# 0xPolygonHermez/pil2-stark-js

Hardware: AMD Instinct MI355X
Metric: STARK prove time (ms_per_step) and trace-cells/s, synthetic Fibonacci AIR, GL Poseidon Merkle + FRI, blow-up 8 (higher is better)
Workload: dtype u64; 1 GPU; full proof (commit, Q, evals, FRI 27/22/17/12/7, 64 queries) of 2^24 rows x 100 cols -> 2^27 rows, plain linear hash, per GPU; mode=prove, config=c3, nBits=24, nCols=100, nBitsExt=27, hash=GL-Poseidon-12, parallelism=single GPU

## Files before the change

### include/pil2gl.h

```cpp
#pragma once
#include <stdint.h>
#include "pil2gl_expr.h"
#ifdef __cplusplus
extern "C" {
#endif

#define PIL2GL_OK        0
#define PIL2GL_EINVAL   -1
#define PIL2GL_ENODEV   -2
#define PIL2GL_ENOMEM   -3
#define PIL2GL_EHIP     -4

int         pil2gl_init(int device);
void        pil2gl_shutdown(void);
const char *pil2gl_last_error(void);
int         pil2gl_version(void);
int         pil2gl_device_info(char *name, uint32_t nameLen, uint32_t *numCUs, uint64_t *totalMem);

int pil2gl_dev_alloc(uint64_t nWords, uint64_t **out);
int pil2gl_dev_free(uint64_t *p);
int pil2gl_dev_zero(uint64_t *p, uint64_t nWords, void *stream);
int pil2gl_dev_upload(uint64_t *dst, const uint64_t *hostSrc, uint64_t nWords);
int pil2gl_dev_download(uint64_t *hostDst, const uint64_t *src, uint64_t nWords);
int pil2gl_sync(void *stream);

int pil2gl_host_alloc(uint64_t nWords, uint64_t **out);
int pil2gl_host_free(uint64_t *p);
int pil2gl_host_register(uint64_t *p, uint64_t nWords);
int pil2gl_host_unregister(uint64_t *p);
int pil2gl_dev_upload_async(uint64_t *dst, const uint64_t *hostSrc, uint64_t nWords);
int pil2gl_dev_download_async(uint64_t *hostDst, const uint64_t *src, uint64_t nWords);
int pil2gl_copy_after(void *stream);
int pil2gl_copy_fence(void *stream);
int pil2gl_copy_sync(void);
int pil2gl_land_rows_dev(const uint64_t *src, uint64_t srcCols, uint64_t *dst, uint64_t dstCols, uint64_t nRows,
                         uint64_t *hostFirstBad, void *stream);
int pil2gl_dev_load_file(const char *fileName, uint64_t byteOffset, uint64_t nRows, uint64_t srcCols,
                         uint64_t *dst, uint64_t dstCols, uint64_t chunkWords, uint64_t *hostFirstBad);
int pil2gl_dev_save_file(const char *fileName, uint64_t byteOffset, const uint64_t *src, uint64_t nWords, uint64_t chunkWords);

int pil2gl_interpolate(const uint64_t *src, uint64_t nPols, uint32_t nBits, uint64_t *dst, uint32_t nBitsExt);
int pil2gl_interpolate_dev(const uint64_t *src, uint64_t nPols, uint32_t nBits, uint64_t *dst, uint32_t nBitsExt, void *stream);
int pil2gl_interpolate_cosets_dev(const uint64_t *src, uint64_t nPols, uint32_t nBits, uint64_t *dst, uint32_t nBitsExt,
                                  uint32_t cosetBegin, uint32_t cosetCount, void *stream);
int pil2gl_extend_cosets_unshifted_dev(const uint64_t *src, uint64_t nPols, uint32_t nBits, uint64_t *dst, uint32_t nBitsExt,
                                       uint32_t cosetBegin, uint32_t cosetCount, void *stream);
int pil2gl_extend_coefs_brev_dev(const uint64_t *coefBrev, uint64_t nPols, uint32_t nBits, uint64_t *dst, uint32_t nBitsExt, void *stream);
int pil2gl_extend_coefs_brev_cosets_dev(const uint64_t *coefBrev, uint64_t nPols, uint32_t nBits, uint64_t *dst, uint32_t nBitsExt,
                                        uint32_t cosetBegin, uint32_t cosetCount, void *stream);
int pil2gl_interpolate_cosets_ws_dev(const uint64_t *src, uint64_t nPols, uint32_t nBits, uint64_t *dst, uint32_t nBitsExt,
                                     uint32_t cosetBegin, uint32_t cosetCount, uint64_t *workspace, void *stream);
int pil2gl_fft(const uint64_t *src, uint64_t nPols, uint32_t nBits, uint64_t *dst);
int pil2gl_ifft(const uint64_t *src, uint64_t nPols, uint32_t nBits, uint64_t *dst);
int pil2gl_fft_dev(const uint64_t *src, uint64_t nPols, uint32_t nBits, uint64_t *dst, void *stream);
int pil2gl_ifft_dev(const uint64_t *src, uint64_t nPols, uint32_t nBits, uint64_t *dst, void *stream);
int pil2gl_fft_block_dev(uint64_t *buf, uint64_t start_pos, uint64_t nPols, uint32_t nBits, uint32_t s, uint32_t blockBits, uint32_t layers, void *stream);
int pil2gl_interpolate_prepare_block_dev(uint64_t *buf, uint64_t width, uint64_t height, uint64_t start, uint64_t inc, void *stream);

int pil2gl_poseidon(const uint64_t *in, const uint64_t *cap, uint64_t count, uint32_t nOut, uint64_t *out);
int pil2gl_poseidon_dev(const uint64_t *in, const uint64_t *cap, uint64_t count, uint32_t nOut, uint64_t *out, void *stream);
int pil2gl_sponge_absorb(const uint64_t *hostBlocks, uint64_t nBlocks, const uint64_t hostCap[4], uint64_t hostOut12[12]);
int pil2gl_linear_hash_rows(const uint64_t *in, uint64_t width, uint64_t height, int split, uint64_t *out);
int pil2gl_linear_hash_rows_dev(const uint64_t *in, uint64_t width, uint64_t height, int split, uint64_t *out, void *stream);
int pil2gl_merkelize_level(const uint64_t *in, uint64_t nOps, uint64_t *out);
int pil2gl_merkelize_level_dev(const uint64_t *in, uint64_t nOps, uint64_t *out, void *stream);
uint64_t pil2gl_merkle_num_nodes(uint64_t height);
int pil2gl_merkelize(const uint64_t *elems, uint64_t width, uint64_t height, int split, uint64_t *nodes);
int pil2gl_merkelize_dev(const uint64_t *elems, uint64_t width, uint64_t height, int split, uint64_t *nodes, void *stream);
int pil2gl_merkelize_digests_dev(uint64_t *nodes, uint64_t height, void *stream);
int pil2gl_group_proof_dev(const uint64_t *elems, const uint64_t *nodes, uint64_t width, uint64_t height,
                           uint64_t idx, uint64_t *hostVals, uint64_t *hostSiblings, uint32_t *nLevels);

int pil2gl_group_proofs_dev(const uint64_t *elems, const uint64_t *nodes, uint64_t width, uint64_t height,
                            const uint64_t *hostIdxs, uint32_t nIdx, uint64_t *hostOut, uint32_t *nLevels);
int pil2gl_roots_from_group_proofs(const uint64_t *hostProofs, uint64_t width, uint32_t levels, const uint64_t *hostIdxs, uint32_t nIdx,
                                   int splitLinearHash, uint64_t *hostRoots );

int pil2gl_fri_fold(const uint64_t *pol, uint32_t polBits, uint32_t outBits, uint64_t shiftInv,
                    const uint64_t challenge[3], uint64_t *out);
int pil2gl_fri_fold_dev(const uint64_t *pol, uint32_t polBits, uint32_t outBits, uint64_t shiftInv,
                        const uint64_t challenge[3], uint64_t *out, void *stream);
int pil2gl_fri_verify_fold(const uint64_t *groups, uint32_t foldBits, uint32_t nQueries, const uint64_t *sinv,
                           const uint64_t challenge[3], uint64_t *out );
int pil2gl_fri_verify_fold_dev(const uint64_t *groups, uint32_t foldBits, uint32_t nQueries, const uint64_t *sinv,
                               const uint64_t challenge[3], uint64_t *out, void *stream);
int pil2gl_fri_transpose(const uint64_t *pol, uint32_t polBits, uint32_t transposeBits, uint64_t *out);
int pil2gl_fri_transpose_dev(const uint64_t *pol, uint32_t polBits, uint32_t transposeBits, uint64_t *out, void *stream);

int pil2gl_build_x_dev(uint32_t nBits, uint64_t shift, uint64_t *x, void *stream);
int pil2gl_geometric_dev(uint64_t first, uint64_t ratio, uint64_t n, uint64_t *out, void *stream);
int pil2gl_build_zhinv_dev(uint32_t nBits, uint32_t nBitsExt, uint64_t *out, void *stream);
int pil2gl_build_one_row_zerofier_inv_dev(uint32_t nBits, uint32_t nBitsExt, uint64_t rowIndex, uint64_t *out, void *stream);
int pil2gl_build_frame_zerofier_dev(uint32_t nBits, uint32_t nBitsExt, uint64_t offsetMin, uint64_t offsetMax, uint64_t *out, void *stream);
int pil2gl_compute_q_split_dev(const uint64_t *qq1, uint32_t nBits, uint32_t nBitsExt, uint32_t qDim, uint32_t qDeg, uint64_t *qq2, void *stream);
int pil2gl_compute_q_split_brev_dev(const uint64_t *qq1, uint32_t nBits, uint32_t nBitsExt, uint32_t qDim, uint32_t qDeg, uint64_t *coefBrev, void *stream);
int pil2gl_compute_q_stark_dev(const glx_program *prog, const glx_ctx *ctx, uint32_t qSection, uint32_t nBits, uint32_t nBitsExt,
                               uint32_t qDim, uint32_t qDeg, uint64_t *dstExt, void *stream);
int pil2gl_x_div_x_sub_xi_dev(uint32_t nBitsExt, const uint64_t xi[3], uint64_t nOpen, uint64_t iOpen, uint64_t *out, void *stream);
int pil2gl_x_div_x_sub_xi_cosets_dev(uint32_t nBitsExt, uint32_t extBits, const uint64_t xi[3], uint64_t nOpen, uint64_t iOpen,
                                     uint32_t cosetBegin, uint32_t cosetCount, uint64_t *out, void *stream);
int pil2gl_build_lev_dev(uint32_t nBits, const uint64_t xi[3], uint64_t *lev, void *stream);
typedef struct { const uint64_t *buf; uint64_t width; uint64_t offset; uint32_t dim; uint32_t levIndex; } pil2gl_eval_desc;
int pil2gl_compute_evals_dev(const pil2gl_eval_desc *descs, uint32_t nEvals, uint32_t nBits, uint32_t extendBits,
                             const uint64_t *const *levs, uint32_t nLevs, uint64_t *hostEvals , void *stream);

int pil2gl_rows_dot_ext_dev(const uint64_t *buf, uint64_t width, uint64_t nRows, const uint64_t *hostCoef, uint32_t nOut,
                            uint64_t *acc, int accumulate, void *stream);
int pil2gl_rows_dot_ext_multi_dev(const uint64_t *const *bufs, const uint64_t *widths, uint32_t nBufs, uint64_t nRows,
                                  const uint64_t *const *hostCoefs, uint32_t nOut, uint64_t *acc, int accumulate, void *stream);
int pil2gl_fri_combine_dev(const uint64_t *acc, const uint64_t *hostK, const uint64_t vf1[3], const uint64_t *xDivXSubXi,
                           uint32_t nOpen, uint64_t nRows, uint64_t *f, void *stream);
int pil2gl_fri_combine_order_dev(const uint64_t *acc, const uint64_t *hostK, const uint64_t vf1[3], const uint64_t *xDivXSubXi,
                                 uint32_t nOpen, const uint32_t *order, uint64_t nRows, uint64_t *f, void *stream);
int pil2gl_cols_dot_ext_dev(const uint64_t *buf, uint64_t width, uint64_t nRows, uint64_t rowStep, const uint64_t *const *levs,
                            uint32_t nLev, uint64_t *hostOut, void *stream);
int pil2gl_cols_dot_ext_multi_dev(const uint64_t *const *bufs, const uint64_t *widths, uint32_t nBufs, uint64_t nRows, uint64_t rowStep,
                                  const uint64_t *const *levs, uint32_t nLev, uint64_t *const *hostOuts, void *stream);
int pil2gl_cols_dot_ext_range_dev(const uint64_t *const *bufs, const uint64_t *strides, const uint64_t *colBegin, const uint64_t *widths, uint32_t nBufs,
                                  uint64_t nRows, uint64_t rowStep, const uint64_t *const *levs, uint32_t nLev, uint64_t *const *hostOuts, void *stream);

int pil2gl_eval_program_dev(const glx_program *prog, const glx_ctx *ctx, void *stream);
int pil2gl_first_nonzero_row_dev(const uint64_t *col, uint32_t dim, uint64_t first, uint64_t last, uint64_t *hostRow, uint64_t *hostVal, void *stream);

int pil2gl_gprod_dev(const uint64_t *num, uint32_t dimNum, const uint64_t *den, uint32_t dimDen, uint64_t n, uint64_t *out, void *stream);
int pil2gl_gsum_dev(const uint64_t *num, uint32_t dimNum, const uint64_t *den, uint32_t dimDen, uint64_t n, uint64_t *out, void *stream);
int pil2gl_h1h2_dev(const uint64_t *f, const uint64_t *t, uint64_t n, uint32_t dim, uint64_t *h1, uint64_t *h2, void *stream);

int pil2gl_bn128_poseidon(const uint64_t *in, const uint64_t *init, uint64_t count, uint32_t nIn, uint32_t nOut, uint64_t *out);
int pil2gl_bn128_sponge_absorb(const uint64_t *hostBlocks, uint64_t nBlocks, uint32_t nIn, const uint64_t hostInit[4], uint64_t *hostOut);
int pil2gl_bn128_poseidon_dev(const uint64_t *in, const uint64_t *init, uint64_t count, uint32_t nIn, uint32_t nOut, uint64_t *out, void *stream);
int pil2gl_bn128_linear_hash_rows(const uint64_t *in, uint64_t width, uint64_t height, uint32_t arity, int custom, uint64_t *out);
int pil2gl_bn128_linear_hash_rows_dev(const uint64_t *in, uint64_t width, uint64_t height, uint32_t arity, int custom, uint64_t *out, void *stream);
int pil2gl_bn128_merkelize_level_dev(const uint64_t *in, uint64_t nOps, uint32_t arity, uint64_t *out, void *stream);
uint64_t pil2gl_bn128_merkle_num_nodes(uint64_t height, uint32_t arity);
int pil2gl_bn128_merkelize(const uint64_t *elems, uint64_t width, uint64_t height, uint32_t arity, int custom, uint64_t *nodes);
int pil2gl_bn128_merkelize_dev(const uint64_t *elems, uint64_t width, uint64_t height, uint32_t arity, int custom, uint64_t *nodes, void *stream);
int pil2gl_bn128_group_proof_dev(const uint64_t *elems, const uint64_t *nodes, uint64_t width, uint64_t height, uint32_t arity,
                                 uint64_t idx, uint64_t *hostVals, uint64_t *hostSiblings, uint32_t *nLevels);
int pil2gl_bn128_group_proofs_dev(const uint64_t *elems, const uint64_t *nodes, uint64_t width, uint64_t height, uint32_t arity,
                                  const uint64_t *hostIdxs, uint32_t nIdx, uint64_t *hostVals, uint64_t *hostSiblings, uint32_t *nLevels);
int pil2gl_bn128_convert(const uint64_t *in, uint64_t n, int toMontgomery, uint64_t *out);
int pil2gl_bn128_convert_dev(const uint64_t *in, uint64_t n, int toMontgomery, uint64_t *out, void *stream);

int pil2gl_synth_fibonacci_dev(uint32_t nBits, uint32_t nPairs, const uint64_t *hostInit, uint64_t *cm, void *stream);

uint64_t pil2gl_add(uint64_t a, uint64_t b);
uint64_t pil2gl_mul(uint64_t a, uint64_t b);
uint64_t pil2gl_square(uint64_t a);

int pil2gl_selftest_field(const uint64_t *a, const uint64_t *b, uint64_t n, uint64_t *mul, uint64_t *add, uint64_t *sub);
int pil2gl_debug_compact_program(const glx_program *prog, glx_op *outOps, uint32_t *outInfo);
int pil2gl_debug_jit_compile(const glx_program *prog, const glx_ctx *ctx, uint64_t *codeBytes, uint32_t *fusedOps);
int pil2gl_debug_plan_program(const glx_program *prog, const glx_ctx *ctx, uint32_t *outInfo);
#define PIL2GL_PLAN_FFT 0
#define PIL2GL_PLAN_IFFT 1
#define PIL2GL_PLAN_INTERPOLATE 2
#define PIL2GL_PLAN_EXTEND_COEFS 3
#define PIL2GL_PLAN_LAUNCH_WORDS 14
int pil2gl_debug_plan_transform(uint32_t op, uint32_t nBits, uint64_t nPols, uint32_t nBitsExt, uint32_t cosetCount,
                                uint32_t *out, uint32_t maxLaunches, uint32_t *nLaunches);
int pil2gl_selftest_products(const uint64_t *a, const uint64_t *b, uint64_t n, uint64_t *x, uint64_t *pb, uint64_t *flag);
int pil2gl_selftest_mds(const uint64_t *states, uint64_t n, uint32_t layers, int mfma, uint64_t *out);
int pil2gl_selftest_poseidon(const uint64_t *states, uint64_t n, int what, uint64_t *out);
int pil2gl_selftest_clock(uint32_t iters, double *mhz);
int pil2gl_selftest_ext(const uint64_t *a, const uint64_t *b, uint64_t n, uint64_t *mul, uint64_t *inv);

#ifdef __cplusplus
}
#endif
```

### pil2-stark-js_amd/csrc/dot.hip

```cpp
#include "common.h"
#include "gl_field.cuh"
#include <vector>
#include <string.h>
#include <stdint.h>
#include <stdlib.h>
#include <algorithm>

using namespace gl;

namespace {

constexpr u32 LIMB_BITS = 22;
constexpr u32 LIMB_MASK = (1u << LIMB_BITS) - 1;

__device__ __forceinline__ u64 fold6(const u64 S[6]) {
    u64 r = canon(S[0]);
    r = add(r, mul(S[1], 1ull << 22));
    r = add(r, mul(S[2], 1ull << 44));
    r = add(r, mul(S[3], 1ull << 32));
    r = add(r, mul(S[4], 1ull << 54));
    r = add(r, mul(S[5], ((1ull << 32) - 1) << 12));
    return r;
}

struct RowsDotParams {
    const u64 *buf; u64 width; u64 nRows;
    u64 stride, col0;
    const u32 *coefLimbs;
    u32 nOut;
    u64 *acc;
    u32 accumulate;
};

template <int NOUT>
__global__ void __launch_bounds__(256) rows_dot_kernel(RowsDotParams P) {
    constexpr u32 CW = 16, LD = CW + 1;
    __shared__ u64 tile[4][64 * LD];
    const u32 wave = threadIdx.x >> 6, lane = threadIdx.x & 63;
    u64 *T = tile[wave];
    const u64 row0 = ((u64)blockIdx.x * 4 + wave) * 64;
    if (row0 >= P.nRows) return;
    u64 S[NOUT][3][6];
#pragma unroll
    for (int o = 0; o < NOUT; o++)
#pragma unroll
        for (int k = 0; k < 3; k++)
#pragma unroll
            for (int i = 0; i < 6; i++) S[o][k][i] = 0;
    const u64 myRow = row0 + lane;
    u64 nxt[CW];
    const u32 lr = lane >> 4, lc = lane & 15;
    auto fetch = [&](u64 c0) {
        const u32 cw = (u32)min((u64)CW, P.width - c0);
        u64 off = (row0 + lr) * P.stride + P.col0 + c0 + lc;
        asm volatile("" : "+v"(off));
        const u64 step = 4 * P.stride;
#pragma unroll
        for (u32 i = 0; i < CW; i++) {
            const u64 gr = row0 + lr + 4 * i;
            nxt[i] = (lc < cw && gr < P.nRows) ? P.buf[off + i * step] : 0;
        }
    };
    fetch(0);
    for (u64 c0 = 0; c0 < P.width; c0 += CW) {
        const u32 cw = (u32)min((u64)CW, P.width - c0);
        {
            u32 to = lr * LD + lc;
            asm volatile("" : "+v"(to));
#pragma unroll
            for (u32 i = 0; i < CW; i++) T[to + i * 4 * LD] = nxt[i];
        }
        if (c0 + CW < P.width) fetch(c0 + CW);
        __builtin_amdgcn_s_waitcnt(0xC07F);
        __builtin_amdgcn_wave_barrier();
        for (u32 c = 0; c < cw; c++) {
            const u64 p = T[lane * LD + c];
            const u32 p0 = (u32)p, p1 = (u32)(p >> 32);
#pragma unroll
            for (int o = 0; o < NOUT; o++) {
                const u32 *L = P.coefLimbs + (((u64)o * P.stride + P.col0 + c0 + c) * 9);
#pragma unroll
                for (int k = 0; k < 3; k++) {
                    const u32 w0 = L[3 * k], w1 = L[3 * k + 1], w2 = L[3 * k + 2];
                    S[o][k][0] += (u64)p0 * w0; S[o][k][1] += (u64)p0 * w1; S[o][k][2] += (u64)p0 * w2;
                    S[o][k][3] += (u64)p1 * w0; S[o][k][4] += (u64)p1 * w1; S[o][k][5] += (u64)p1 * w2;
                }
            }
        }
        __builtin_amdgcn_wave_barrier();
    }
    if (myRow >= P.nRows) return;
    u64 *out = P.acc + myRow * (3ull * P.nOut);
#pragma unroll
    for (int o = 0; o < NOUT; o++)
#pragma unroll
        for (int k = 0; k < 3; k++) {
            u64 v = fold6(S[o][k]);
            if (P.accumulate) v = add(v, out[3 * o + k]);
            out[3 * o + k] = v;
        }
}

constexpr u32 STREAM_CW_MAX = 128;
template <int NOUT>
__global__ void __launch_bounds__(256) rows_dot_stream_kernel(RowsDotParams P, u32 cw, u32 LD) {
    extern __shared__ u64 sm[];
    const u32 tid = threadIdx.x, lane = tid & 63;
    const u32 wave = __builtin_amdgcn_readfirstlane(tid >> 6);
    const u64 row0 = (u64)blockIdx.x * 64;
    u64 S[NOUT][3][6];
#pragma unroll
    for (int o = 0; o < NOUT; o++)
#pragma unroll
        for (int k = 0; k < 3; k++)
#pragma unroll
            for (int i = 0; i < 6; i++) S[o][k][i] = 0;
    constexpr u32 NB = 13;
    for (u64 c0 = 0; c0 < P.width; c0 += cw) {
        const u32 w = (u32)min((u64)cw, P.width - c0);
        const u32 total = 64 * w, dq = 256 / w, dr = 256 - dq * w;
        u32 r = tid / w, c = tid - r * w;
        for (u32 u0 = 0; u0 < total; u0 += 256 * NB) {
            u64 v[NB]; u32 at[NB];
#pragma unroll
            for (u32 i = 0; i < NB; i++) {
                const bool in = u0 + 256 * i + tid < total;
                at[i] = in ? r * LD + c : 0xFFFFFFFFu;
                v[i] = (in && row0 + r < P.nRows) ? P.buf[(row0 + r) * P.stride + P.col0 + c0 + c] : 0;
                c += dr; r += dq;
                if (c >= w) { c -= w; r++; }
            }
            if (u0 == 0) __syncthreads();
#pragma unroll
            for (u32 i = 0; i < NB; i++) if (at[i] != 0xFFFFFFFFu) sm[at[i]] = v[i];
        }
        __syncthreads();
        const u32 cb = w * wave / 4, ce = w * (wave + 1) / 4;
        for (u32 cc = cb; cc < ce; cc++) {
            const u64 p = sm[lane * LD + cc];
            const u32 p0 = (u32)p, p1 = (u32)(p >> 32);
#pragma unroll
            for (int o = 0; o < NOUT; o++) {
                const u32 *L = P.coefLimbs + (((u64)o * P.stride + P.col0 + c0 + cc) * 9);
#pragma unroll
                for (int k = 0; k < 3; k++) {
                    const u32 w0 = L[3 * k], w1 = L[3 * k + 1], w2 = L[3 * k + 2];
                    S[o][k][0] += (u64)p0 * w0; S[o][k][1] += (u64)p0 * w1; S[o][k][2] += (u64)p0 * w2;
                    S[o][k][3] += (u64)p1 * w0; S[o][k][4] += (u64)p1 * w1; S[o][k][5] += (u64)p1 * w2;
                }
            }
        }
    }
    __syncthreads();
    if (wave == 0) {
#pragma unroll
        for (int o = 0; o < NOUT; o++)
#pragma unroll
            for (int k = 0; k < 3; k++)
#pragma unroll
                for (int i = 0; i < 6; i++) sm[((o * 3 + k) * 6 + i) * 64 + lane] = S[o][k][i];
    }
    __syncthreads();
    if (wave != 0) {
#pragma unroll
        for (int o = 0; o < NOUT; o++)
#pragma unroll
            for (int k = 0; k < 3; k++)
#pragma unroll
                for (int i = 0; i < 6; i++)
                    __hip_atomic_fetch_add(&sm[((o * 3 + k) * 6 + i) * 64 + lane], S[o][k][i], __ATOMIC_RELAXED, __HIP_MEMORY_SCOPE_WORKGROUP);
    }
    __syncthreads();
    const u64 myRow = row0 + lane;
    if (myRow >= P.nRows) return;
    u64 *out = P.acc + myRow * (3ull * P.nOut);
    for (u32 pi = wave; pi < 3 * NOUT; pi += 4) {
        u64 T6[6];
#pragma unroll
        for (int i = 0; i < 6; i++) T6[i] = sm[(pi * 6 + i) * 64 + lane];
        u64 v = fold6(T6);
        if (P.accumulate) v = add(v, out[pi]);
        out[pi] = v;
    }
}


typedef int v4i __attribute__((ext_vector_type(4)));
typedef int v16i __attribute__((ext_vector_type(16)));
constexpr u32 MF_WAVES = 8, MF_ROWS = 64, MF_MAXW = 112;
constexpr int MF_PLANE_OFFSET = 1 << 24;

constexpr u32 MF_MAXSEG = 4;
struct RowsDotMfmaParams {
    const u64 *segBuf[MF_MAXSEG]; u32 segW[MF_MAXSEG], segPitch[MF_MAXSEG], segU0[MF_MAXSEG], nSeg;
    u64 nRows; u32 width, nOut;
    const v4i *atab;
    const u64 *bias;
    u64 *acc; u32 accumulate, accStride;
    u64 nTiles;
    u32 kSteps;
};

typedef int v4i_a8 __attribute__((ext_vector_type(4), aligned(8)));
template <int NT, bool ODD = false>
__global__ void __launch_bounds__(512, 1) rows_dot_mfma_kernel(RowsDotMfmaParams P) {
    extern __shared__ u64 sm[];
    constexpr u32 NTH = 64 * MF_WAVES, NG = MF_ROWS / 32;
    const u32 tid = threadIdx.x, lane = tid & 63;
    const u32 wave = __builtin_amdgcn_readfirstlane(tid >> 6);
    const u32 rowBytes = P.width * 8, LDB = rowBytes + 16;
    unsigned char *tile = (unsigned char *)sm;
    v4i *Alds = (v4i *)(tile + MF_ROWS * LDB);
    const u32 upr = P.width / 2;
    for (u32 i = tid; i < P.kSteps * NT * 64; i += NTH) Alds[i] = P.atab[i];
    const u32 n = lane & 31, gk = lane >> 5;
    const u32 total = MF_ROWS * upr, dq = NTH / upr, dr = NTH - dq * upr;
    constexpr u32 NL = (MF_ROWS * (MF_MAXW / 2) + NTH - 1) / NTH;
    const u32 r00 = tid / upr, c00 = tid - r00 * upr;
    v4i nxt[NL];
    auto fetch = [&](u64 tileIdx) {
        const u64 row0 = tileIdx * MF_ROWS;
        u32 r = r00, c = c00;
#pragma unroll
        for (u32 i = 0; i < NL; i++) {
            const v4i z = { 0, 0, 0, 0 };
            const u64 *sb = P.segBuf[0]; u32 sw = P.segW[0], sp = P.segPitch[0], su = 0;
#pragma unroll
            for (u32 k = 1; k < MF_MAXSEG; k++) if (k < P.nSeg && c >= P.segU0[k]) { sb = P.segBuf[k]; sw = P.segW[k]; sp = P.segPitch[k]; su = P.segU0[k]; }
            if constexpr (!ODD) nxt[i] = (NTH * i + tid < total && row0 + r < P.nRows) ? *(const v4i *)(sb + (row0 + r) * sp + 2 * (c - su)) : z;
            else {
                nxt[i] = z;
                if (NTH * i + tid < total && row0 + r < P.nRows) {
                    const u64 *q = sb + (row0 + r) * sp + 2 * (c - su);
                    if (2 * (c - su) + 1 < sw) nxt[i] = *(const v4i_a8 *)q;
                    else { const u64 v = *q; nxt[i][0] = (int)(u32)v; nxt[i][1] = (int)(u32)(v >> 32); }
                }
            }
            c += dr; r += dq;
            if (c >= upr) { c -= upr; r++; }
        }
    };
    if (blockIdx.x < P.nTiles) fetch(blockIdx.x);
    const u32 g = wave / NT, t = wave - g * NT;
    const unsigned char *brow = tile + (32 * g + n) * LDB + 16 * gk;
    const v4i *arow = Alds + t * 64 + lane;
    for (u64 tileIdx = blockIdx.x; tileIdx < P.nTiles; tileIdx += gridDim.x) {
        const u64 row0 = tileIdx * MF_ROWS;
        __syncthreads();
        {
            u32 r = r00, c = c00;
#pragma unroll
            for (u32 i = 0; i < NL; i++) {
                if (NTH * i + tid < total) *(v4i *)(tile + r * LDB + 16 * c) = nxt[i] ^ (int)0x80808080;
                c += dr; r += dq;
                if (c >= upr) { c -= upr; r++; }
            }
        }
        if (tileIdx + gridDim.x < P.nTiles) fetch(tileIdx + gridDim.x);
        __syncthreads();
        if (wave < NG * NT) {
            v16i acc;
#pragma unroll
            for (int i = 0; i < 16; i++) acc[i] = MF_PLANE_OFFSET;
            for (u32 s_ = 0; s_ < P.kSteps; s_++)
                acc = __builtin_amdgcn_mfma_i32_32x32x32_i8(arow[s_ * NT * 64], *(const v4i *)(brow + 32 * s_), acc, 0, 0, 0);
            const u32 o = 2 * t + gk;
            const u64 row = row0 + 32 * g + n;
            if (o < 3 * P.nOut && row < P.nRows) {
                u64 w[4];
#pragma unroll
                for (int j = 0; j < 4; j++)
                    w[j] = (u64)(u32)acc[4 * j] + ((u64)(u32)acc[4 * j + 1] << 8) + ((u64)(u32)acc[4 * j + 2] << 16) + ((u64)(u32)acc[4 * j + 3] << 24);
                u64 v = add(add(w[0], mul(w[1], 1ull << 32)), mul(w[2], EPS));
                v = add(sub(v, w[3]), P.bias[o]);
                u64 *out = P.acc + row * (u64)P.accStride + o;
                if (P.accumulate) v = add(v, *out);
                *out = v;
            }
        }
    }
}

__global__ void fri_combine_kernel(const u64 *__restrict__ acc, const u64 *__restrict__ K, E3 vf1, const u64 *__restrict__ xdiv,
                                   u32 nOpen, u32 order, u64 nRows, u64 *__restrict__ f) {
    const u64 r = (u64)blockIdx.x * blockDim.x + threadIdx.x;
    if (r >= nRows) return;
    E3 res = { { 0, 0, 0 } };
    for (u32 k = 0; k < nOpen; k++) {
        const u32 o = (order >> (8 * k)) & 255;
        const u64 *a = acc + (r * nOpen + o) * 3, *x = xdiv + (r * nOpen + o) * 3;
        E3 F = { { sub(a[0], K[3 * o]), sub(a[1], K[3 * o + 1]), sub(a[2], K[3 * o + 2]) } };
        E3 X = { { x[0], x[1], x[2] } };
        E3 t = e3_mul(F, X);
        res = k == 0 ? t : e3_add(e3_mul(vf1, res), t);
    }
    f[3 * r] = res.v[0]; f[3 * r + 1] = res.v[1]; f[3 * r + 2] = res.v[2];
}

constexpr u32 CD_MAXSEG = 8;
struct ColsDotParams {
    const u64 *segBuf[CD_MAXSEG]; u32 segW[CD_MAXSEG], segC0[CD_MAXSEG], segStride[CD_MAXSEG], nSeg;
    u64 width; u64 nRows; u64 rowStep;
    const u32 *levLimbs;
    u32 nLev;
    u64 *partial;
    u32 rowsPerChunk;
};

template <int NLEV>
__global__ void __launch_bounds__(256) cols_dot_kernel(ColsDotParams P) {
    const u64 c = (u64)blockIdx.y * blockDim.x + threadIdx.x;
    const u64 chunk = blockIdx.x;
    const u64 k0 = chunk * P.rowsPerChunk, k1 = min(P.nRows, k0 + P.rowsPerChunk);
    u64 S[NLEV][3][6];
#pragma unroll
    for (int l = 0; l < NLEV; l++)
#pragma unroll
        for (int k = 0; k < 3; k++)
#pragma unroll
            for (int i = 0; i < 6; i++) S[l][k][i] = 0;
    const bool valid = c < P.width;
    constexpr int RB = 8;
    const u64 *buf = P.segBuf[0]; u64 sw = P.segStride[0], cl = c;
#pragma unroll
    for (u32 k = 1; k < CD_MAXSEG; k++) if (k < P.nSeg && c >= P.segC0[k]) { buf = P.segBuf[k]; sw = P.segStride[k]; cl = c - P.segC0[k]; }
    const u64 stride = P.rowStep * sw;
    for (u64 kb = k0; kb < k1; kb += RB) {
        u64 pv[RB];
#pragma unroll
        for (int j = 0; j < RB; j++) pv[j] = (valid && kb + j < k1) ? buf[(kb + j) * stride + cl] : 0;
#pragma unroll
        for (int j = 0; j < RB; j++) {
            const u64 k = kb + j;
            if (k >= k1) break;
            const u32 p0 = (u32)pv[j], p1 = (u32)(pv[j] >> 32);
#pragma unroll
            for (int l = 0; l < NLEV; l++) {
                const u32 *L = P.levLimbs + (((u64)l * P.nRows + k) * 9);
#pragma unroll
                for (int q = 0; q < 3; q++) {
                    const u32 w0 = L[3 * q], w1 = L[3 * q + 1], w2 = L[3 * q + 2];
                    S[l][q][0] += (u64)p0 * w0; S[l][q][1] += (u64)p0 * w1; S[l][q][2] += (u64)p0 * w2;
                    S[l][q][3] += (u64)p1 * w0; S[l][q][4] += (u64)p1 * w1; S[l][q][5] += (u64)p1 * w2;
                }
            }
        }
    }
    if (!valid) return;
#pragma unroll
    for (int l = 0; l < NLEV; l++)
#pragma unroll
        for (int q = 0; q < 3; q++)
            P.partial[((chunk * P.nLev + l) * P.width + c) * 3 + q] = fold6(S[l][q]);
}
__global__ void cols_dot_final_kernel(const u64 *__restrict__ partial, u64 nChunks, u64 per, u64 n , u64 *__restrict__ out) {
    const u64 i = (u64)blockIdx.x * blockDim.x + threadIdx.x;
    if (i >= n) return;
    const u64 c0 = (u64)blockIdx.y * per, c1 = min(nChunks, c0 + per);
    u64 acc = 0;
    for (u64 ch = c0; ch < c1; ch++) acc = add(acc, partial[ch * n + i]);
    out[(u64)blockIdx.y * n + i] = acc;
}
__global__ void limbs_kernel(const u64 *__restrict__ in, u64 n, u32 *__restrict__ out) {
    const u64 i = (u64)blockIdx.x * blockDim.x + threadIdx.x;
    if (i >= n) return;
    const u64 v = in[i];
    out[3 * i] = (u32)v & LIMB_MASK; out[3 * i + 1] = (u32)(v >> LIMB_BITS) & LIMB_MASK; out[3 * i + 2] = (u32)(v >> (2 * LIMB_BITS));
}

inline unsigned nblk(u64 n, u32 t = 256) { return (unsigned)((n + t - 1) / t); }

}

using namespace pil2gl;

struct MfSeg { const u64 *buf; u64 pitch, col0, width; const u64 *coef; };
static u64 mf_padded(const MfSeg *segs, u32 n) { u64 t = 0; for (u32 k = 0; k < n; k++) t += segs[k].width + (segs[k].width & 1); return t; }
static bool rows_dot_mfma_fits(const MfSeg *segs, u32 nSeg, u32 nOut) {
    const char *sw = getenv("PIL2GL_ROWS_DOT_MFMA");
    if ((sw && sw[0] == '0') || nOut < 1 || nOut > 2 || nSeg < 1 || nSeg > MF_MAXSEG) return false;
    for (u32 k = 0; k < nSeg; k++)
        if (segs[k].width == 0 || ((uintptr_t)segs[k].buf & 7) || (segs[k].pitch >> 31)) return false;
    const u64 total = mf_padded(segs, nSeg);
    if (total < 32 || total > MF_MAXW) return false;
    static int ldsMax = -1;
    if (ldsMax < 0) {
        int dev = 0, v = 0;
        (void)hipGetDevice(&dev);
        if (hipDeviceGetAttribute(&v, hipDeviceAttributeMaxSharedMemoryPerBlock, dev) != hipSuccess) v = 0;
        ldsMax = v;
    }
    const u32 kSteps = (u32)((total * 8 + 31) / 32), NT = nOut == 1 ? 2 : 3;
    const size_t need = (size_t)MF_ROWS * (total * 8 + 16) + (size_t)kSteps * NT * 1024;
    return (size_t)ldsMax >= need;
}
static int launch_rows_dot_mfma(const MfSeg *segs, u32 nBufs, u64 nRows, u32 nOut, u64 *acc, u32 accStride, bool accumulate, hipStream_t st) {
    const u64 Pm = 0xFFFFFFFF00000001ull;
    const int NT = nOut == 1 ? 2 : 3;
    const u32 nO = 3 * nOut;
    const u64 winWidth = mf_padded(segs, nBufs);
    bool odd = false;
    for (u32 k = 0; k < nBufs; k++) odd |= ((segs[k].width | segs[k].pitch | segs[k].col0) & 1) != 0 || ((uintptr_t)segs[k].buf & 15);
    std::vector<signed char> dig((size_t)winWidth * nO * 9, 0);
    std::vector<u64> bias(nO);
    unsigned __int128 k128 = 0, offs = 0;
    for (int i = 0; i < 8; i++) k128 += (unsigned __int128)128 << (8 * i);
    {
        unsigned __int128 pw = 1;
        for (int p_ = 0; p_ < 16; p_++) { offs = (offs + (pw * (u64)MF_PLANE_OFFSET) % Pm) % Pm; pw = (pw * 256) % Pm; }
    }
    for (u32 o = 0; o < nO; o++) {
        unsigned __int128 sumw = 0;
        u64 c = 0;
        for (u32 k = 0; k < nBufs; k++, c += c & 1)
            for (u64 cl = 0; cl < segs[k].width; cl++, c++) {
                u64 w = segs[k].coef[((u64)(o / 3) * segs[k].pitch + segs[k].col0 + cl) * 3 + (o % 3)] % Pm;
                sumw = (sumw + w) % Pm;
                int carry = 0;
                for (int j = 0; j < 9; j++) {
                    int b = (j < 8 ? (int)((w >> (8 * j)) & 255) : 0) + carry;
                    carry = 0;
                    if (b >= 128) { b -= 256; carry = 1; }
                    dig[((size_t)c * nO + o) * 9 + j] = (signed char)b;
                }
            }
        unsigned __int128 b = ((k128 % Pm) * sumw) % Pm;
        bias[o] = (u64)((b + Pm - offs) % Pm);
    }
    const u32 kSteps = (u32)((winWidth * 8 + 31) / 32);
    std::vector<signed char> atab((size_t)kSteps * NT * 64 * 16, 0);
    for (u32 s_ = 0; s_ < kSteps; s_++)
        for (int t = 0; t < NT; t++)
            for (u32 lane = 0; lane < 64; lane++) {
                const u32 m = lane & 31, gk = lane >> 5;
                const u32 h = (m >> 2) & 1, pl = 4 * (m >> 3) + (m & 3), o = 2 * t + h;
                if (o >= nO) continue;
                signed char *dst = &atab[(((size_t)s_ * NT + t) * 64 + lane) * 16];
                for (u32 kk = 0; kk < 16; kk++) {
                    const u64 byteOff = 32ull * s_ + 16 * gk + kk;
                    if (byteOff >= winWidth * 8) continue;
                    const u64 c = byteOff >> 3; const u32 i = (u32)(byteOff & 7);
                    const int j = (int)pl - (int)i;
                    dst[kk] = (j >= 0 && j <= 8) ? dig[((size_t)c * nO + o) * 9 + j] : 0;
                }
            }
    u64 *d;
    const size_t atWords = (atab.size() + 7) / 8;
    P2_TRY(scratch(7, atWords + nO + 2, &d));
    HIP_TRY(hipMemcpyAsync(d, atab.data(), atab.size(), hipMemcpyHostToDevice, st));
    HIP_TRY(hipMemcpyAsync(d + atWords, bias.data(), nO * 8, hipMemcpyHostToDevice, st));
    RowsDotMfmaParams P;
    u32 u0 = 0;
    for (u32 k = 0; k < MF_MAXSEG; k++) {
        P.segBuf[k] = k < nBufs ? segs[k].buf + segs[k].col0 : nullptr; P.segW[k] = k < nBufs ? (u32)segs[k].width : 0; P.segPitch[k] = k < nBufs ? (u32)segs[k].pitch : 0; P.segU0[k] = u0;
        if (k < nBufs) u0 += (u32)((segs[k].width + 1) / 2);
    }
    P.nSeg = nBufs; P.nRows = nRows; P.width = (u32)winWidth; P.nOut = nOut; P.atab = (const v4i *)d; P.bias = d + atWords;
    P.acc = acc; P.accumulate = (u32)accumulate; P.accStride = accStride; P.nTiles = (nRows + MF_ROWS - 1) / MF_ROWS; P.kSteps = kSteps;
    const size_t lds = (size_t)MF_ROWS * (winWidth * 8 + 16) + atab.size();
    int dev = 0, cus = 256;
    (void)hipGetDevice(&dev);
    (void)hipDeviceGetAttribute(&cus, hipDeviceAttributeMultiprocessorCount, dev);
    const unsigned grid = (unsigned)std::min<u64>(P.nTiles, (u64)cus);
#define RD_LAUNCH(NT_, ODD_) { HIP_TRY(hipFuncSetAttribute((const void *)rows_dot_mfma_kernel<NT_, ODD_>, hipFuncAttributeMaxDynamicSharedMemorySize, (int)lds)); \
                              hipLaunchKernelGGL((rows_dot_mfma_kernel<NT_, ODD_>), dim3(grid), dim3(64 * MF_WAVES), lds, st, P); }
    if (NT == 2) { if (odd) RD_LAUNCH(2, true) else RD_LAUNCH(2, false) }
    else { if (odd) RD_LAUNCH(3, true) else RD_LAUNCH(3, false) }
#undef RD_LAUNCH
    KERNEL_CHECK();
    HIP_TRY(hipStreamSynchronize(st));
    return PIL2GL_OK;
}

static int rows_dot_ext_plain(const uint64_t *buf, uint64_t width, uint64_t nRows, const uint64_t *hostCoef, uint32_t nOut,
                              uint64_t *acc, int accumulate, void *stream) {
    hipStream_t st = as_stream(stream);
    const u64 nC = (u64)nOut * width * 3;
    std::vector<u32> limbs(nC * 3);
    for (u64 i = 0; i < nC; i++) {
        const u64 v = hostCoef[i] % 0xFFFFFFFF00000001ull;
        limbs[3 * i] = (u32)v & LIMB_MASK; limbs[3 * i + 1] = (u32)(v >> LIMB_BITS) & LIMB_MASK; limbs[3 * i + 2] = (u32)(v >> (2 * LIMB_BITS));
    }
    u64 *d;
    P2_TRY(scratch(7, (limbs.size() * 4 + 7) / 8 + 1, &d));
    HIP_TRY(hipMemcpyAsync(d, limbs.data(), limbs.size() * 4, hipMemcpyHostToDevice, st));
    const unsigned blocks = (unsigned)((nRows + 255) / 256);
    const char *sw = getenv("PIL2GL_ROWS_DOT_STREAM");
    const bool stream_ok = !(sw && sw[0] == '0');
    for (u64 col0 = 0; col0 < width; col0 += 1024) {
        RowsDotParams P = { buf, std::min<u64>(1024, width - col0), nRows, width, col0, (const u32 *)d, nOut, acc, (u32)(accumulate != 0 || col0 != 0) };
        if (stream_ok && P.width >= 32) {
            const u32 nch = (u32)((P.width + STREAM_CW_MAX - 1) / STREAM_CW_MAX), cw = (u32)((P.width + nch - 1) / nch), LD = cw | 1;
            const size_t lds = 8 * std::max<size_t>((size_t)64 * LD, (size_t)nOut * 18 * 64);
            const unsigned sb = (unsigned)((nRows + 63) / 64);
#define STREAM_CASE(N_) { if (lds > 48 * 1024) HIP_TRY(hipFuncSetAttribute((const void *)rows_dot_stream_kernel<N_>, hipFuncAttributeMaxDynamicSharedMemorySize, (int)lds)); \
                          hipLaunchKernelGGL((rows_dot_stream_kernel<N_>), dim3(sb), dim3(256), lds, st, P, cw, LD); }
            switch (nOut) {
            case 1: STREAM_CASE(1) break;
            case 2: STREAM_CASE(2) break;
            case 3: STREAM_CASE(3) break;
            default: STREAM_CASE(4) break;
            }
#undef STREAM_CASE
            KERNEL_CHECK();
            continue;
        }
        switch (nOut) {
        case 1: rows_dot_kernel<1><<<blocks, 256, 0, st>>>(P); break;
        case 2: rows_dot_kernel<2><<<blocks, 256, 0, st>>>(P); break;
        case 3: rows_dot_kernel<3><<<blocks, 256, 0, st>>>(P); break;
        default: rows_dot_kernel<4><<<blocks, 256, 0, st>>>(P); break;
        }
        KERNEL_CHECK();
    }
    HIP_TRY(hipStreamSynchronize(st));
    return PIL2GL_OK;
}

static bool rows_dot_mfma_plan(const uint64_t *const *bufs, const uint64_t *widths, const uint64_t *const *hostCoefs, u32 nBufs, u32 nOut,
                               std::vector<std::vector<MfSeg>> &launches, std::vector<u32> &leftovers) {
    std::vector<MfSeg> wins;
    for (u32 k = 0; k < nBufs; k++) {
        const u64 W = widths[k];
        if (W == 0) continue;
        const u64 n = (W + (W & 1) + MF_MAXW - 1) / MF_MAXW;
        u64 per = (W + n - 1) / n; per += per & 1;
        for (u64 c0 = 0; c0 < W; c0 += per) wins.push_back({ bufs[k], W, c0, std::min<u64>(per, W - c0), hostCoefs[k] });
    }
    std::stable_sort(wins.begin(), wins.end(), [](const MfSeg &a, const MfSeg &b) { return a.width > b.width; });
    std::vector<u64> fill;
    for (const MfSeg &w : wins) {
        const u64 pw = w.width + (w.width & 1);
        size_t b = 0;
        while (b < launches.size() && (launches[b].size() >= MF_MAXSEG || fill[b] + pw > MF_MAXW)) b++;
        if (b == launches.size()) { launches.emplace_back(); fill.push_back(0); }
        launches[b].push_back(w); fill[b] += pw;
    }
    bool any = false;
    for (size_t b = 0; b < launches.size();) {
        if (rows_dot_mfma_fits(launches[b].data(), (u32)launches[b].size(), std::min<u32>(nOut, 2))) { any = true; b++; continue; }
        for (const MfSeg &w : launches[b]) {
            if (w.width != w.pitch) return false;
            for (u32 k = 0; k < nBufs; k++) if (bufs[k] == w.buf && hostCoefs[k] == w.coef) { leftovers.push_back(k); break; }
        }
        launches.erase(launches.begin() + b); fill.erase(fill.begin() + b);
    }
    return any;
}

extern "C" {

int pil2gl_rows_dot_ext_multi_dev(const uint64_t *const *bufs, const uint64_t *widths, uint32_t nBufs, uint64_t nRows,
                                  const uint64_t *const *hostCoefs, uint32_t nOut, uint64_t *acc, int accumulate, void *stream);
int pil2gl_rows_dot_ext_dev(const uint64_t *buf, uint64_t width, uint64_t nRows, const uint64_t *hostCoef, uint32_t nOut,
                            uint64_t *acc, int accumulate, void *stream) {
    P2_TRY(ensure_init());
    if (!buf || !hostCoef || !acc) return fail(PIL2GL_EINVAL, "null buffer");
    if (nOut < 1 || nOut > 4) return fail(PIL2GL_EINVAL, "nOut must be 1..4");
    if (width == 0 || nRows == 0) return PIL2GL_OK;
    return pil2gl_rows_dot_ext_multi_dev(&buf, &width, 1, nRows, &hostCoef, nOut, acc, accumulate, stream);
}

int pil2gl_rows_dot_ext_multi_dev(const uint64_t *const *bufs, const uint64_t *widths, uint32_t nBufs, uint64_t nRows,
                                  const uint64_t *const *hostCoefs, uint32_t nOut, uint64_t *acc, int accumulate, void *stream) {
    P2_TRY(ensure_init());
    if (!bufs || !widths || !hostCoefs || !acc || nBufs == 0) return fail(PIL2GL_EINVAL, "null buffer");
    for (uint32_t k = 0; k < nBufs; k++) if (!bufs[k] || !hostCoefs[k]) return fail(PIL2GL_EINVAL, "null buffer");
    if (nOut < 1 || nOut > 4) return fail(PIL2GL_EINVAL, "nOut must be 1..4");
    if (nRows == 0) return PIL2GL_OK;
    std::vector<std::vector<MfSeg>> launches;
    std::vector<u32> leftovers;
    bool acc1 = accumulate != 0;
    if (rows_dot_mfma_plan(bufs, widths, hostCoefs, nBufs, nOut, launches, leftovers)) {
        for (u32 o0 = 0; o0 < nOut; o0 += 2) {
            const u32 no = std::min<u32>(2, nOut - o0);
            bool accg = accumulate != 0;
            for (auto l : launches) {
                for (MfSeg &sg : l) sg.coef += (u64)o0 * sg.pitch * 3;
                P2_TRY(launch_rows_dot_mfma(l.data(), (u32)l.size(), nRows, no, acc + 3 * o0, 3 * nOut, accg, as_stream(stream)));
                accg = true;
            }
        }
        acc1 = true;
        for (u32 k : leftovers) P2_TRY(rows_dot_ext_plain(bufs[k], widths[k], nRows, hostCoefs[k], nOut, acc, 1, stream));
        return PIL2GL_OK;
    }
    for (uint32_t k = 0; k < nBufs; k++) {
        if (widths[k] == 0) continue;
        P2_TRY(rows_dot_ext_plain(bufs[k], widths[k], nRows, hostCoefs[k], nOut, acc, acc1 ? 1 : 0, stream)); acc1 = true;
    }
    return PIL2GL_OK;
}

int pil2gl_fri_combine_dev(const uint64_t *acc, const uint64_t *hostK, const uint64_t vf1[3], const uint64_t *xDivXSubXi,
                           uint32_t nOpen, uint64_t nRows, uint64_t *f, void *stream) {
    const uint32_t ident[4] = { 0, 1, 2, 3 };
    return pil2gl_fri_combine_order_dev(acc, hostK, vf1, xDivXSubXi, nOpen, ident, nRows, f, stream);
}
int pil2gl_fri_combine_order_dev(const uint64_t *acc, const uint64_t *hostK, const uint64_t vf1[3], const uint64_t *xDivXSubXi,
                                 uint32_t nOpen, const uint32_t *order, uint64_t nRows, uint64_t *f, void *stream) {
    P2_TRY(ensure_init());
    if (!acc || !hostK || !vf1 || !xDivXSubXi || !f || !order || nOpen < 1 || nOpen > 4) return fail(PIL2GL_EINVAL, "bad FRI combine arguments");
    u32 ord = 0, seen = 0;
    for (u32 k = 0; k < nOpen; k++) {
        if (order[k] >= nOpen || (seen >> order[k] & 1)) return fail(PIL2GL_EINVAL, "order must be a permutation of the openings");
        seen |= 1u << order[k]; ord |= order[k] << (8 * k);
    }
    hipStream_t st = as_stream(stream);
    std::vector<u64> k(hostK, hostK + 3ull * nOpen);
    u64 *d;
    P2_TRY(scratch(7, 16, &d));
    HIP_TRY(hipMemcpyAsync(d, k.data(), k.size() * 8, hipMemcpyHostToDevice, st));
    E3 v = { { vf1[0], vf1[1], vf1[2] } };
    fri_combine_kernel<<<nblk(nRows), 256, 0, st>>>(acc, d, v, xDivXSubXi, nOpen, ord, nRows, f);
    KERNEL_CHECK();
    HIP_TRY(hipStreamSynchronize(st));
    return PIL2GL_OK;
}

int pil2gl_cols_dot_ext_multi_dev(const uint64_t *const *bufs, const uint64_t *widths, uint32_t nBufs, uint64_t nRows, uint64_t rowStep,
                                  const uint64_t *const *levs, uint32_t nLev, uint64_t *const *hostOuts, void *stream) {
    return pil2gl_cols_dot_ext_range_dev(bufs, widths, nullptr, widths, nBufs, nRows, rowStep, levs, nLev, hostOuts, stream);
}
int pil2gl_cols_dot_ext_range_dev(const uint64_t *const *bufs, const uint64_t *strides, const uint64_t *colBegin, const uint64_t *widths, uint32_t nBufs,
                                  uint64_t nRows, uint64_t rowStep, const uint64_t *const *levs, uint32_t nLev, uint64_t *const *hostOuts, void *stream) {
    P2_TRY(ensure_init());
    if (!bufs || !widths || !strides || !levs || !hostOuts || nBufs == 0) return fail(PIL2GL_EINVAL, "null buffer");
    for (uint32_t k = 0; k < nBufs && k < CD_MAXSEG; k++)
        if ((colBegin ? colBegin[k] : 0) + widths[k] > strides[k] || (strides[k] >> 31)) return fail(PIL2GL_EINVAL, "column range outside the matrix");
    if (nBufs > CD_MAXSEG) return fail(PIL2GL_EINVAL, "at most %u matrices per call", CD_MAXSEG);
    if (nLev < 1 || nLev > 64) return fail(PIL2GL_EINVAL, "nLev must be 1..64");
    u64 width = 0;
    for (uint32_t k = 0; k < nBufs; k++) { if (!bufs[k] || !hostOuts[k]) return fail(PIL2GL_EINVAL, "null buffer"); if (widths[k] >> 31) return fail(PIL2GL_EINVAL, "matrix too wide"); width += widths[k]; }
    for (uint32_t l = 0; l < nLev; l++) if (!levs[l]) return fail(PIL2GL_EINVAL, "null buffer");
    if (width == 0 || nRows == 0) return PIL2GL_OK;
    if (nLev > 4) {
        for (uint32_t l0 = 0; l0 < nLev; l0 += 4) {
            std::vector<uint64_t *> outs(nBufs);
            for (uint32_t k = 0; k < nBufs; k++) outs[k] = hostOuts[k] + (u64)l0 * widths[k] * 3;
            P2_TRY(pil2gl_cols_dot_ext_range_dev(bufs, strides, colBegin, widths, nBufs, nRows, rowStep, levs + l0, std::min<u32>(4, nLev - l0), outs.data(), stream));
        }
        return PIL2GL_OK;
    }
    hipStream_t st = as_stream(stream);
    const u32 rpc = 1024;
    const u64 nChunks = (nRows + rpc - 1) / rpc, n = (u64)nLev * width * 3;
    u64 *d;
    const u64 nGroups = std::min<u64>(64, nChunks), per = (nChunks + nGroups - 1) / nGroups;
    P2_TRY(scratch(7, ((u64)nLev * nRows * 9 * 4 + 7) / 8 + nChunks * n + nGroups * n + n + 1, &d));
    u32 *limbs = (u32 *)d;
    u64 *partial = d + ((u64)nLev * nRows * 9 * 4 + 7) / 8, *part2 = partial + nChunks * n, *res = part2 + nGroups * n;
    for (u32 l = 0; l < nLev; l++) limbs_kernel<<<nblk(nRows * 3), 256, 0, st>>>(levs[l], nRows * 3, limbs + (u64)l * nRows * 9);
    ColsDotParams P;
    u32 c0 = 0;
    for (u32 k = 0; k < CD_MAXSEG; k++) {
        P.segBuf[k] = k < nBufs ? bufs[k] + (colBegin ? colBegin[k] : 0) : nullptr; P.segW[k] = k < nBufs ? (u32)widths[k] : 0; P.segStride[k] = k < nBufs ? (u32)strides[k] : 0;
        P.segC0[k] = c0; if (k < nBufs) c0 += (u32)widths[k];
    }
    P.nSeg = nBufs; P.width = width; P.nRows = nRows; P.rowStep = rowStep; P.levLimbs = limbs; P.nLev = nLev; P.partial = partial; P.rowsPerChunk = rpc;
    const u32 threads = (u32)std::min<u64>(256, (width + 63) / 64 * 64);
    dim3 grid((unsigned)nChunks, nblk(width, threads));
    switch (nLev) {
    case 1: cols_dot_kernel<1><<<grid, threads, 0, st>>>(P); break;
    case 2: cols_dot_kernel<2><<<grid, threads, 0, st>>>(P); break;
    case 3: cols_dot_kernel<3><<<grid, threads, 0, st>>>(P); break;
    default: cols_dot_kernel<4><<<grid, threads, 0, st>>>(P); break;
    }
    cols_dot_final_kernel<<<dim3(nblk(n), (unsigned)nGroups), 256, 0, st>>>(partial, nChunks, per, n, part2);
    cols_dot_final_kernel<<<dim3(nblk(n), 1), 256, 0, st>>>(part2, (nChunks + per - 1) / per, nGroups, n, res);
    KERNEL_CHECK();
    std::vector<u64> host(n);
    HIP_TRY(hipMemcpyAsync(host.data(), res, n * 8, hipMemcpyDeviceToHost, st));
    HIP_TRY(hipStreamSynchronize(st));
    u64 cbeg = 0;
    for (uint32_t k = 0; k < nBufs; k++) {
        for (u32 l = 0; l < nLev; l++)
            memcpy(hostOuts[k] + ((u64)l * widths[k]) * 3, host.data() + ((u64)l * width + cbeg) * 3, widths[k] * 3 * 8);
        cbeg += widths[k];
    }
    return PIL2GL_OK;
}

int pil2gl_cols_dot_ext_dev(const uint64_t *buf, uint64_t width, uint64_t nRows, uint64_t rowStep, const uint64_t *const *levs,
                            uint32_t nLev, uint64_t *hostOut, void *stream) {
    if (!buf || !hostOut) { P2_TRY(ensure_init()); return fail(PIL2GL_EINVAL, "null buffer"); }
    return pil2gl_cols_dot_ext_multi_dev(&buf, &width, 1, nRows, rowStep, levs, nLev, &hostOut, stream);
}

}
```

### pil2-stark-js_amd/csrc/fri.hip

```cpp
#include "common.h"
#include "gl_field.cuh"
#include <vector>

using namespace gl;

namespace {

__device__ __forceinline__ u64 pow256(const u64 *__restrict__ T, u32 e) {
    u64 r = T[e & 255];
    r = mul_lazy(r, T[256 + ((e >> 8) & 255)]);
    r = mul_lazy(r, T[512 + ((e >> 16) & 255)]);
    return mul(r, T[768 + (e >> 24)]);
}
__device__ __forceinline__ u64 root_pow(const u64 *__restrict__ T, u32 logM, u32 e) { return logM ? pow256(T, e << (32 - logM)) : 1; }

__device__ __forceinline__ E3 ld3(const u64 *p) { return { { p[0], p[1], p[2] } }; }
__device__ __forceinline__ void st3(u64 *p, const E3 &v) { p[0] = v.v[0]; p[1] = v.v[1]; p[2] = v.v[2]; }

__global__ void fri_horner_kernel(const u64 *__restrict__ coef, u32 polBits, u64 pol2N, u64 nX, u64 shiftInv, E3 challenge,
                                  const u64 *__restrict__ powWi, const u64 *__restrict__ sinvOf, u64 *__restrict__ out) {
    const u64 g = (u64)blockIdx.x * blockDim.x + threadIdx.x;
    if (g >= pol2N) return;
    const u64 sinv = sinvOf ? sinvOf[g] : mul(shiftInv, root_pow(powWi, polBits, (u32)g));
    const E3 Y = e3_scale(challenge, sinv);
    E3 acc = ld3(coef + ((nX - 1) * pol2N + g) * 3);
    for (u64 i = nX - 1; i-- > 0;) acc = e3_add(e3_mul(acc, Y), ld3(coef + (i * pol2N + g) * 3));
    st3(out + 3 * g, acc);
}

__global__ void fri_transpose_kernel(const u64 *__restrict__ pol, u32 polBits, u32 tBits, u64 *__restrict__ out) {
    const u64 o = (u64)blockIdx.x * blockDim.x + threadIdx.x;
    const u64 n = 1ull << polBits;
    if (o >= n) return;
    const u64 h = n >> tBits;
    const u64 i = o / h, j = o - i * h;
    st3(out + 3 * o, ld3(pol + 3 * ((j << tBits) + i)));
}

__global__ void build_x_kernel(u32 nBits, u64 shift, const u64 *__restrict__ powW, u64 *__restrict__ x) {
    const u64 i = (u64)blockIdx.x * blockDim.x + threadIdx.x;
    if (i >= (1ull << nBits)) return;
    x[i] = mul(shift, root_pow(powW, nBits, (u32)i));
}
struct GeomPow { u64 p[40]; };
__global__ void geometric_kernel(u64 first, GeomPow R, u64 n, u64 *__restrict__ out) {
    const u64 i = (u64)blockIdx.x * blockDim.x + threadIdx.x;
    if (i >= n) return;
    u64 acc = first;
    for (u32 b = 0; (i >> b) != 0; b++) if ((i >> b) & 1) acc = mul(acc, R.p[b]);
    out[i] = acc;
}
__global__ void periodic_kernel(const u64 *__restrict__ tab, u64 period, u64 n, u64 *__restrict__ out) {
    const u64 i = (u64)blockIdx.x * blockDim.x + threadIdx.x;
    if (i < n) out[i] = tab[i % period];
}

template <int CH>
__device__ __forceinline__ void batch_inv(u64 v[CH]) {
    u64 pre[CH];
    u64 acc = 1;
#pragma unroll
    for (int i = 0; i < CH; i++) { pre[i] = acc; acc = mul(acc, v[i]); }
    u64 z = inv(acc);
#pragma unroll
    for (int i = CH - 1; i >= 0; i--) { u64 t = mul(z, pre[i]); z = mul(z, v[i]); v[i] = t; }
}

__global__ void one_row_zerofier_kernel(u32 nBitsExt, u64 root, const u64 *__restrict__ zh, u64 ext,
                                        const u64 *__restrict__ powW, u64 *__restrict__ out) {
    constexpr int CH = 8;
    const u64 i0 = ((u64)blockIdx.x * blockDim.x + threadIdx.x) * CH;
    const u64 n = 1ull << nBitsExt;
    if (i0 >= n) return;
    u64 v[CH];
#pragma unroll
    for (int k = 0; k < CH; k++) { u64 i = i0 + k < n ? i0 + k : i0; v[k] = sub(mul(7, root_pow(powW, nBitsExt, (u32)i)), root); }
    batch_inv<CH>(v);
#pragma unroll
    for (int k = 0; k < CH; k++) if (i0 + k < n) out[i0 + k] = mul(v[k], zh[(i0 + k) % ext]);
}
__global__ void frame_zerofier_kernel(u32 nBitsExt, const u64 *__restrict__ roots, u32 nRoots, const u64 *__restrict__ powW, u64 *__restrict__ out) {
    const u64 i = (u64)blockIdx.x * blockDim.x + threadIdx.x;
    if (i >= (1ull << nBitsExt)) return;
    const u64 x = mul(7, root_pow(powW, nBitsExt, (u32)i));
    u64 zi = 1;
    for (u32 j = 0; j < nRoots; j++) zi = mul(zi, sub(x, roots[j]));
    out[i] = zi;
}
__global__ void q_split_kernel(const u64 *__restrict__ qq1, u32 nBits, u32 nBitsExt, u32 qDim, u32 qDeg,
                               const u64 *__restrict__ sPow , u64 *__restrict__ qq2) {
    const u64 o = (u64)blockIdx.x * blockDim.x + threadIdx.x;
    const u64 W = (u64)qDim * qDeg, N = 1ull << nBits;
    if (o >= (W << nBitsExt)) return;
    const u64 i = o / W, r = o - i * W;
    if (i >= N) { qq2[o] = 0; return; }
    const u64 p = r / qDim, k = r - p * qDim;
    qq2[o] = mul(qq1[(p * N + i) * qDim + k], sPow[p]);
}
__global__ void q_split_brev_kernel(const u64 *__restrict__ qq1, u32 nBits, u32 qDim, u32 qDeg, const u64 *__restrict__ sPow, u64 *__restrict__ out) {
    const u64 o = (u64)blockIdx.x * blockDim.x + threadIdx.x;
    const u64 W = (u64)qDim * qDeg, N = 1ull << nBits;
    if (o >= W * N) return;
    const u64 i = o / W, r = o - i * W;
    const u64 p = r / qDim, k = r - p * qDim;
    out[(u64)bitrev32((u32)i, nBits) * W + r] = mul(qq1[(p * N + i) * qDim + k], sPow[p]);
}
constexpr int XD_BATCH = 16;
struct XDivConst { u64 xi0, b, c, c2, bc2, m1, k0, cc, ccbb; };
__global__ void __launch_bounds__(256) x_div_x_sub_xi_kernel(u32 nBitsExt, XDivConst K, u64 nOpen, u64 iOpen, const u64 *__restrict__ powW, u64 wStep, u64 *__restrict__ out,
                                                             u64 E , u32 extBits, u32 cosetBegin, u32 ccLog) {
    const u64 T = (u64)gridDim.x * blockDim.x;
    const u64 k0 = (u64)blockIdx.x * blockDim.x + threadIdx.x;
    if (k0 >= E) return;
    u64 xs[XD_BATCH], as[XD_BATCH], ts[XD_BATCH], pre[XD_BATCH];
    const u64 g0 = ((k0 >> ccLog) << extBits) + cosetBegin + (k0 & ((1ull << ccLog) - 1));
    u64 x = mul(7, root_pow(powW, nBitsExt, (u32)g0));
    int n = 0;
#pragma unroll
    for (int i = 0; i < XD_BATCH; i++) {
        if (k0 + (u64)i * T < E) {
            const u64 a = sub(x, K.xi0);
            const u64 u = mul(a, add(a, K.c2));
            const u64 t = add(mul(a, add(sub(K.m1, u), K.bc2)), K.k0);
            xs[i] = x; as[i] = a; ts[i] = t;
            pre[i] = i ? mul(pre[i - 1], t) : t;
            x = mul(x, wStep);
            n = i + 1;
        }
    }
    u64 tinv = inv(pre[n - 1]);
#pragma unroll
    for (int i = XD_BATCH - 1; i >= 0; i--) {
        if (i < n) {
            const u64 ti = i ? mul(tinv, pre[i - 1]) : tinv;
            if (i) tinv = mul(tinv, ts[i]);
            const u64 a = as[i], s = mul(ti, xs[i]);
            const u64 i1 = sub(K.m1, mul(a, add(a, K.c2)));
            const u64 i2 = sub(mul(K.b, a), K.cc);
            const u64 i3 = add(mul(K.c, a), K.ccbb);
            u64 *o = out + 3 * ((k0 + (u64)i * T) * nOpen + iOpen);
            o[0] = mul(i1, s); o[1] = mul(i2, s); o[2] = mul(i3, s);
        }
    }
}
__global__ void lev_pow_kernel(u32 nBits, const u64 *__restrict__ xiPow, u64 *__restrict__ lev) {
    const u64 k = (u64)blockIdx.x * blockDim.x + threadIdx.x;
    if (k >= (1ull << nBits)) return;
    E3 acc = { { 1, 0, 0 } };
    for (u32 b = 0; b < nBits; b++) if ((k >> b) & 1) acc = e3_mul(acc, ld3(xiPow + 3 * b));
    st3(lev + 3 * k, acc);
}
__global__ void evals_partial_kernel(pil2gl_eval_desc d, const u64 *__restrict__ lev, u32 nBits, u32 eb, u64 *__restrict__ partial) {
    __shared__ u64 red[256 * 3];
    const u64 N = 1ull << nBits;
    E3 acc = { { 0, 0, 0 } };
    for (u64 k = (u64)blockIdx.x * blockDim.x + threadIdx.x; k < N; k += (u64)gridDim.x * blockDim.x) {
        const u64 *v = d.buf + (k << eb) * d.width + d.offset;
        const E3 l = ld3(lev + 3 * k);
        acc = e3_add(acc, d.dim == 1 ? e3_scale(l, v[0]) : e3_mul(ld3(v), l));
    }
    red[threadIdx.x * 3] = acc.v[0]; red[threadIdx.x * 3 + 1] = acc.v[1]; red[threadIdx.x * 3 + 2] = acc.v[2];
    __syncthreads();
    for (u32 s = blockDim.x / 2; s > 0; s >>= 1) {
        if (threadIdx.x < s) for (int c = 0; c < 3; c++) red[threadIdx.x * 3 + c] = add(red[threadIdx.x * 3 + c], red[(threadIdx.x + s) * 3 + c]);
        __syncthreads();
    }
    if (threadIdx.x < 3) partial[(u64)blockIdx.x * 3 + threadIdx.x] = red[threadIdx.x];
}
__global__ void evals_final_kernel(const u64 *__restrict__ partial, u32 nBlocks, u32 nEvals, u64 *__restrict__ out) {
    const u32 e = blockIdx.x * blockDim.x + threadIdx.x;
    if (e >= nEvals * 3) return;
    const u32 ev = e / 3, c = e % 3;
    u64 acc = 0;
    for (u32 b = 0; b < nBlocks; b++) acc = add(acc, partial[((u64)ev * nBlocks + b) * 3 + c]);
    out[e] = acc;
}

__global__ void synth_fibonacci_kernel(u32 nBits, u32 nPairs, const u64 *__restrict__ init, u64 *__restrict__ cm) {
    const u32 k = blockIdx.x * blockDim.x + threadIdx.x;
    if (k >= nPairs) return;
    u64 l1 = canon(init[2 * k]), l2 = canon(init[2 * k + 1]);
    const u64 N = 1ull << nBits, W = 2ull * nPairs;
    for (u64 i = 0; i < N; i++) {
        cm[i * W + 2 * k] = l1; cm[i * W + 2 * k + 1] = l2;
        const u64 n1 = add(mul(l1, l1), mul(l2, l2));
        l2 = l1; l1 = n1;
    }
}

inline unsigned nblk(u64 n, u32 t = 256) { return (unsigned)((n + t - 1) / t); }

}

using namespace pil2gl;

extern "C" {

int pil2gl_fri_fold_dev(const uint64_t *pol, uint32_t polBits, uint32_t outBits, uint64_t shiftInv,
                        const uint64_t challenge[3], uint64_t *out, void *stream) {
    P2_TRY(ensure_init());
    if (!pol || !out || !challenge) return fail(PIL2GL_EINVAL, "null buffer");
    if (outBits > polBits || polBits > PIL2GL_MAX_NTT_BITS) return fail(PIL2GL_EINVAL, "Invalid polynomial size");
    hipStream_t st = as_stream(stream);
    const u64 n = 1ull << polBits;
    u64 *coef;
    P2_TRY(scratch(1, 3 * n, &coef));
    P2_TRY(ntt_launch(pol, 3ull << outBits, polBits - outBits, coef, true, st));
    E3 ch = { { challenge[0], challenge[1], challenge[2] } };
    fri_horner_kernel<<<nblk(1ull << outBits), 256, 0, st>>>(coef, polBits, 1ull << outBits, 1ull << (polBits - outBits), shiftInv, ch, tables().powWi, nullptr, out);
    KERNEL_CHECK();
    return PIL2GL_OK;
}

int pil2gl_fri_verify_fold_dev(const uint64_t *groups, uint32_t foldBits, uint32_t nQueries, const uint64_t *sinv,
                               const uint64_t challenge[3], uint64_t *out, void *stream) {
    P2_TRY(ensure_init());
    if (!groups || !sinv || !out || !challenge) return fail(PIL2GL_EINVAL, "null buffer");
    if (foldBits > 20 || nQueries == 0) return fail(PIL2GL_EINVAL, "Invalid group size or query count");
    hipStream_t st = as_stream(stream);
    const u64 nX = 1ull << foldBits;
    const u64 *coef = groups;
    if (foldBits > 0) {
        u64 *c;
        P2_TRY(scratch(1, 3 * nX * nQueries, &c));
        P2_TRY(ntt_launch(groups, 3ull * nQueries, foldBits, c, true, st));
        coef = c;
    }
    E3 ch = { { challenge[0], challenge[1], challenge[2] } };
    fri_horner_kernel<<<nblk(nQueries), 256, 0, st>>>(coef, 0, nQueries, nX, 0, ch, tables().powWi, sinv, out);
    KERNEL_CHECK();
    return PIL2GL_OK;
}

int pil2gl_fri_transpose_dev(const uint64_t *pol, uint32_t polBits, uint32_t transposeBits, uint64_t *out, void *stream) {
    P2_TRY(ensure_init());
    if (!pol || !out) return fail(PIL2GL_EINVAL, "null buffer");
    if (transposeBits > polBits || polBits > 31) return fail(PIL2GL_EINVAL, "Invalid polynomial size");
    fri_transpose_kernel<<<nblk(1ull << polBits), 256, 0, as_stream(stream)>>>(pol, polBits, transposeBits, out);
    KERNEL_CHECK();
    return PIL2GL_OK;
}

static int host3(const uint64_t *in, u64 nIn, uint64_t *out, u64 nOut, int (*fn)(const u64 *, u64 *, void *), void *arg) {
    P2_TRY(ensure_init());
    u64 *d = nullptr;
    HIP_TRY(hipMalloc((void **)&d, (nIn + nOut + 1) * 8));
    int rc = PIL2GL_OK;
    hipError_t e = hipMemcpy(d, in, nIn * 8, hipMemcpyHostToDevice);
    if (e != hipSuccess) rc = hip_fail(e, "hipMemcpy H2D");
    if (rc == PIL2GL_OK) rc = fn(d, d + nIn, arg);
    if (rc == PIL2GL_OK) { e = hipMemcpy(out, d + nIn, nOut * 8, hipMemcpyDeviceToHost); if (e != hipSuccess) rc = hip_fail(e, "hipMemcpy D2H"); }
    (void)hipFree(d);
    return rc;
}
struct FoldArgs { u32 polBits, outBits; u64 shiftInv; const u64 *ch; };
int pil2gl_fri_fold(const uint64_t *pol, uint32_t polBits, uint32_t outBits, uint64_t shiftInv, const uint64_t challenge[3], uint64_t *out) {
    if (outBits > polBits || polBits > PIL2GL_MAX_NTT_BITS) return fail(PIL2GL_EINVAL, "Invalid polynomial size");
    FoldArgs a = { polBits, outBits, shiftInv, challenge };
    return host3(pol, 3ull << polBits, out, 3ull << outBits,
                 [](const u64 *i, u64 *o, void *p) { FoldArgs *a = (FoldArgs *)p; return pil2gl_fri_fold_dev(i, a->polBits, a->outBits, a->shiftInv, a->ch, o, nullptr); }, &a);
}
int pil2gl_fri_verify_fold(const uint64_t *groups, uint32_t foldBits, uint32_t nQueries, const uint64_t *sinv,
                           const uint64_t challenge[3], uint64_t *out) {
    P2_TRY(ensure_init());
    if (!groups || !sinv || !out || !challenge) return fail(PIL2GL_EINVAL, "null buffer");
    if (foldBits > 20 || nQueries == 0) return fail(PIL2GL_EINVAL, "Invalid group size or query count");
    const u64 nG = (3ull << foldBits) * nQueries;
    u64 *d = nullptr;
    HIP_TRY(hipMalloc((void **)&d, (nG + 4ull * nQueries) * 8));
    int rc = PIL2GL_OK;
    hipError_t e = hipMemcpy(d, groups, nG * 8, hipMemcpyHostToDevice);
    if (e == hipSuccess) e = hipMemcpy(d + nG, sinv, nQueries * 8ull, hipMemcpyHostToDevice);
    if (e != hipSuccess) rc = hip_fail(e, "hipMemcpy H2D");
    if (rc == PIL2GL_OK) rc = pil2gl_fri_verify_fold_dev(d, foldBits, nQueries, d + nG, challenge, d + nG + nQueries, nullptr);
    if (rc == PIL2GL_OK) { e = hipMemcpy(out, d + nG + nQueries, 3ull * nQueries * 8, hipMemcpyDeviceToHost); if (e != hipSuccess) rc = hip_fail(e, "hipMemcpy D2H"); }
    (void)hipFree(d);
    return rc;
}
int pil2gl_fri_transpose(const uint64_t *pol, uint32_t polBits, uint32_t transposeBits, uint64_t *out) {
    if (transposeBits > polBits || polBits > 31) return fail(PIL2GL_EINVAL, "Invalid polynomial size");
    u32 a[2] = { polBits, transposeBits };
    return host3(pol, 3ull << polBits, out, 3ull << polBits,
                 [](const u64 *i, u64 *o, void *p) { u32 *a = (u32 *)p; return pil2gl_fri_transpose_dev(i, a[0], a[1], o, nullptr); }, a);
}

int pil2gl_build_x_dev(uint32_t nBits, uint64_t shift, uint64_t *x, void *stream) {
    P2_TRY(ensure_init());
    if (nBits > 31) return fail(PIL2GL_EINVAL, "nBits too large");
    if (!x) return fail(PIL2GL_EINVAL, "null buffer");
    build_x_kernel<<<nblk(1ull << nBits), 256, 0, as_stream(stream)>>>(nBits, shift, tables().powW, x);
    KERNEL_CHECK();
    return PIL2GL_OK;
}

int pil2gl_geometric_dev(uint64_t first, uint64_t ratio, uint64_t n, uint64_t *out, void *stream) {
    P2_TRY(ensure_init());
    if (n == 0) return PIL2GL_OK;
    if (!out || n > (1ull << 40)) return fail(PIL2GL_EINVAL, "bad geometric-sequence arguments");
    if ((n + 255) / 256 > 0x7fffffffull) return fail(PIL2GL_EINVAL, "grid too large");
    const u64 p = 0xFFFFFFFF00000001ull;
    GeomPow R;
    u64 cur = ratio % p;
    for (int b = 0; b < 40; b++) { R.p[b] = cur; cur = h_mul(cur, cur); }
    geometric_kernel<<<nblk(n), 256, 0, as_stream(stream)>>>(first % p, R, n, out);
    KERNEL_CHECK();
    return PIL2GL_OK;
}

static void zh_table(u32 nBits, u32 nBitsExt, std::vector<u64> &zh, bool inverted) {
    u32 eb = nBitsExt - nBits;
    u64 sn = 7;
    for (u32 i = 0; i < nBits; i++) sn = h_mul(sn, sn);
    u64 w = 1, we = h_root(eb);
    zh.resize(1ull << eb);
    for (u64 i = 0; i < zh.size(); i++) { u64 z = h_sub(h_mul(sn, w), 1); zh[i] = inverted ? h_inv(z) : z; w = h_mul(w, we); }
}
static int upload_small(const std::vector<u64> &h, u32 slot, u64 **d, hipStream_t st) {
    P2_TRY(scratch(slot, h.size() ? h.size() : 1, d));
    HIP_TRY(hipMemcpyAsync(*d, h.data(), h.size() * 8, hipMemcpyHostToDevice, st));
    return PIL2GL_OK;
}

int pil2gl_build_zhinv_dev(uint32_t nBits, uint32_t nBitsExt, uint64_t *out, void *stream) {
    P2_TRY(ensure_init());
    if (nBitsExt < nBits || nBitsExt > 31 || nBitsExt - nBits > 20) return fail(PIL2GL_EINVAL, "bad domain sizes");
    if (!out) return fail(PIL2GL_EINVAL, "null buffer");
    std::vector<u64> zh; zh_table(nBits, nBitsExt, zh, true);
    u64 *d; P2_TRY(upload_small(zh, 2, &d, as_stream(stream)));
    periodic_kernel<<<nblk(1ull << nBitsExt), 256, 0, as_stream(stream)>>>(d, zh.size(), 1ull << nBitsExt, out);
    KERNEL_CHECK();
    HIP_TRY(hipStreamSynchronize(as_stream(stream)));
    return PIL2GL_OK;
}
int pil2gl_build_one_row_zerofier_inv_dev(uint32_t nBits, uint32_t nBitsExt, uint64_t rowIndex, uint64_t *out, void *stream) {
    P2_TRY(ensure_init());
    if (nBitsExt < nBits || nBitsExt > 31 || nBitsExt - nBits > 20) return fail(PIL2GL_EINVAL, "bad domain sizes");
    if (!out) return fail(PIL2GL_EINVAL, "null buffer");
    std::vector<u64> zh; zh_table(nBits, nBitsExt, zh, false);
    u64 *d; P2_TRY(upload_small(zh, 2, &d, as_stream(stream)));
    u64 root = h_pow(h_root(nBits), rowIndex);
    one_row_zerofier_kernel<<<nblk(((1ull << nBitsExt) + 7) / 8), 256, 0, as_stream(stream)>>>(nBitsExt, root, d, zh.size(), tables().powW, out);
    KERNEL_CHECK();
    HIP_TRY(hipStreamSynchronize(as_stream(stream)));
    return PIL2GL_OK;
}
int pil2gl_build_frame_zerofier_dev(uint32_t nBits, uint32_t nBitsExt, uint64_t offsetMin, uint64_t offsetMax, uint64_t *out, void *stream) {
    P2_TRY(ensure_init());
    if (nBitsExt < nBits || nBitsExt > 31 || offsetMin + offsetMax > 4096 || !out) return fail(PIL2GL_EINVAL, "bad frame zerofier arguments");
    std::vector<u64> roots;
    u64 w = h_root(nBits), N = 1ull << nBits;
    for (u64 i = 0; i < offsetMin; i++) roots.push_back(h_pow(w, i));
    for (u64 i = 0; i < offsetMax; i++) roots.push_back(h_pow(w, N - i - 1));
    u64 *d; P2_TRY(upload_small(roots, 2, &d, as_stream(stream)));
    frame_zerofier_kernel<<<nblk(1ull << nBitsExt), 256, 0, as_stream(stream)>>>(nBitsExt, d, (u32)roots.size(), tables().powW, out);
    KERNEL_CHECK();
    HIP_TRY(hipStreamSynchronize(as_stream(stream)));
    return PIL2GL_OK;
}
int pil2gl_compute_q_split_dev(const uint64_t *qq1, uint32_t nBits, uint32_t nBitsExt, uint32_t qDim, uint32_t qDeg, uint64_t *qq2, void *stream) {
    P2_TRY(ensure_init());
    if (!qq1 || !qq2) return fail(PIL2GL_EINVAL, "null buffer");
    if (nBitsExt < nBits || nBitsExt > 31 || !qDim || !qDeg || ((u64)qDeg << nBits) > (1ull << nBitsExt)) return fail(PIL2GL_EINVAL, "bad q split arguments");
    std::vector<u64> sp(qDeg);
    u64 shiftIn = h_pow(h_inv(7), 1ull << nBits), cur = 1;
    for (u32 p = 0; p < qDeg; p++) { sp[p] = cur; cur = h_mul(cur, shiftIn); }
    u64 *d; P2_TRY(upload_small(sp, 2, &d, as_stream(stream)));
    q_split_kernel<<<nblk(((u64)qDim * qDeg) << nBitsExt), 256, 0, as_stream(stream)>>>(qq1, nBits, nBitsExt, qDim, qDeg, d, qq2);
    KERNEL_CHECK();
    HIP_TRY(hipStreamSynchronize(as_stream(stream)));
    return PIL2GL_OK;
}
int pil2gl_compute_q_split_brev_dev(const uint64_t *qq1, uint32_t nBits, uint32_t nBitsExt, uint32_t qDim, uint32_t qDeg, uint64_t *coefBrev, void *stream) {
    P2_TRY(ensure_init());
    if (!qq1 || !coefBrev) return fail(PIL2GL_EINVAL, "null buffer");
    if (nBitsExt < nBits || nBitsExt > 31 || !qDim || !qDeg || ((u64)qDeg << nBits) > (1ull << nBitsExt)) return fail(PIL2GL_EINVAL, "bad q split arguments");
    std::vector<u64> sp(qDeg);
    u64 shiftIn = h_pow(h_inv(7), 1ull << nBits), cur = 1;
    for (u32 p = 0; p < qDeg; p++) { sp[p] = cur; cur = h_mul(cur, shiftIn); }
    u64 *d; P2_TRY(upload_small(sp, 2, &d, as_stream(stream)));
    q_split_brev_kernel<<<nblk(((u64)qDim * qDeg) << nBits), 256, 0, as_stream(stream)>>>(qq1, nBits, qDim, qDeg, d, coefBrev);
    KERNEL_CHECK();
    HIP_TRY(hipStreamSynchronize(as_stream(stream)));
    return PIL2GL_OK;
}
int pil2gl_compute_q_stark_dev(const glx_program *prog, const glx_ctx *ctx, uint32_t qSection, uint32_t nBits, uint32_t nBitsExt,
                               uint32_t qDim, uint32_t qDeg, uint64_t *dstExt, void *stream) {
    P2_TRY(ensure_init());
    if (!prog || !ctx || !dstExt || (prog->nOps && !prog->ops) || (ctx->nSections && !ctx->sections)) return fail(PIL2GL_EINVAL, "null argument");
    if (nBitsExt < nBits || nBitsExt > PIL2GL_MAX_NTT_BITS || !qDim || !qDeg || ((u64)qDeg << nBits) > (1ull << nBitsExt)) return fail(PIL2GL_EINVAL, "bad q stage arguments");
    if (ctx->nBits != nBitsExt) return fail(PIL2GL_EINVAL, "the context has 2^%u rows, the extended domain 2^%u", ctx->nBits, nBitsExt);
    if (qSection >= ctx->nSections || ctx->sections[qSection].width != qDim) return fail(PIL2GL_EINVAL, "section %u is not a destination of %u columns", qSection, qDim);
    u32 m = nBits;
    while ((1ull << m) < ((u64)qDeg << nBits)) m++;
    const u32 s = nBitsExt - m;
    for (u32 k = 0; k < prog->nOps; k++) {
        const glx_op &o = prog->ops[k];
        if (o.dest.kind == GLX_SEC && o.dest.section != qSection) return fail(PIL2GL_EINVAL, "op %u writes section %u, not the quotient's", k, o.dest.section);
        for (int t = 0; t < 3; t++) {
            const glx_ref &r = t < 2 ? o.src[t] : o.dest;
            if (r.kind == GLX_SEC && r.prime != 0 && ctx->primeShift < s && !(t == 1 && o.op == GLX_OP_COPY))
                return fail(PIL2GL_EINVAL, "op %u: row offset %d << %u leaves the rows k * 2^%u", k, r.prime, ctx->primeShift, s);
        }
    }
    for (u32 i = 0; i < ctx->nSections; i++) if (i != qSection && (ctx->sections[i].width << s) >> 32) return fail(PIL2GL_EINVAL, "section %u too wide", i);
    const u64 M = 1ull << m, W = (u64)qDim * qDeg;
    u64 *q, *coef;
    P2_TRY(scratch(14, M * qDim, &q));
    P2_TRY(scratch(15, W << nBits, &coef));
    std::vector<glx_section> secs(ctx->sections, ctx->sections + ctx->nSections);
    for (u32 i = 0; i < ctx->nSections; i++) secs[i].width <<= s;
    secs[qSection].ptr = q; secs[qSection].width = qDim;
    glx_ctx sub = *ctx;
    sub.nBits = m; sub.primeShift = ctx->primeShift < s ? 0 : ctx->primeShift - s; sub.sections = secs.data();
    P2_TRY(pil2gl_eval_program_dev(prog, &sub, stream));
    P2_TRY(ntt_launch(q, qDim, m, q, true, as_stream(stream)));
    P2_TRY(pil2gl_compute_q_split_brev_dev(q, nBits, nBitsExt, qDim, qDeg, coef, stream));
    return lde_launch(coef, W, nBits, dstExt, nBitsExt, as_stream(stream), 0, 0, nullptr, true, true);
}
static bool base_point_is_a_row(u64 xi0, u64 xi1, u64 xi2, u32 nBitsExt) {
    return xi1 == 0 && xi2 == 0 && h_pow(h_mul(xi0, h_inv(7)), 1ull << nBitsExt) == 1;
}
int pil2gl_x_div_x_sub_xi_dev(uint32_t nBitsExt, const uint64_t xi[3], uint64_t nOpen, uint64_t iOpen, uint64_t *out, void *stream) {
    return pil2gl_x_div_x_sub_xi_cosets_dev(nBitsExt, 0, xi, nOpen, iOpen, 0, 1, out, stream);
}
int pil2gl_x_div_x_sub_xi_cosets_dev(uint32_t nBitsExt, uint32_t extBits, const uint64_t xi[3], uint64_t nOpen, uint64_t iOpen,
                                     uint32_t cosetBegin, uint32_t cosetCount, uint64_t *out, void *stream) {
    P2_TRY(ensure_init());
    if (!xi || !out || iOpen >= nOpen || nBitsExt > 31 || extBits > nBitsExt) return fail(PIL2GL_EINVAL, "bad xDivXSubXi arguments");
    if (cosetCount == 0 || (cosetCount & (cosetCount - 1)) || (uint64_t)cosetBegin + cosetCount > (1ull << extBits))
        return fail(PIL2GL_EINVAL, "coset range [%u,%u) outside 2^%u (the count must be a power of two)", cosetBegin, cosetBegin + cosetCount, extBits);
    if (cosetCount > 256) return fail(PIL2GL_EINVAL, "at most 256 cosets per call (%u asked)", cosetCount);
    u32 ccLog = 0; while ((1u << ccLog) < cosetCount) ccLog++;
    const u64 GP = 0xFFFFFFFF00000001ull;
    const u64 xi0 = xi[0] % GP, b = h_sub(0, xi[1] % GP), c = h_sub(0, xi[2] % GP);
    if (base_point_is_a_row(xi0, b, c, nBitsExt)) return fail(PIL2GL_EINVAL, "xi is a point of the 2^%u-row coset 7<w>: x / (x - xi) divides by zero at that row", nBitsExt);
    const u64 bb = h_mul(b, b), cc = h_mul(c, c), bc = h_mul(b, c);
    XDivConst K;
    K.xi0 = xi0; K.b = b; K.c = c; K.c2 = h_add(c, c); K.bc2 = h_add(bc, bc);
    K.m1 = h_sub(h_add(bc, bb), cc);
    K.k0 = h_sub(h_sub(h_mul(b, cc), h_mul(bb, b)), h_mul(cc, c));
    K.cc = cc; K.ccbb = h_sub(cc, bb);
    const u64 E = (1ull << (nBitsExt - extBits)) << ccLog;
    const unsigned blocks = nblk((E + XD_BATCH - 1) / XD_BATCH);
    const u64 T = (u64)blocks * 256;
    const u64 wStep = h_pow(h_root(nBitsExt), (T >> ccLog) << extBits);
    x_div_x_sub_xi_kernel<<<blocks, 256, 0, as_stream(stream)>>>(nBitsExt, K, nOpen, iOpen, tables().powW, wStep, out, E, extBits, cosetBegin, ccLog);
    KERNEL_CHECK();
    return PIL2GL_OK;
}
__global__ void e3_scale_kernel(u64 *__restrict__ v, u64 n, E3 c) {
    const u64 k = (u64)blockIdx.x * blockDim.x + threadIdx.x;
    if (k < n) st3(v + 3 * k, e3_mul(ld3(v + 3 * k), c));
}
int pil2gl_build_lev_dev(uint32_t nBits, const uint64_t xi[3], uint64_t *lev, void *stream) {
    P2_TRY(ensure_init());
    if (!xi || !lev || nBits > PIL2GL_MAX_NTT_BITS) return fail(PIL2GL_EINVAL, "bad LEv arguments");
    static const bool viaNtt = getenv("PIL2GL_LEV_NTT") && atoi(getenv("PIL2GL_LEV_NTT"));
    const u64 GP = 0xFFFFFFFF00000001ull;
    if (!viaNtt && nBits > 0 && !base_point_is_a_row(h_mul(7, xi[0] % GP), xi[1] % GP, xi[2] % GP, nBits)) {
        u64 z[3] = { xi[0] % GP, xi[1] % GP, xi[2] % GP }, zN[3] = { z[0], z[1], z[2] };
        for (u32 b = 0; b < nBits; b++) h_e3_mul(zN, zN, zN);
        const u64 invN = h_inv((1ull << nBits) % GP);
        E3 c = { { h_mul(h_sub(1, zN[0]), invN), h_mul(h_sub(0, zN[1]), invN), h_mul(h_sub(0, zN[2]), invN) } };
        const u64 z7[3] = { h_mul(7, z[0]), h_mul(7, z[1]), h_mul(7, z[2]) };
        P2_TRY(pil2gl_x_div_x_sub_xi_cosets_dev(nBits, 0, z7, 1, 0, 0, 1, lev, stream));
        e3_scale_kernel<<<nblk(1ull << nBits), 256, 0, as_stream(stream)>>>(lev, 1ull << nBits, c);
        KERNEL_CHECK();
        HIP_TRY(hipStreamSynchronize(as_stream(stream)));
        return PIL2GL_OK;
    }
    std::vector<u64> xp(3 * (nBits ? nBits : 1));
    u64 cur[3] = { xi[0], xi[1], xi[2] };
    for (u32 b = 0; b < nBits; b++) { xp[3 * b] = cur[0]; xp[3 * b + 1] = cur[1]; xp[3 * b + 2] = cur[2]; h_e3_mul(cur, cur, cur); }
    u64 *d; P2_TRY(upload_small(xp, 2, &d, as_stream(stream)));
    lev_pow_kernel<<<nblk(1ull << nBits), 256, 0, as_stream(stream)>>>(nBits, d, lev);
    KERNEL_CHECK();
    P2_TRY(ntt_launch(lev, 3, nBits, lev, true, as_stream(stream)));
    HIP_TRY(hipStreamSynchronize(as_stream(stream)));
    return PIL2GL_OK;
}
int pil2gl_compute_evals_dev(const pil2gl_eval_desc *descs, uint32_t nEvals, uint32_t nBits, uint32_t extendBits,
                             const uint64_t *const *levs, uint32_t nLevs, uint64_t *hostEvals, void *stream) {
    P2_TRY(ensure_init());
    if (!nEvals) return PIL2GL_OK;
    if (!descs || !levs || !hostEvals) return fail(PIL2GL_EINVAL, "null buffer");
    hipStream_t st = as_stream(stream);
    const u32 nBlocks = (u32)std::min<u64>(256, ((1ull << nBits) + 255) / 256);
    u64 *partial, *res;
    P2_TRY(scratch(3, (u64)nEvals * nBlocks * 3 + (u64)nEvals * 3, &partial));
    res = partial + (u64)nEvals * nBlocks * 3;
    for (u32 e = 0; e < nEvals; e++) {
        if (descs[e].levIndex >= nLevs || (descs[e].dim != 1 && descs[e].dim != 3)) return fail(PIL2GL_EINVAL, "bad eval descriptor %u", e);
        evals_partial_kernel<<<nBlocks, 256, 0, st>>>(descs[e], levs[descs[e].levIndex], nBits, extendBits, partial + (u64)e * nBlocks * 3);
    }
    KERNEL_CHECK();
    evals_final_kernel<<<nblk(nEvals * 3), 256, 0, st>>>(partial, nBlocks, nEvals, res);
    KERNEL_CHECK();
    HIP_TRY(hipMemcpyAsync(hostEvals, res, (u64)nEvals * 24, hipMemcpyDeviceToHost, st));
    HIP_TRY(hipStreamSynchronize(st));
    return PIL2GL_OK;
}

int pil2gl_synth_fibonacci_dev(uint32_t nBits, uint32_t nPairs, const uint64_t *hostInit, uint64_t *cm, void *stream) {
    P2_TRY(ensure_init());
    if (!hostInit || !cm || nBits > 31 || nPairs == 0) return fail(PIL2GL_EINVAL, "bad synthetic trace arguments");
    std::vector<u64> h(hostInit, hostInit + 2ull * nPairs);
    u64 *d; P2_TRY(upload_small(h, 2, &d, as_stream(stream)));
    synth_fibonacci_kernel<<<nblk(nPairs, 64), 64, 0, as_stream(stream)>>>(nBits, nPairs, d, cm);
    KERNEL_CHECK();
    HIP_TRY(hipStreamSynchronize(as_stream(stream)));
    return PIL2GL_OK;
}

}
```

### pil2-stark-js_amd/csrc/merkle.hip

```cpp
#include "common.h"
#include <vector>
#include <string.h>
#include "poseidon_gl.cuh"
#include <algorithm>

using namespace gl;

namespace {

__device__ __forceinline__ void sponge(const u64 *__restrict__ v, u32 width, u64 digest[4], const MdsMfma &m) {
    u64 st[12];
    st[8] = st[9] = st[10] = st[11] = 0;
    for (u32 i = 0; i < width; i += 8) {
        const u32 n = min(8u, width - i);
#pragma unroll
        for (u32 j = 0; j < 8; j++) st[j] = j < n ? v[i + j] : 0;
        poseidon_perm<0, 4>(st, m);
        st[8] = st[0]; st[9] = st[1]; st[10] = st[2]; st[11] = st[3];
    }
    digest[0] = canon(st[8]); digest[1] = canon(st[9]); digest[2] = canon(st[10]); digest[3] = canon(st[11]);
}
__device__ __forceinline__ void linear_hash_plain(const u64 *__restrict__ v, u32 width, u64 digest[4], const MdsMfma &m) {
    if (width <= 4) {
#pragma unroll
        for (u32 j = 0; j < 4; j++) digest[j] = j < width ? v[j] : 0;
        return;
    }
    sponge(v, width, digest, m);
}

__global__ void __launch_bounds__(256, 4) linear_hash_kernel(const u64 *__restrict__ in, u64 width, u64 height, u64 *__restrict__ out) {
    const u64 row0 = (u64)blockIdx.x * blockDim.x + threadIdx.x;
    const bool live = row0 < height;
    const u64 row = live ? row0 : height - 1;
    const u64 *v = in + row * width;
    MdsMfma m;
    poseidon_init(m);
    u64 d[4];
    linear_hash_plain(v, (u32)width, d, m);
    if (!live) return;
    u64 *o = out + 4 * row;
    o[0] = d[0]; o[1] = d[1]; o[2] = d[2]; o[3] = d[3];
}

constexpr u32 SPLIT_BLOCK = 512;
__global__ void __launch_bounds__(SPLIT_BLOCK, 4) linear_hash_split_kernel(const u64 *__restrict__ in, u64 width, u64 height, u64 *__restrict__ out) {
    __shared__ u64 park[8][SPLIT_BLOCK];
    const u32 tid = threadIdx.x;
    const u64 row0 = (u64)blockIdx.x * blockDim.x + tid;
    const bool live = row0 < height;
    const u64 row = live ? row0 : height - 1;
    const u64 *v = in + row * width;
    MdsMfma m;
    poseidon_init(m);
    const u32 w = (u32)width, batch = max(8u, (w + 3) / 4), nb = (w + batch - 1) / batch;
    u64 st[12];
    for (u32 b = 0; b < nb; b++) {
        const u32 bw = min(batch, w - b * batch);
        const u64 *vb = v + (u64)b * batch;
        const u32 nChunks = bw <= 4 ? 0 : (bw + 7) / 8;
        const bool closes = (b & 1) || b == nb - 1;
        for (u32 i = 0; i < nChunks + (closes ? 1 : 0); i++) {
            if (i < nChunks) {
                const u32 n = min(8u, bw - 8 * i);
#pragma unroll
                for (u32 j = 0; j < 8; j++) st[j] = j < n ? vb[8 * i + j] : 0;
                if (i == 0) st[8] = st[9] = st[10] = st[11] = 0;
            } else {
                u64 d[4];
#pragma unroll
                for (u32 j = 0; j < 4; j++) d[j] = nChunks ? canon(st[8 + j]) : (j < bw ? vb[j] : 0);
#pragma unroll
                for (u32 j = 0; j < 4; j++) {
                    st[j] = (b & 1) ? park[j][tid] : d[j];
                    st[4 + j] = (b & 1) ? d[j] : 0;
                    st[8 + j] = b >= 2 ? park[4 + j][tid] : 0;
                }
            }
            poseidon_perm<0, 4>(st, m);
            st[8] = st[0]; st[9] = st[1]; st[10] = st[2]; st[11] = st[3];
        }
        if (!closes) {
#pragma unroll
            for (u32 j = 0; j < 4; j++) park[j][tid] = nChunks ? canon(st[8 + j]) : (j < bw ? vb[j] : 0);
        } else if (b < nb - 1) {
#pragma unroll
            for (u32 j = 0; j < 4; j++) park[4 + j][tid] = st[8 + j];
        }
    }
    if (!live) return;
    u64 *o = out + 4 * row;
    o[0] = canon(st[8]); o[1] = canon(st[9]); o[2] = canon(st[10]); o[3] = canon(st[11]);
}

__global__ void __launch_bounds__(256, 4) merkle_level_kernel(const u64 *__restrict__ in, u64 nOps, u64 *__restrict__ out) {
    const u64 i0 = (u64)blockIdx.x * blockDim.x + threadIdx.x;
    const bool live = i0 < nOps;
    const u64 i = live ? i0 : nOps - 1;
    MdsMfma m;
    poseidon_init(m);
    u64 st[12];
#pragma unroll
    for (int j = 0; j < 8; j++) st[j] = in[8 * i + j];
    st[8] = st[9] = st[10] = st[11] = 0;
    poseidon_perm<4, 4>(st, m);
    if (!live) return;
    u64 *o = out + 4 * i;
    o[0] = st[0]; o[1] = st[1]; o[2] = st[2]; o[3] = st[3];
}

__global__ void __launch_bounds__(256, 2) merkle_path_roots_kernel(const u64 *__restrict__ leaf, const u64 *__restrict__ sib, const u64 *__restrict__ idx,
                                                                  u64 count, u32 levels, u64 *__restrict__ roots) {
    const u64 i0 = (u64)blockIdx.x * blockDim.x + threadIdx.x;
    const bool live = i0 < count;
    const u64 i = live ? i0 : count - 1;
    MdsMfma m;
    poseidon_init(m);
    u64 cur[4];
#pragma unroll
    for (int j = 0; j < 4; j++) cur[j] = canon(leaf[4 * i + j]);
    u64 pos = idx[i];
    for (u32 l = 0; l < levels; l++) {
        const u64 *s = sib + (i * levels + l) * 4;
        const bool right = pos & 1;
        u64 st[12];
#pragma unroll
        for (int j = 0; j < 4; j++) { const u64 sv = canon(s[j]); st[j] = right ? sv : cur[j]; st[4 + j] = right ? cur[j] : sv; }
        st[8] = st[9] = st[10] = st[11] = 0;
        poseidon_perm(st, m);
#pragma unroll
        for (int j = 0; j < 4; j++) cur[j] = st[j];
        pos >>= 1;
    }
    if (!live) return;
#pragma unroll
    for (int j = 0; j < 4; j++) roots[4 * i + j] = cur[j];
}

__global__ void __launch_bounds__(64) sponge_chain_kernel(const u64 *__restrict__ blocks, u64 nBlocks, const u64 *__restrict__ cap, u64 *__restrict__ out12) {
    constexpr u32 MC[12] = { 17, 15, 41, 16, 2, 28, 13, 13, 39, 18, 34, 20 };
    __shared__ u64 sh[12];
    const u32 lane = threadIdx.x;
    const bool act = lane < 12;
    const u32 l = act ? lane : 0;
    u32 mrow[12];
#pragma unroll
    for (int j = 0; j < 12; j++) mrow[j] = MC[(j + 12 - l) % 12] + ((l == 0 && j == 0) ? 8u : 0u);
    u64 carry = (act && l >= 8) ? canon(cap[l - 8]) : 0;
    u64 s = 0;
    for (u64 b = 0; b < nBlocks; b++) {
        s = l < 8 ? canon(blocks[8 * b + l]) : carry;
        for (int r = 0; r < 30; r++) {
            s = add_lazy_canon(s, POSEIDON_GL_RC[r * 12 + l]);
            const bool full = r < 4 || r >= 26;
            if (full || l == 0) s = pow7_lazy(s);
            if (act) sh[l] = s;
            __builtin_amdgcn_s_waitcnt(0xC07F);
            __builtin_amdgcn_wave_barrier();
            u64 al = 0, ah = 0;
#pragma unroll
            for (int j = 0; j < 12; j++) { const u64 v = sh[j]; al += (u64)(u32)v * mrow[j]; ah += (u64)(u32)(v >> 32) * mrow[j]; }
            __builtin_amdgcn_wave_barrier();
            const u64 lo = al + (ah << 32);
            const u64 hi = (ah >> 32) + (lo < al ? 1 : 0);
            s = reduce128_lazy(lo, hi);
        }
        s = canon(s);
        if (act) sh[l] = s;
        __builtin_amdgcn_s_waitcnt(0xC07F);
        __builtin_amdgcn_wave_barrier();
        carry = (l >= 8) ? sh[l - 8] : 0;
        __builtin_amdgcn_wave_barrier();
    }
    if (act) out12[l] = s;
}

__global__ void __launch_bounds__(256, 4) poseidon_batch_kernel(const u64 *__restrict__ in, const u64 *__restrict__ cap, u64 count, u32 nOut, u64 *__restrict__ out) {
    const u64 i0 = (u64)blockIdx.x * blockDim.x + threadIdx.x;
    const bool live = i0 < count;
    const u64 i = live ? i0 : count - 1;
    MdsMfma m;
    poseidon_init(m);
    u64 st[12];
#pragma unroll
    for (int j = 0; j < 8; j++) st[j] = canon(in[8 * i + j]);
#pragma unroll
    for (int j = 0; j < 4; j++) st[8 + j] = cap ? canon(cap[4 * i + j]) : 0;
    poseidon_perm(st, m);
    if (!live) return;
    for (u32 j = 0; j < nOut; j++) out[(u64)nOut * i + j] = st[j];
}

__global__ void __launch_bounds__(256, 2) mds_selftest_kernel(const u64 *__restrict__ in, u64 n, u32 layers, int mfma, u64 *__restrict__ out) {
    const u64 i0 = (u64)blockIdx.x * blockDim.x + threadIdx.x;
    const bool live = i0 < n;
    const u64 i = live ? i0 : n - 1;
    MdsMfma m;
    mds_mfma_init(m);
    u64 st[12];
#pragma unroll
    for (int j = 0; j < 12; j++) st[j] = in[12 * i + j];
    for (u32 l = 0; l < layers; l++) { if (mfma) mds_layer_mfma(st, m); else mds_layer(st); }
    if (!live) return;
#pragma unroll
    for (int j = 0; j < 12; j++) out[12 * i + j] = canon(st[j]);
}

__global__ void __launch_bounds__(256, 2) poseidon_selftest_kernel(const u64 *__restrict__ in, u64 n, int what, u64 *__restrict__ out) {
    const u64 i0 = (u64)blockIdx.x * blockDim.x + threadIdx.x;
    const bool live = i0 < n;
    const u64 i = live ? i0 : n - 1;
    MdsMfma m;
    mds_mfma_init(m);
    poseidon_init(m);
    u64 st[12];
#pragma unroll
    for (int j = 0; j < 12; j++) st[j] = in[12 * i + j];
    if (what == 0) poseidon_perm(st, m);
    else if (what == 1) poseidon_perm_single(st, m);
    else if (what == 2) poseidon_perm(st);
    else poseidon_partial_rounds(st, m, what == 3 ? 0 : 1);
    if (!live) return;
#pragma unroll
    for (int j = 0; j < 12; j++) out[12 * i + j] = canon(st[j]);
}

__global__ void __launch_bounds__(256, 4) clock_probe_kernel(u64 *__restrict__ sink, int iters, u64 *__restrict__ clk) {
    MdsMfma m;
    poseidon_init(m);
    u64 st[12];
    const u64 id = (u64)blockIdx.x * blockDim.x + threadIdx.x;
#pragma unroll
    for (int j = 0; j < 12; j++) st[j] = ((id * 12 + j) * 0x9E3779B97F4A7C15ull) >> 1;
    const u64 c0 = __builtin_readcyclecounter(), r0 = wall_clock64();
    for (int i = 0; i < iters; i++) poseidon_perm<0>(st, m);
    const u64 c1 = __builtin_readcyclecounter(), r1 = wall_clock64();
    u64 x = 0;
#pragma unroll
    for (int j = 0; j < 12; j++) x ^= st[j];
    sink[id] = x;
    if (threadIdx.x == 0) { clk[2 * blockIdx.x] = c1 - c0; clk[2 * blockIdx.x + 1] = r1 - r0; }
}

__global__ void group_proofs_kernel(const u64 *__restrict__ elems, const u64 *__restrict__ nodes, u64 width, u64 height,
                                    const u64 *__restrict__ idxs, u32 nLevels, u64 *__restrict__ out) {
    const u64 stride = width + 4ull * nLevels;
    u64 *o = out + (u64)blockIdx.x * stride;
    u64 idx = idxs[blockIdx.x];
    for (u64 c = threadIdx.x; c < width; c += blockDim.x) o[c] = elems[idx * width + c];
    if (threadIdx.x < 4) {
        u64 offset = 0, n = height * 4;
        for (u32 l = 0; l < nLevels; l++) {
            o[width + 4 * l + threadIdx.x] = nodes[offset + (idx ^ 1) * 4 + threadIdx.x];
            const u64 nextN = ((n - 1) / 8 + 1) * 4;
            offset += nextN * 2; n = nextN; idx >>= 1;
        }
    }
}

}

using namespace pil2gl;

extern "C" {

uint64_t pil2gl_merkle_num_nodes(uint64_t height) {
    if (height == 0) return 0;
    uint64_t n = height * 4;
    uint64_t nextN = ((n - 1) / 8 + 1) * 4;
    uint64_t acc = nextN * 2;
    while (n > 4) {
        n = nextN;
        nextN = ((n - 1) / 8 + 1) * 4;
        if (n > 4) acc += nextN * 2; else acc += 4;
    }
    return acc;
}

int pil2gl_linear_hash_rows_dev(const uint64_t *in, uint64_t width, uint64_t height, int split, uint64_t *out, void *stream) {
    P2_TRY(ensure_init());
    if (height == 0) return PIL2GL_OK;
    if (!out || (!in && width)) return fail(PIL2GL_EINVAL, "null buffer");
    if (width >= (1ull << 31)) return fail(PIL2GL_EINVAL, "row width too large");
    u64 blocks = (height + 255) / 256;
    if (blocks > 0x7fffffffull) return fail(PIL2GL_EINVAL, "grid too large");
    if (split && width > 8) linear_hash_split_kernel<<<(unsigned)((height + SPLIT_BLOCK - 1) / SPLIT_BLOCK), SPLIT_BLOCK, 0, as_stream(stream)>>>(in, width, height, out);
    else linear_hash_kernel<<<(unsigned)blocks, 256, 0, as_stream(stream)>>>(in, width, height, out);
    KERNEL_CHECK();
    return PIL2GL_OK;
}

int pil2gl_merkelize_level_dev(const uint64_t *in, uint64_t nOps, uint64_t *out, void *stream) {
    P2_TRY(ensure_init());
    if (nOps == 0) return PIL2GL_OK;
    if (!in || !out) return fail(PIL2GL_EINVAL, "null buffer");
    if (nOps > (0x7fffffffull << 8)) return fail(PIL2GL_EINVAL, "grid too large");
    merkle_level_kernel<<<(unsigned)((nOps + 255) / 256), 256, 0, as_stream(stream)>>>(in, nOps, out);
    KERNEL_CHECK();
    return PIL2GL_OK;
}

int pil2gl_poseidon_dev(const uint64_t *in, const uint64_t *cap, uint64_t count, uint32_t nOut, uint64_t *out, void *stream) {
    P2_TRY(ensure_init());
    if (count == 0) return PIL2GL_OK;
    if (!in || !out) return fail(PIL2GL_EINVAL, "null buffer");
    if (nOut < 1 || nOut > 12) return fail(PIL2GL_EINVAL, "nOut must be 1..12");
    if (count > (0x7fffffffull << 8)) return fail(PIL2GL_EINVAL, "grid too large");
    poseidon_batch_kernel<<<(unsigned)((count + 255) / 256), 256, 0, as_stream(stream)>>>(in, cap, count, nOut, out);
    KERNEL_CHECK();
    return PIL2GL_OK;
}

int pil2gl_merkelize_digests_dev(uint64_t *nodes, uint64_t height, void *stream) {
    P2_TRY(ensure_init());
    if (height == 0) return fail(PIL2GL_EINVAL, "height must be > 0");
    if (!nodes) return fail(PIL2GL_EINVAL, "null buffer");
    hipStream_t st = as_stream(stream);
    u64 total = pil2gl_merkle_num_nodes(height);
    if (total > height * 4) HIP_TRY(hipMemsetAsync(nodes + height * 4, 0, (total - height * 4) * 8, st));
    u64 pIn = 0, n64 = height * 4;
    u64 nextN64 = ((n64 - 1) / 8 + 1) * 4;
    u64 pOut = pIn + nextN64 * 2;
    while (n64 > 4) {
        P2_TRY(pil2gl_merkelize_level_dev(nodes + pIn, nextN64 / 4, nodes + pOut, stream));
        n64 = nextN64;
        nextN64 = ((n64 - 1) / 8 + 1) * 4;
        pIn = pOut;
        pOut = pIn + nextN64 * 2;
    }
    return PIL2GL_OK;
}

int pil2gl_merkelize_dev(const uint64_t *elems, uint64_t width, uint64_t height, int split, uint64_t *nodes, void *stream) {
    P2_TRY(ensure_init());
    if (height == 0) return fail(PIL2GL_EINVAL, "height must be > 0");
    if (!nodes || (!elems && width)) return fail(PIL2GL_EINVAL, "null buffer");
    P2_TRY(pil2gl_linear_hash_rows_dev(elems, width, height, split, nodes, stream));
    return pil2gl_merkelize_digests_dev(nodes, height, stream);
}

int pil2gl_group_proof_dev(const uint64_t *elems, const uint64_t *nodes, uint64_t width, uint64_t height,
                           uint64_t idx, uint64_t *hostVals, uint64_t *hostSiblings, uint32_t *nLevels) {
    P2_TRY(ensure_init());
    if (idx >= height) return fail(PIL2GL_EINVAL, "Out of range");
    if (!nodes || !hostSiblings || (width && (!elems || !hostVals))) return fail(PIL2GL_EINVAL, "null buffer");
    if (width) HIP_TRY(hipMemcpy(hostVals, elems + idx * width, width * 8, hipMemcpyDeviceToHost));
    u64 offset = 0, n = height * 4;
    uint32_t lvl = 0;
    while (n > 4) {
        u64 si = (idx ^ 1) * 4;
        HIP_TRY(hipMemcpy(hostSiblings + 4 * lvl, nodes + offset + si, 32, hipMemcpyDeviceToHost));
        u64 nextN = ((n - 1) / 8 + 1) * 4;
        offset += nextN * 2; n = nextN; idx >>= 1; lvl++;
    }
    if (nLevels) *nLevels = lvl;
    return PIL2GL_OK;
}

int pil2gl_group_proofs_dev(const uint64_t *elems, const uint64_t *nodes, uint64_t width, uint64_t height,
                            const uint64_t *hostIdxs, uint32_t nIdx, uint64_t *hostOut, uint32_t *nLevels) {
    P2_TRY(ensure_init());
    if (!nIdx) return PIL2GL_OK;
    if (!nodes || !hostIdxs || !hostOut || (!elems && width)) return fail(PIL2GL_EINVAL, "null buffer");
    u32 lv = 0;
    for (u64 n = height * 4; n > 4; n = ((n - 1) / 8 + 1) * 4) lv++;
    for (u32 i = 0; i < nIdx; i++) if (hostIdxs[i] >= height) return fail(PIL2GL_EINVAL, "Out of range");
    const u64 stride = width + 4ull * lv;
    u64 *d;
    P2_TRY(scratch(6, (u64)nIdx * (stride + 1), &d));
    u64 *dIdx = d + (u64)nIdx * stride;
    HIP_TRY(hipMemcpy(dIdx, hostIdxs, (u64)nIdx * 8, hipMemcpyHostToDevice));
    group_proofs_kernel<<<nIdx, 64>>>(elems, nodes, width, height, dIdx, lv, d);
    KERNEL_CHECK();
    HIP_TRY(hipMemcpy(hostOut, d, (u64)nIdx * stride * 8, hipMemcpyDeviceToHost));
    if (nLevels) *nLevels = lv;
    return PIL2GL_OK;
}

int pil2gl_roots_from_group_proofs(const uint64_t *hostProofs, uint64_t width, uint32_t levels, const uint64_t *hostIdxs, uint32_t nIdx,
                                   int splitLinearHash, uint64_t *hostRoots) {
    P2_TRY(ensure_init());
    if (!nIdx) return PIL2GL_OK;
    if (!hostProofs || !hostIdxs || !hostRoots) return fail(PIL2GL_EINVAL, "null buffer");
    if (levels > 64) return fail(PIL2GL_EINVAL, "too many levels");
    const u64 stride = width + 4ull * levels, nv = (u64)nIdx * width, ns = (u64)nIdx * levels * 4;
    std::vector<u64> h(nv + ns + nIdx + 1);
    for (u32 q = 0; q < nIdx; q++) {
        memcpy(h.data() + (u64)q * width, hostProofs + q * stride, width * 8);
        memcpy(h.data() + nv + (u64)q * levels * 4, hostProofs + q * stride + width, 4ull * levels * 8);
        h[nv + ns + q] = hostIdxs[q];
    }
    u64 *d;
    P2_TRY(scratch(6, nv + ns + nIdx + 8ull * nIdx + 1, &d));
    u64 *dVals = d, *dSib = d + nv, *dIdx = dSib + ns, *dLeaf = dIdx + nIdx, *dRoots = dLeaf + 4ull * nIdx;
    HIP_TRY(hipMemcpy(d, h.data(), (nv + ns + nIdx) * 8, hipMemcpyHostToDevice));
    P2_TRY(pil2gl_linear_hash_rows_dev(dVals, width, nIdx, splitLinearHash, dLeaf, nullptr));
    merkle_path_roots_kernel<<<(nIdx + 255) / 256, 256>>>(dLeaf, dSib, dIdx, nIdx, levels, dRoots);
    KERNEL_CHECK();
    HIP_TRY(hipMemcpy(hostRoots, dRoots, 4ull * nIdx * 8, hipMemcpyDeviceToHost));
    return PIL2GL_OK;
}

int pil2gl_sponge_absorb(const uint64_t *hostBlocks, uint64_t nBlocks, const uint64_t hostCap[4], uint64_t hostOut12[12]) {
    P2_TRY(ensure_init());
    if (!hostBlocks || !hostCap || !hostOut12) return fail(PIL2GL_EINVAL, "null buffer");
    if (nBlocks == 0) return fail(PIL2GL_EINVAL, "nothing to absorb");
    u64 *d; bool owned;
    P2_TRY(stage_acquire(8 * nBlocks + 4 + 12, &d, &owned));
    int rc = PIL2GL_OK;
    hipError_t e = hipMemcpy(d, hostBlocks, 8 * nBlocks * 8, hipMemcpyHostToDevice);
    if (e == hipSuccess) e = hipMemcpy(d + 8 * nBlocks, hostCap, 32, hipMemcpyHostToDevice);
    if (e != hipSuccess) rc = hip_fail(e, "hipMemcpy H2D");
    if (rc == PIL2GL_OK) {
        sponge_chain_kernel<<<1, 64>>>(d, nBlocks, d + 8 * nBlocks, d + 8 * nBlocks + 4);
        e = hipGetLastError();
        if (e == hipSuccess) e = hipMemcpy(hostOut12, d + 8 * nBlocks + 4, 96, hipMemcpyDeviceToHost);
        if (e != hipSuccess) rc = hip_fail(e, "sponge_chain_kernel");
    }
    stage_release(d, owned);
    return rc;
}

static int with_dev(const uint64_t *hIn, u64 nIn, const uint64_t *hIn2, u64 nIn2, uint64_t *hOut, u64 nOut,
                    int (*fn)(const u64 *, const u64 *, u64 *, void *), void *arg) {
    P2_TRY(ensure_init());
    u64 *d = nullptr; bool owned = false;
    P2_TRY(stage_acquire(nIn + nIn2 + nOut, &d, &owned));
    int rc = PIL2GL_OK;
    hipError_t e = hipSuccess;
    if (nIn) e = hipMemcpy(d, hIn, nIn * 8, hipMemcpyHostToDevice);
    if (e == hipSuccess && nIn2) e = hipMemcpy(d + nIn, hIn2, nIn2 * 8, hipMemcpyHostToDevice);
    if (e != hipSuccess) rc = hip_fail(e, "hipMemcpy H2D");
    if (rc == PIL2GL_OK) rc = fn(d, nIn2 ? d + nIn : nullptr, d + nIn + nIn2, arg);
    if (rc == PIL2GL_OK && nOut) { e = hipMemcpy(hOut, d + nIn + nIn2, nOut * 8, hipMemcpyDeviceToHost); if (e != hipSuccess) rc = hip_fail(e, "hipMemcpy D2H"); }
    stage_release(d, owned);
    return rc;
}
struct LhArgs { u64 width, height; int split; };
struct PsArgs { u64 count; u32 nOut; };

int pil2gl_linear_hash_rows(const uint64_t *in, uint64_t width, uint64_t height, int split, uint64_t *out) {
    LhArgs a = { width, height, split };
    return with_dev(in, width * height, nullptr, 0, out, height * 4,
                    [](const u64 *i, const u64 *, u64 *o, void *p) { LhArgs *a = (LhArgs *)p; return pil2gl_linear_hash_rows_dev(i, a->width, a->height, a->split, o, nullptr); }, &a);
}
int pil2gl_merkelize_level(const uint64_t *in, uint64_t nOps, uint64_t *out) {
    return with_dev(in, nOps * 8, nullptr, 0, out, nOps * 4,
                    [](const u64 *i, const u64 *, u64 *o, void *p) { return pil2gl_merkelize_level_dev(i, *(u64 *)p, o, nullptr); }, &nOps);
}
int pil2gl_poseidon(const uint64_t *in, const uint64_t *cap, uint64_t count, uint32_t nOut, uint64_t *out) {
    if (nOut < 1 || nOut > 12) return fail(PIL2GL_EINVAL, "nOut must be 1..12");
    PsArgs a = { count, nOut };
    return with_dev(in, count * 8, cap, cap ? count * 4 : 0, out, count * nOut,
                    [](const u64 *i, const u64 *c, u64 *o, void *p) { PsArgs *a = (PsArgs *)p; return pil2gl_poseidon_dev(i, c, a->count, a->nOut, o, nullptr); }, &a);
}
struct MdsArgs { u64 n; u32 layers; int mfma; };
int pil2gl_selftest_mds(const uint64_t *states, uint64_t n, uint32_t layers, int mfma, uint64_t *out) {
    if (n == 0) return PIL2GL_OK;
    MdsArgs a = { n, layers, mfma };
    return with_dev(states, n * 12, nullptr, 0, out, n * 12,
                    [](const u64 *i, const u64 *, u64 *o, void *p) {
                        MdsArgs *a = (MdsArgs *)p;
                        mds_selftest_kernel<<<(unsigned)((a->n + 255) / 256), 256>>>(i, a->n, a->layers, a->mfma, o);
                        KERNEL_CHECK();
                        return (int)PIL2GL_OK;
                    }, &a);
}
int pil2gl_selftest_poseidon(const uint64_t *states, uint64_t n, int what, uint64_t *out) {
    if (n == 0) return PIL2GL_OK;
    if (what < 0 || what > 4) return fail(PIL2GL_EINVAL, "what must be 0..4");
    MdsArgs a = { n, 0, what };
    return with_dev(states, n * 12, nullptr, 0, out, n * 12,
                    [](const u64 *i, const u64 *, u64 *o, void *p) {
                        MdsArgs *a = (MdsArgs *)p;
                        poseidon_selftest_kernel<<<(unsigned)((a->n + 255) / 256), 256>>>(i, a->n, a->mfma, o);
                        KERNEL_CHECK();
                        return (int)PIL2GL_OK;
                    }, &a);
}
int pil2gl_selftest_clock(uint32_t iters, double *mhz ) {
    P2_TRY(ensure_init());
    if (!mhz || iters == 0 || iters > 4096) return fail(PIL2GL_EINVAL, "iters must be 1..4096");
    const unsigned blocks = 256 * 4 * 8;
    u64 *d;
    P2_TRY(scratch(5, (u64)blocks * 256 + 2ull * blocks, &d));
    clock_probe_kernel<<<blocks, 256>>>(d, (int)iters, d + (u64)blocks * 256);
    KERNEL_CHECK();
    std::vector<u64> h(2 * blocks);
    HIP_TRY(hipMemcpy(h.data(), d + (u64)blocks * 256, 16ull * blocks, hipMemcpyDeviceToHost));
    std::vector<double> v;
    for (unsigned i = 0; i < blocks; i++) if (h[2 * i + 1]) v.push_back(100.0 * (double)h[2 * i] / (double)h[2 * i + 1]);
    if (v.empty()) return fail(PIL2GL_EHIP, "no clock samples");
    std::sort(v.begin(), v.end());
    mhz[0] = v[v.size() / 2]; mhz[1] = v[v.size() / 20]; mhz[2] = v[v.size() * 19 / 20];
    return PIL2GL_OK;
}
int pil2gl_merkelize(const uint64_t *elems, uint64_t width, uint64_t height, int split, uint64_t *nodes) {
    if (height == 0) return fail(PIL2GL_EINVAL, "height must be > 0");
    LhArgs a = { width, height, split };
    return with_dev(elems, width * height, nullptr, 0, nodes, pil2gl_merkle_num_nodes(height),
                    [](const u64 *i, const u64 *, u64 *o, void *p) { LhArgs *a = (LhArgs *)p; return pil2gl_merkelize_dev(i, a->width, a->height, a->split, o, nullptr); }, &a);
}

}
```

### pil2-stark-js_amd/python/pil2gl/_lib.py

```python
import ctypes as C
import os

_HERE = os.path.dirname(os.path.abspath(__file__))
PKG_ROOT = os.path.dirname(os.path.dirname(_HERE))
LIB_PATH = os.environ.get("PIL2GL_LIB") or os.path.join(PKG_ROOT, "lib", "libpil2gl.so")

u64p = C.POINTER(C.c_uint64)
vp = C.c_void_p


class Pil2glError(RuntimeError):
    pass


class GlxRef(C.Structure):
    _fields_ = [("kind", C.c_uint8), ("dim", C.c_uint8), ("section", C.c_uint16),
                ("prime", C.c_int32), ("index", C.c_uint32), ("pad_", C.c_uint32)]


class GlxOp(C.Structure):
    _fields_ = [("op", C.c_uint32), ("pad_", C.c_uint32), ("dest", GlxRef), ("src", GlxRef * 2)]


class GlxSection(C.Structure):
    _fields_ = [("ptr", C.c_void_p), ("width", C.c_uint64)]


class GlxCtx(C.Structure):
    _fields_ = [("nBits", C.c_uint32), ("primeShift", C.c_uint32), ("nSections", C.c_uint32),
                ("nScalars", C.c_uint32), ("sections", C.POINTER(GlxSection)), ("scalars", u64p)]


class GlxProgram(C.Structure):
    _fields_ = [("nOps", C.c_uint32), ("nTmp", C.c_uint32), ("ops", C.POINTER(GlxOp))]


class EvalDesc(C.Structure):
    _fields_ = [("buf", C.c_void_p), ("width", C.c_uint64), ("offset", C.c_uint64),
                ("dim", C.c_uint32), ("levIndex", C.c_uint32)]


_U64, _U32, _I = C.c_uint64, C.c_uint32, C.c_int
SIGNATURES = {
    "pil2gl_init": (_I, [_I]),
    "pil2gl_shutdown": (None, []),
    "pil2gl_last_error": (C.c_char_p, []),
    "pil2gl_version": (_I, []),
    "pil2gl_device_info": (_I, [C.c_char_p, _U32, C.POINTER(_U32), C.POINTER(_U64)]),
    "pil2gl_dev_alloc": (_I, [_U64, C.POINTER(vp)]),
    "pil2gl_dev_free": (_I, [vp]),
    "pil2gl_dev_zero": (_I, [vp, _U64, vp]),
    "pil2gl_dev_upload": (_I, [vp, vp, _U64]),
    "pil2gl_add": (_U64, [_U64, _U64]),
    "pil2gl_mul": (_U64, [_U64, _U64]),
    "pil2gl_square": (_U64, [_U64]),
    "pil2gl_dev_download": (_I, [vp, vp, _U64]),
    "pil2gl_sync": (_I, [vp]),
    "pil2gl_host_alloc": (_I, [_U64, C.POINTER(vp)]),
    "pil2gl_host_free": (_I, [vp]),
    "pil2gl_host_register": (_I, [vp, _U64]),
    "pil2gl_host_unregister": (_I, [vp]),
    "pil2gl_dev_upload_async": (_I, [vp, vp, _U64]),
    "pil2gl_dev_download_async": (_I, [vp, vp, _U64]),
    "pil2gl_copy_after": (_I, [vp]),
    "pil2gl_copy_fence": (_I, [vp]),
    "pil2gl_copy_sync": (_I, []),
    "pil2gl_land_rows_dev": (_I, [vp, _U64, vp, _U64, _U64, C.POINTER(_U64), vp]),
    "pil2gl_dev_load_file": (_I, [C.c_char_p, _U64, _U64, _U64, vp, _U64, _U64, C.POINTER(_U64)]),
    "pil2gl_dev_save_file": (_I, [C.c_char_p, _U64, vp, _U64, _U64]),
    "pil2gl_interpolate": (_I, [vp, _U64, _U32, vp, _U32]),
    "pil2gl_interpolate_dev": (_I, [vp, _U64, _U32, vp, _U32, vp]),
    "pil2gl_interpolate_cosets_dev": (_I, [vp, _U64, _U32, vp, _U32, _U32, _U32, vp]),
    "pil2gl_extend_cosets_unshifted_dev": (_I, [vp, _U64, _U32, vp, _U32, _U32, _U32, vp]),
    "pil2gl_interpolate_cosets_ws_dev": (_I, [vp, _U64, _U32, vp, _U32, _U32, _U32, vp, vp]),
    "pil2gl_fft": (_I, [vp, _U64, _U32, vp]),
    "pil2gl_ifft": (_I, [vp, _U64, _U32, vp]),
    "pil2gl_fft_dev": (_I, [vp, _U64, _U32, vp, vp]),
    "pil2gl_ifft_dev": (_I, [vp, _U64, _U32, vp, vp]),
    "pil2gl_poseidon": (_I, [vp, vp, _U64, _U32, vp]),
    "pil2gl_poseidon_dev": (_I, [vp, vp, _U64, _U32, vp, vp]),
    "pil2gl_linear_hash_rows": (_I, [vp, _U64, _U64, _I, vp]),
    "pil2gl_linear_hash_rows_dev": (_I, [vp, _U64, _U64, _I, vp, vp]),
    "pil2gl_merkelize_level": (_I, [vp, _U64, vp]),
    "pil2gl_merkelize_level_dev": (_I, [vp, _U64, vp, vp]),
    "pil2gl_merkle_num_nodes": (_U64, [_U64]),
    "pil2gl_merkelize": (_I, [vp, _U64, _U64, _I, vp]),
    "pil2gl_merkelize_dev": (_I, [vp, _U64, _U64, _I, vp, vp]),
    "pil2gl_merkelize_digests_dev": (_I, [vp, _U64, vp]),
    "pil2gl_group_proof_dev": (_I, [vp, vp, _U64, _U64, _U64, vp, vp, C.POINTER(_U32)]),
    "pil2gl_group_proofs_dev": (_I, [vp, vp, _U64, _U64, vp, _U32, vp, C.POINTER(_U32)]),
    "pil2gl_roots_from_group_proofs": (_I, [vp, _U64, _U32, vp, _U32, C.c_int, vp]),
    "pil2gl_sponge_absorb": (_I, [vp, _U64, vp, vp]),
    "pil2gl_bn128_sponge_absorb": (_I, [vp, _U64, _U32, vp, vp]),
    "pil2gl_fri_fold": (_I, [vp, _U32, _U32, _U64, vp, vp]),
    "pil2gl_fri_fold_dev": (_I, [vp, _U32, _U32, _U64, vp, vp, vp]),
    "pil2gl_fri_verify_fold": (_I, [vp, _U32, _U32, vp, vp, vp]),
    "pil2gl_fri_verify_fold_dev": (_I, [vp, _U32, _U32, vp, vp, vp, vp]),
    "pil2gl_fri_transpose": (_I, [vp, _U32, _U32, vp]),
    "pil2gl_fri_transpose_dev": (_I, [vp, _U32, _U32, vp, vp]),
    "pil2gl_build_x_dev": (_I, [_U32, _U64, vp, vp]),
    "pil2gl_geometric_dev": (_I, [_U64, _U64, _U64, vp, vp]),
    "pil2gl_build_zhinv_dev": (_I, [_U32, _U32, vp, vp]),
    "pil2gl_build_one_row_zerofier_inv_dev": (_I, [_U32, _U32, _U64, vp, vp]),
    "pil2gl_build_frame_zerofier_dev": (_I, [_U32, _U32, _U64, _U64, vp, vp]),
    "pil2gl_compute_q_split_dev": (_I, [vp, _U32, _U32, _U32, _U32, vp, vp]),
    "pil2gl_compute_q_split_brev_dev": (_I, [vp, _U32, _U32, _U32, _U32, vp, vp]),
    "pil2gl_compute_q_stark_dev": (_I, [C.POINTER(GlxProgram), C.POINTER(GlxCtx), _U32, _U32, _U32, _U32, _U32, vp, vp]),
    "pil2gl_extend_coefs_brev_dev": (_I, [vp, _U64, _U32, vp, _U32, vp]),
    "pil2gl_extend_coefs_brev_cosets_dev": (_I, [vp, _U64, _U32, vp, _U32, _U32, _U32, vp]),
    "pil2gl_x_div_x_sub_xi_dev": (_I, [_U32, vp, _U64, _U64, vp, vp]),
    "pil2gl_x_div_x_sub_xi_cosets_dev": (_I, [_U32, _U32, vp, _U64, _U64, _U32, _U32, vp, vp]),
    "pil2gl_build_lev_dev": (_I, [_U32, vp, vp, vp]),
    "pil2gl_compute_evals_dev": (_I, [C.POINTER(EvalDesc), _U32, _U32, _U32, C.POINTER(vp), _U32, vp, vp]),
    "pil2gl_rows_dot_ext_dev": (_I, [vp, _U64, _U64, vp, _U32, vp, _I, vp]),
    "pil2gl_rows_dot_ext_multi_dev": (_I, [vp, vp, _U32, _U64, vp, _U32, vp, _I, vp]),
    "pil2gl_fri_combine_dev": (_I, [vp, vp, vp, vp, _U32, _U64, vp, vp]),
    "pil2gl_fri_combine_order_dev": (_I, [vp, vp, vp, vp, _U32, vp, _U64, vp, vp]),
    "pil2gl_cols_dot_ext_dev": (_I, [vp, _U64, _U64, _U64, C.POINTER(vp), _U32, vp, vp]),
    "pil2gl_cols_dot_ext_multi_dev": (_I, [vp, vp, _U32, _U64, _U64, vp, _U32, vp, vp]),
    "pil2gl_cols_dot_ext_range_dev": (_I, [vp, vp, vp, vp, _U32, _U64, _U64, vp, _U32, vp, vp]),
    "pil2gl_eval_program_dev": (_I, [C.POINTER(GlxProgram), C.POINTER(GlxCtx), vp]),
    "pil2gl_first_nonzero_row_dev": (_I, [vp, _U32, _U64, _U64, vp, vp, vp]),
    "pil2gl_fft_block_dev": (_I, [vp, _U64, _U64, _U32, _U32, _U32, _U32, vp]),
    "pil2gl_interpolate_prepare_block_dev": (_I, [vp, _U64, _U64, _U64, _U64, vp]),
    "pil2gl_synth_fibonacci_dev": (_I, [_U32, _U32, vp, vp, vp]),
    "pil2gl_debug_compact_program": (_I, [C.POINTER(GlxProgram), C.POINTER(GlxOp), C.POINTER(_U32)]),
    "pil2gl_debug_jit_compile": (_I, [C.POINTER(GlxProgram), C.POINTER(GlxCtx), C.POINTER(_U64), C.POINTER(_U32)]),
    "pil2gl_debug_plan_program": (_I, [C.POINTER(GlxProgram), C.POINTER(GlxCtx), C.POINTER(_U32)]),
    "pil2gl_debug_plan_transform": (_I, [_U32, _U32, _U64, _U32, _U32, C.POINTER(_U32), _U32, C.POINTER(_U32)]),
    "pil2gl_gprod_dev": (_I, [vp, _U32, vp, _U32, _U64, vp, vp]),
    "pil2gl_gsum_dev": (_I, [vp, _U32, vp, _U32, _U64, vp, vp]),
    "pil2gl_h1h2_dev": (_I, [vp, vp, _U64, _U32, vp, vp, vp]),
    "pil2gl_bn128_poseidon": (_I, [vp, vp, _U64, _U32, _U32, vp]),
    "pil2gl_bn128_poseidon_dev": (_I, [vp, vp, _U64, _U32, _U32, vp, vp]),
    "pil2gl_bn128_linear_hash_rows": (_I, [vp, _U64, _U64, _U32, _I, vp]),
    "pil2gl_bn128_linear_hash_rows_dev": (_I, [vp, _U64, _U64, _U32, _I, vp, vp]),
    "pil2gl_bn128_merkelize_level_dev": (_I, [vp, _U64, _U32, vp, vp]),
    "pil2gl_bn128_merkle_num_nodes": (_U64, [_U64, _U32]),
    "pil2gl_bn128_merkelize": (_I, [vp, _U64, _U64, _U32, _I, vp]),
    "pil2gl_bn128_merkelize_dev": (_I, [vp, _U64, _U64, _U32, _I, vp, vp]),
    "pil2gl_bn128_group_proof_dev": (_I, [vp, vp, _U64, _U64, _U32, _U64, vp, vp, vp]),
    "pil2gl_bn128_group_proofs_dev": (_I, [vp, vp, _U64, _U64, _U32, vp, _U32, vp, vp, vp]),
    "pil2gl_bn128_convert": (_I, [vp, _U64, _I, vp]),
    "pil2gl_bn128_convert_dev": (_I, [vp, _U64, _I, vp, vp]),
    "pil2gl_selftest_field": (_I, [vp, vp, _U64, vp, vp, vp]),
    "pil2gl_selftest_ext": (_I, [vp, vp, _U64, vp, vp]),
    "pil2gl_selftest_products": (_I, [vp, vp, _U64, vp, vp, vp]),
    "pil2gl_selftest_mds": (_I, [vp, _U64, _U32, _I, vp]),
    "pil2gl_selftest_poseidon": (_I, [vp, _U64, _I, vp]),
    "pil2gl_selftest_clock": (_I, [C.c_uint32, vp]),
}

_lib = None


def load():
    global _lib
    if _lib is not None:
        return _lib
    if not os.path.exists(LIB_PATH):
        raise Pil2glError("libpil2gl.so not built (%s): run `make -C pil2-stark-js_amd` or __graft_entry__.build(); "
                          "there is no CPU fallback" % LIB_PATH)
    L = C.CDLL(LIB_PATH)
    for name, (res, args) in SIGNATURES.items():
        fn = getattr(L, name)
        fn.restype = res
        fn.argtypes = args
    _lib = L
    return L


def check(rc):
    if rc != 0:
        msg = load().pil2gl_last_error()
        raise Pil2glError("pil2gl error %d: %s" % (rc, msg.decode() if msg else "?"))


def call(name, *args):
    check(getattr(load(), name)(*args))
```

### pil2-stark-js_amd/python/pil2gl/stark.py

```python
import ctypes as C

import numpy as np

from . import _lib
from ._lib import call

P = 0xFFFFFFFF00000001
SHIFT = 7
TMP, SEC, SCALAR = 0, 1, 2
OPC = {"add": 0, "sub": 1, "mul": 2, "copy": 3}


def _inv(a):
    return pow(int(a) % P, P - 2, P)


def root_of_unity(bits):
    w = 7277203076849721926
    for _ in range(32 - bits):
        w = w * w % P
    return w


def ext_mul(a, b):
# ... 400 lines not shown
        hints.append({"name": "gprod", "fields": [{"name": "numerator", "op": "tmp", "id": 2 + 2 * k, "dim": 3}, {"name": "denominator", "op": "tmp", "id": 3 + 2 * k, "dim": 3},
                                                  {"name": "reference", "op": "cm", "id": Z(k)}]
                                       + ([{"name": "result", "op": "subproofValue", "id": k}] if with_result else [])})
    expressionsInfo = {"imPolsCode": [{"tmpUsed": 0, "code": []}, {"tmpUsed": 0, "code": []}], "hintsInfo": hints, "expressionsCode": codes,
                       "constraints": constraint_codes([(c, {"boundary": "everyRow"}) for c in cexp(prover_leaf, None)], 2, "permutation.pil")}
    info["cExpId"], info["friExpId"] = 0, 1
    return info, expressionsInfo, {"qVerifier": qVerifier, "friexp": friexp}


def permutation_trace(n_bits, seed=3, stride=5, offset=3, copies=1):
    N = 1 << n_bits
    rng = np.random.default_rng(seed)
    cols = []
    for k in range(copies):
        a = rng.integers(0, 1 << 62, size=N, dtype=np.uint64)
        idx = (np.arange(N, dtype=np.uint64) * np.uint64(stride + 2 * k) + np.uint64(offset + k)) % np.uint64(N)
        cols += [a, a[idx.astype(np.int64)]]
    cm = np.stack(cols, axis=1).astype(np.uint64)
    consts = np.zeros((N, 2), dtype=np.uint64)
    consts[0, 0] = 1; consts[N - 1, 1] = 1
    return cm, consts, []


def fibonacci_trace(n_bits, n_pairs, seed=1, im_pols=False):
    N = 1 << n_bits
    rng = np.random.default_rng(seed)
    l2 = [int(v) for v in rng.integers(0, 1 << 62, size=n_pairs)]
    l1 = [int(v) for v in rng.integers(0, 1 << 62, size=n_pairs)]
    cm = np.zeros((N, 2 * n_pairs), dtype=np.uint64)
    a = np.array(l1, dtype=object); b = np.array(l2, dtype=object)
    for i in range(N):
        cm[i, 0::2] = np.array([int(v) for v in a], dtype=np.uint64); cm[i, 1::2] = np.array([int(v) for v in b], dtype=np.uint64)
        a, b = (a * a + b * b) % P, a
    consts = np.zeros((N, 2), dtype=np.uint64)
    consts[0, 0] = 1; consts[N - 1, 1] = 1
    publics = [int(cm[0, 1]), int(cm[0, 0]), int(cm[N - 1, 0])]
    if im_pols:
        cm = np.concatenate([cm, np.zeros((N, n_pairs), dtype=np.uint64)], axis=1)
    return cm, consts, publics


def query_verifier_of(info, exprs):
    import copy
    code = copy.deepcopy(expr_code(exprs, info["friExpId"])["code"])
    n_tmp = 1 + max([r["id"] for c in code for r in [c["dest"]] + c["src"] if r["type"] == "tmp"], default=-1)
    for c in code:
        for r in [c["dest"]] + c["src"]:
            if r["type"] == "cm":
                p = info["cmPolsMap"][r["id"]]
                r.update(type="tree%d" % p["stage"], treePos=p["stagePos"], dim=p["dim"], stageId=0)
                r.pop("id"); r.pop("prime", None)
            elif r["type"] == "const":
                r.pop("prime", None)
    assert code[-1]["dest"]["type"] == "f"
    code[-1]["dest"] = {"type": "tmp", "id": n_tmp, "dim": 3}
    return {"code": code}


def build_zi_table(be, boundary, nb, nbe):
    name = boundary["name"]
    if name == "everyRow":
        return be.build_zhinv(nb, nbe)
    if name == "firstRow":
        return be.build_one_row_zerofier_inv(nb, nbe, 0)
    if name == "lastRow":
        return be.build_one_row_zerofier_inv(nb, nbe, (1 << nb) - 1)
    if name == "everyFrame":
        return be.build_frame_zerofier(nb, nbe, boundary["offsetMin"], boundary["offsetMax"])
    raise ValueError("Boundary " + str(name) + " not supported")


def zi_at(boundary, xi, nb):
    N = 1 << nb
    xN = ext_pow(xi, N)
    zh = [(xN[0] - 1) % P, xN[1], xN[2]]
    name = boundary["name"]
    w = root_of_unity(nb)
    sub = lambda r: [(int(xi[0]) - r) % P, int(xi[1]), int(xi[2])]
    if name == "everyRow":
        return ext_inv(zh)
    if name == "firstRow":
        return ext_mul(zh, ext_inv(sub(1)))
    if name == "lastRow":
        return ext_mul(zh, ext_inv(sub(pow(w, N - 1, P))))
    if name == "everyFrame":
        z = [1, 0, 0]
        for j in range(boundary["offsetMin"]):
            z = ext_mul(z, sub(pow(w, j, P)))
        for j in range(boundary["offsetMax"]):
            z = ext_mul(z, sub(pow(w, N - j - 1, P)))
        return z
    raise ValueError("Boundary " + str(name) + " not supported")


def encode_code(code, dom, ctx):
    info = ctx["pilInfo"]
    sections, sec_index, scalars = [], {}, []

    def section(name):
        if name not in sec_index:
            sec_index[name] = len(sections); sections.append(name)
        return sec_index[name]

    def scalar(v):
        off = len(scalars)
        if isinstance(v, (list, tuple, np.ndarray)):
            scalars.extend(int(x) % P for x in v); return off, 3
        scalars.append(int(v) % P); return off, 1

    def ref(r):
        t = r["type"]
        if t == "tmp":
            return (TMP, r["dim"], 0, 0, r["id"])
        if t == "const":
            return (SEC, 1, section("const_" + dom), r.get("prime", 0), r["id"])
        if t == "cm":
            p = info["cmPolsMap"][r["id"]]
            return (SEC, p["dim"], section("cm%d_%s" % (p["stage"], dom)), r.get("prime", 0), p["stagePos"])
        if t.startswith("tree"):
            return (SEC, r["dim"], section("cm%d_%s" % (int(t[4:]), dom)), 0, r["treePos"])
        if t == "q":
            return (SEC, r["dim"], section("q_ext"), 0, 0)
        if t == "f":
            return (SEC, 3, section("f_ext"), 0, 0)
        if t == "$ret":
            return (SEC, r["dim"], section("$ret"), 0, 0)
        if t == "x":
            return (SEC, r.get("dim", 1), section("x_" + dom), 0, 0)
        if t == "Zi":
            return (SEC, 1, section("Zi_ext#%d" % r["boundaryId"]), 0, 0)
        if t == "xDivXSubXi":
            return (SEC, 3, section("xDivXSubXi_ext"), 0, 3 * r["id"])
        if t == "number":
            v = r["value"]
            o, d = scalar(int(v, 0) if isinstance(v, str) else int(v)); return (SCALAR, d, 0, 0, o)
        if t == "public":
            o, d = scalar(ctx["publics"][r["id"]]); return (SCALAR, d, 0, 0, o)
        if t == "challenge":
            ch = ctx["challenges"][r["stage"] - 1][r["stageId"]] if "stage" in r else ctx["challengesFlat"][r["id"]]
            o, _ = scalar(ch); return (SCALAR, 3, 0, 0, o)
        if t == "subproofValue":
            sv = ctx["subproofValues"]
            v = sv[r["subproofId"]][r["id"]] if ctx.get("global") else sv[r["id"]]
            o, d = scalar(v); return (SCALAR, d, 0, 0, o)
        if t == "eval":
            o, _ = scalar(ctx["evals"][r["id"]]); return (SCALAR, 3, 0, 0, o)
        raise ValueError("Invalid reference type get: " + t)
    ops, n_tmp = [], 0
    for c in code:
        for r in [c["dest"]] + c["src"]:
            if r["type"] == "tmp":
                n_tmp = max(n_tmp, r["id"] + 1)
    for c in code:
        if c["op"] == "muladd":
            prod = (TMP, max(r.get("dim", 1) for r in c["src"][:2]), 0, 0, n_tmp)
            ops.append((OPC["mul"], prod, ref(c["src"][0]), ref(c["src"][1])))
            ops.append((OPC["add"], ref(c["dest"]), prod, ref(c["src"][2])))
            continue
        if c["op"] not in OPC:
            raise ValueError("Invalid op:" + c["op"])
        ops.append((OPC[c["op"]], ref(c["dest"]), ref(c["src"][0]), ref(c["src"][1]) if c["op"] != "copy" else None))
    if any(c["op"] == "muladd" for c in code):
        n_tmp += 1
    return ops, n_tmp, sections, np.array(scalars if scalars else [0], dtype=np.uint64)


def make_c_program(ops, n_tmp):
    arr = (_lib.GlxOp * len(ops))()
    for k, (op, d, s0, s1) in enumerate(ops):
        arr[k].op = op
        for tgt, r in ((arr[k].dest, d), (arr[k].src[0], s0), (arr[k].src[1], s1)):
            if r is not None:
                tgt.kind, tgt.dim, tgt.section, tgt.prime, tgt.index = r
    prog = _lib.GlxProgram(len(ops), n_tmp, arr)
    prog._keep = arr
    return prog


class GpuBackend:
    name = "gpu"

    def __init__(self, device=0, split=False, hash_type="GL", arity=16, custom=False):
        import torch
        import pil2gl
        self.torch, self.gl = torch, pil2gl
        pil2gl.init(device)
        self.dev = torch.device("cuda", device)
        self.hash_type, self.arity, self.custom = hash_type, arity, custom
        if hash_type == "BN128":
            from pil2gl import bn128
            self.bn = bn128
            self.MH = bn128.buildMerkleHash(arity, custom)
        else:
            self.MH = pil2gl.buildMerkleHash(split)

    def _st(self):
        return C.c_void_p(self.torch.cuda.current_stream().cuda_stream)

    def _p(self, t):
        return C.c_void_p(t.data_ptr())

    def empty(self, n):
        return self.torch.empty(int(n), dtype=self.torch.int64, device=self.dev)

    def zeros(self, n):
        return self.torch.zeros(int(n), dtype=self.torch.int64, device=self.dev)

    def from_host(self, a):
        return self.torch.from_numpy(np.ascontiguousarray(a, dtype=np.uint64).reshape(-1).view(np.int64)).to(self.dev)

    def to_host(self, t):
        return t.reshape(-1).cpu().numpy().view(np.uint64)

    def interpolate(self, src, C_, nb, dst, nbe): self.gl.interpolate(src, C_, nb, dst, nbe)
    def fft(self, src, C_, nb, dst): self.gl.fft(src, C_, nb, dst)
    def ifft(self, src, C_, nb, dst): self.gl.ifft(src, C_, nb, dst)
    def merkelize(self, buf, w, h): return self.MH.merkelize(buf, w, h)
    def interpolate_cosets(self, src, C_, nb, dst, nbe, cb, cc, ws=None): self.gl.interpolateCosets(src, C_, nb, dst, nbe, cb, cc, ws)
    def merkelize_digest_block(self, parts, N, cc, r, sliced=False):
        world = len(parts)
        nb_ = N // world
        h = nb_ * cc * world
        nodes = self.torch.empty(self.MH._getNNodes(h * 4), dtype=self.torch.int64, device=self.dev)
        leaf = nodes[:h * 4].view(nb_, world, cc * 4)
        for s_, part in enumerate(parts):
            leaf[:, s_, :] = (part.view(nb_, cc * 4) if sliced else part.view(N, cc * 4)[r * nb_:(r + 1) * nb_]).to(self.dev, non_blocking=True)
        self.gl.call("pil2gl_merkelize_digests_dev", self._p(nodes), h, self._st())
        return nodes

    def extend_cosets_unshifted(self, src, C_, nb, dst, nbe, cb, cc):
        call("pil2gl_extend_cosets_unshifted_dev", self._p(src), C_, nb, self._p(dst), nbe, cb, cc, self._st())

    def extend_coefs_brev_cosets(self, coef_brev, C_, nb, dst, nbe, cb, cc):
        call("pil2gl_extend_coefs_brev_cosets_dev", self._p(coef_brev), C_, nb, self._p(dst), nbe, cb, cc, self._st())

    def linear_hash_rows(self, buf, w, h): return self.gl.linearHash(buf[:w * h], w, self.MH.splitLinearHash)
    def linear_hash_rows_into(self, buf, w, h, out): self.gl.linearHash(buf[:w * h], w, self.MH.splitLinearHash, out=out)
    def merkelize_digests(self, leaves, h): return self.MH.merkelizeDigests(leaves, h)

    def merkelize_digest_parts(self, parts, N, cc):
        world, h = len(parts), N * cc * len(parts)
        nodes = self.torch.empty(self.MH._getNNodes(h * 4), dtype=self.torch.int64, device=self.dev)
        leaf = nodes[:h * 4].view(N, world, cc * 4)
        for r, part in enumerate(parts):
            leaf[:, r, :] = part.view(N, cc * 4).to(self.dev, non_blocking=True)
        self.gl.call("pil2gl_merkelize_digests_dev", self._p(nodes), h, self._st())
        return nodes
    def as_torch(self, t): return t
    def from_torch(self, t): return t.to(self.dev)
    def root(self, tree): return self.MH.root(tree)
    def group_proofs(self, tree, idxs):
        return self.MH.getGroupProofs(tree, idxs)

    def get_column(self, buf, width, off, dim, n): return buf.view(n, width)[:, off:off + dim].contiguous().reshape(-1)
    def set_column(self, buf, width, off, dim, n, col): buf.view(n, width)[:, off:off + dim] = col.view(n, dim)
    def gprod(self, num, dn, den, dd): return self.gl.calculateZ(num, den, dn, dd)
    def gsum(self, num, dn, den, dd): return self.gl.calculateS(num, den, dn, dd)
    def h1h2(self, f, t, dim): return self.gl.calculateH1H2(f, t, dim)

    def merkle_siblings(self, nodes, height, idxs):
        tree = {"elements": self.empty(1), "nodes": nodes, "width": 0, "height": height}
        return [mp for _, mp in self.MH.getGroupProofs(tree, idxs)]

    def new_transcript(self):
        if self.hash_type == "BN128":
            return self.bn.Transcript(self.arity if self.custom else 16)
        return self.gl.Transcript()
    def poseidon(self, inp, cap, n): return self.gl.poseidon(inp, cap, n)

    def build_x(self, nb, shift):
        x = self.empty(1 << nb); call("pil2gl_build_x_dev", nb, shift, self._p(x), self._st()); return x

    def geometric(self, first, ratio, n):
        o = self.empty(n); call("pil2gl_geometric_dev", int(first) % P, int(ratio) % P, int(n), self._p(o), self._st()); return o

    def build_zhinv(self, nb, nbe):
        z = self.empty(1 << nbe); call("pil2gl_build_zhinv_dev", nb, nbe, self._p(z), self._st()); return z

    def build_one_row_zerofier_inv(self, nb, nbe, row):
        z = self.empty(1 << nbe); call("pil2gl_build_one_row_zerofier_inv_dev", nb, nbe, row, self._p(z), self._st()); return z

    def build_frame_zerofier(self, nb, nbe, off_min, off_max):
        z = self.empty(1 << nbe); call("pil2gl_build_frame_zerofier_dev", nb, nbe, off_min, off_max, self._p(z), self._st()); return z

    def q_extend(self, qq1, nb, nbe, qDim, qDeg, out):
        c = self.empty((qDim * qDeg) << nb)
        call("pil2gl_compute_q_split_brev_dev", self._p(qq1), nb, nbe, qDim, qDeg, self._p(c), self._st())
        call("pil2gl_extend_coefs_brev_dev", self._p(c), qDim * qDeg, nb, self._p(out), nbe, self._st())

    def q_stark(self, ops, n_tmp, sections, scalars, q_section, nb, nbe, qDim, qDeg, out):
        prog = make_c_program(ops, n_tmp)
        cs = (_lib.GlxSection * len(sections))()
        for i, (t, w) in enumerate(sections):
            cs[i].ptr = None if t is None else t.data_ptr(); cs[i].width = w
        ctx = _lib.GlxCtx(nbe, nbe - nb, len(sections), scalars.size, cs, scalars.ctypes.data_as(_lib.u64p))
        call("pil2gl_compute_q_stark_dev", C.byref(prog), C.byref(ctx), q_section, nb, nbe, qDim, qDeg, self._p(out), self._st())

    def q_split(self, qq1, nb, nbe, qDim, qDeg):
        o = self.empty((qDim * qDeg) << nbe)
        call("pil2gl_compute_q_split_dev", self._p(qq1), nb, nbe, qDim, qDeg, self._p(o), self._st()); return o

    def x_div_x_sub_xi(self, nbe, xis):
        n_open = len(xis); o = self.empty((3 * n_open) << nbe)
        for i, xi in enumerate(xis):
            a = np.array([int(v) % P for v in xi], dtype=np.uint64)
            call("pil2gl_x_div_x_sub_xi_dev", nbe, C.c_void_p(a.ctypes.data), n_open, i, self._p(o), self._st())
        return o

    def x_div_x_sub_xi_cosets(self, nbe, eb, xis, cb, cc):
        n_open = len(xis); o = self.empty((3 * n_open * cc) << (nbe - eb))
        for i, xi in enumerate(xis):
            a = np.array([int(v) % P for v in xi], dtype=np.uint64)
            call("pil2gl_x_div_x_sub_xi_cosets_dev", nbe, eb, C.c_void_p(a.ctypes.data), n_open, i, cb, cc, self._p(o), self._st())
        return o

    def build_lev(self, nb, xi):
        o = self.empty(3 << nb); a = np.array([int(v) % P for v in xi], dtype=np.uint64)
        call("pil2gl_build_lev_dev", nb, C.c_void_p(a.ctypes.data), self._p(o), self._st()); return o

    def compute_evals(self, descs, nb, eb, levs):
        n = len(descs)
        d = (_lib.EvalDesc * n)()
        for i, (buf, width, off, dim, li) in enumerate(descs):
            d[i].buf = buf.data_ptr(); d[i].width = width; d[i].offset = off; d[i].dim = dim; d[i].levIndex = li
        lv = (C.c_void_p * len(levs))(*[t.data_ptr() for t in levs])
        res = np.zeros((n, 3), np.uint64)
        call("pil2gl_compute_evals_dev", d, n, nb, eb, lv, len(levs), C.c_void_p(res.ctypes.data), self._st())
        return [[int(v) for v in r] for r in res]

    def eval_program(self, ops, n_tmp, sections, scalars, nb, prime_shift):
        prog = make_c_program(ops, n_tmp)
        cs = (_lib.GlxSection * len(sections))()
        for i, (t, w) in enumerate(sections):
            cs[i].ptr = t.data_ptr(); cs[i].width = w
        ctx = _lib.GlxCtx(nb, prime_shift, len(sections), scalars.size, cs, scalars.ctypes.data_as(_lib.u64p))
        call("pil2gl_eval_program_dev", C.byref(prog), C.byref(ctx), self._st())

    def fri_polynomial_fast(self, info, bufs, widths, evals, vf1, vf2, nbe, f_ext):
        plan = fri_polynomial_plan(info, evals, vf2)
        if plan is None:
            return False
        coefs, K, n_open, order = plan
        acc = self.empty((3 * n_open) << nbe)
        names = list(coefs)
        ptrs = (C.c_void_p * len(names))(*[bufs[nm].data_ptr() for nm in names])
        ws = np.array([widths[nm] for nm in names], dtype=np.uint64)
        cps = (C.c_void_p * len(names))(*[coefs[nm].ctypes.data for nm in names])
        call("pil2gl_rows_dot_ext_multi_dev", ptrs, C.c_void_p(ws.ctypes.data), len(names), 1 << nbe, cps, n_open, self._p(acc), 0, self._st())
        v1 = np.array([int(c) % P for c in vf1], dtype=np.uint64)
        od = np.array(order, dtype=np.uint32)
        call("pil2gl_fri_combine_order_dev", self._p(acc), C.c_void_p(K.ctypes.data), C.c_void_p(v1.ctypes.data), self._p(bufs["xDivXSubXi_ext"]),
             n_open, C.c_void_p(od.ctypes.data), 1 << nbe, self._p(f_ext), self._st())
        return True

    def eval_matrices(self, info):
        return sorted({("const_ext" if ev["type"] == "const" else "cm%d_ext" % info["cmPolsMap"][ev["id"]]["stage"]) for ev in info["evMap"]})

    def col_sums(self, names, bufs, widths, nb, eb, levs, ranges=None):
        n_lev = len(levs)
        lv = (C.c_void_p * n_lev)(*[t.data_ptr() for t in levs])
        sums = {name: np.zeros((n_lev, widths[name], 3), np.uint64) for name in names}
        live = [nm for nm in names if ranges is None or ranges[nm][1] > ranges[nm][0]]
        for g0 in range(0, len(live), 8):
            grp = live[g0:g0 + 8]
            ptrs = (C.c_void_p * len(grp))(*[bufs[nm].data_ptr() for nm in grp])
            st = np.array([widths[nm] for nm in grp], dtype=np.uint64)
            c0 = np.array([0 if ranges is None else ranges[nm][0] for nm in grp], dtype=np.uint64)
            ws = np.array([widths[nm] if ranges is None else ranges[nm][1] - ranges[nm][0] for nm in grp], dtype=np.uint64)
            part = [np.zeros((n_lev, int(w), 3), np.uint64) for w in ws]
            outs = (C.c_void_p * len(grp))(*[p.ctypes.data for p in part])
            call("pil2gl_cols_dot_ext_range_dev", ptrs, C.c_void_p(st.ctypes.data), C.c_void_p(c0.ctypes.data), C.c_void_p(ws.ctypes.data), len(grp), 1 << nb, 1 << eb, lv, n_lev, outs, self._st())
            for nm, b, w, p in zip(grp, c0, ws, part):
                sums[nm][:, int(b):int(b) + int(w)] = p
        return sums

    def evals_fast(self, info, bufs, widths, nb, eb, levs):
        return evals_from_col_sums(info, self.col_sums(self.eval_matrices(info), bufs, widths, nb, eb, levs))

    def fri_fold(self, pol, pol_bits, out_bits, shift_inv, challenge):
        o = self.empty(3 << out_bits); ch = np.array([int(c) % P for c in challenge], dtype=np.uint64)
        call("pil2gl_fri_fold_dev", self._p(pol), pol_bits, out_bits, shift_inv, C.c_void_p(ch.ctypes.data), self._p(o), self._st()); return o

    def fri_transpose(self, pol, pol_bits, t_bits):
        o = self.empty(3 << pol_bits); call("pil2gl_fri_transpose_dev", self._p(pol), pol_bits, t_bits, self._p(o), self._st()); return o

    def sync(self):
        self.torch.cuda.synchronize()


def evals_from_col_sums(info, sums):
    res = []
    for ev in info["evMap"]:
        li = info["openingPoints"].index(ev["prime"])
        if ev["type"] == "const":
            res.append([int(v) for v in sums["const_ext"][li, ev["id"]]])
        else:
            p = info["cmPolsMap"][ev["id"]]
            s = sums["cm%d_ext" % p["stage"]][li]
            if p["dim"] == 1:
                res.append([int(v) for v in s[p["stagePos"]]])
            else:
                acc = [0, 0, 0]
                for t in range(3):
                    term = [int(v) for v in s[p["stagePos"] + t]]
                    for _ in range(t):
                        term = ext_mul_x(term)
                    acc = [(a + b) % P for a, b in zip(acc, term)]
                res.append(acc)
    return res


class Transcript:
    def __init__(self, be):
        self.be, self.state, self.pending, self.out = be, [0, 0, 0, 0], [], []

    def _perm(self):
        while len(self.pending) < 8:
            self.pending.append(0)
        self.out = [int(v) for v in self.be.poseidon(self.pending, self.state, 12)]
        self.pending = []; self.state = self.out[:4]

    def put(self, a):
        if isinstance(a, (list, tuple, np.ndarray)):
            for v in a:
                self.put(v)
            return
        self.out = []
        self.pending.append(int(a))
        if len(self.pending) == 8:
            self._perm()

    def getState(self):
        if self.pending:
            self._perm()
        return self.state

    def getFields1(self):
        if not self.out:
            self._perm()
        return self.out.pop(0)

    def getField(self):
        return [self.getFields1(), self.getFields1(), self.getFields1()]

    def getPermutations(self, n, nBits):
        NFields = (n * nBits - 1) // 63 + 1
        fields = [self.getFields1() for _ in range(NFields)]
        res, cf, cb = [], 0, 0
        for _ in range(n):
            a = 0
            for j in range(nBits):
                if (fields[cf] >> cb) & 1:
                    a += 1 << j
                cb += 1
                if cb == 63:
                    cb = 0; cf += 1
            res.append(a)
        return res


def calculate_hash(be, inputs):
    t = be.new_transcript()
    for v in inputs:
        t.put(v)
    st = t.getState()
    return list(st) if isinstance(st, (list, tuple)) else st


def put_commit(be, transcript, values, hash_commits):
    transcript.put(calculate_hash(be, values) if hash_commits else values)


def build_const_tree(be, consts, info):
    ss = info["starkStruct"]
    nC = info["nConstants"]
    const_n = be.from_host(consts)
    const_ext = be.empty(nC << ss["nBitsExt"])
    be.interpolate(const_n, nC, ss["nBits"], const_ext, ss["nBitsExt"])
    tree = be.merkelize(const_ext, nC, 1 << ss["nBitsExt"])
    return {"const_n": const_n, "constTree": tree, "constRoot": be.root(tree)}


def fri_commit_phase(be, ss, f_ext, transcript, tree_builder=None, resume=None):
    steps = ss["steps"]
    friPol, friTrees, friProof, challengesFRI = f_ext, [None] * len(steps), [{} for _ in range(len(steps) + 1)], []
    pol_bits, first = steps[0]["nBits"], 0
    if resume is not None:
        first, friPol, friTrees, friProof, challengesFRI = resume
        pol_bits = steps[first]["nBits"]
    for step in range(first, len(steps)):
        out_bits = steps[step]["nBits"]
        if resume is None or step > first:
            ch = transcript.getField(); challengesFRI.append(ch)
            if step > 0:
                shift_inv = pow(_inv(SHIFT), 1 << (steps[0]["nBits"] - steps[step - 1]["nBits"]), P)
                friPol = be.fri_fold(friPol, pol_bits, out_bits, shift_inv, ch)
        if step < len(steps) - 1:
            gb = steps[step + 1]["nBits"]
            tb = be.fri_transpose(friPol, out_bits, gb)
            w, h = 3 * ((1 << out_bits) >> gb), 1 << gb
            tree = tree_builder(step + 1, tb, w, h) if tree_builder else None
            if tree is None:
                tree = be.merkelize(tb, w, h)
            friTrees[step + 1] = tree
            friProof[step + 1] = {"root": list(tree.root) if hasattr(tree, "root") else be.root(tree)}
            transcript.put(friProof[step + 1]["root"])
        else:
            last = [[int(v) for v in r] for r in be.to_host(friPol).reshape(-1, 3)]
            friProof[step + 1] = last
            put_commit(be, transcript, last, ss.get("hashCommits", False))
        pol_bits = out_bits
    return friTrees, friProof, challengesFRI


def expr_code(exprs, exp_id):
    e = next((x for x in exprs["expressionsCode"] if x and x.get("expId") == exp_id), None)
    if e is None:
        raise ValueError("expression %d not found" % exp_id)
    return e["code"]


def calculate_expression(be, exprs, exp_id, bufs, widths, nb, ctx):
    entry = next((e for e in exprs["expressionsCode"] if e and e.get("expId") == exp_id), None)
    if entry is None:
        raise ValueError("expression %d not found" % exp_id)
    code = [dict(c) for c in entry["code"]["code"]]
    if not code:
        raise ValueError("expression %d is empty" % exp_id)
    dim = code[-1]["dest"].get("dim", 1)
    if code[-1]["dest"]["type"] == "tmp":
        code[-1]["dest"] = {"type": "$ret", "dim": dim}
    else:
        code.append({"op": "copy", "dest": {"type": "$ret", "dim": dim}, "src": [dict(code[-1]["dest"])]})
    ops, n_tmp, secs, scalars = encode_code(code, "n", ctx)
    out = be.zeros(dim << nb)
    be.eval_program(ops, n_tmp, [((out, dim) if s_ == "$ret" else (bufs[s_], widths[s_])) for s_ in secs], scalars, nb, 0)
    return out, dim


def resolve_hints_info(be, info, exprs, stage, bufs, widths, nb, ctx):
    N = 1 << nb

    def field(h, name, required=True):
        f = next((x for x in h["fields"] if x["name"] == name), None)
        if f is None and required:
            raise ValueError("%s field is missing" % name)
        return f

    def column(f):
        if f["op"] == "cm":
            p = info["cmPolsMap"][f["id"]]
            name = "cm%d_n" % p["stage"]
            return be.get_column(bufs[name], widths[name], p["stagePos"], p["dim"], N), p["dim"]
        if f["op"] == "const":
            return be.get_column(bufs["const_n"], widths["const_n"], f["id"], 1, N), 1
        if f["op"] == "tmp":
            return calculate_expression(be, exprs, f["id"], bufs, widths, nb, ctx)
        raise ValueError("Case not considered")

    def field_stage(f):
        if f["op"] == "cm":
            return info["cmPolsMap"][f["id"]]["stage"]
        if f["op"] == "tmp":
            entry = next((e for e in exprs["expressionsCode"] if e and e.get("expId") == f["id"]), None)
            st = 0
            for c in (entry["code"]["code"] if entry else []):
                for r in [c["dest"]] + c["src"]:
                    if r["type"] == "cm":
                        st = max(st, info["cmPolsMap"][r["id"]]["stage"])
                    elif r["type"] == "challenge":
                        st = max(st, r.get("stage", 0))
            return st
        return 0

    def store(f, col, dim):
        p = info["cmPolsMap"][f["id"]]
        name = "cm%d_n" % p["stage"]
        if dim == 1 and p["dim"] == 3:
            wide = be.zeros(3 * N)
            be.set_column(wide, 3, 0, 1, N, col)
            col = wide
        elif dim != p["dim"]:
            raise ValueError("invalid dim")
        be.set_column(bufs[name], widths[name], p["stagePos"], p["dim"], N, col)
        return col

    for h in exprs.get("hintsInfo", []):
        if h["name"] in ("gprod", "gsum"):
            ref = field(h, "reference")
            if info["cmPolsMap"][ref["id"]]["stage"] != stage:
                continue
            den, dd = column(field(h, "denominator"))
            numf = field(h, "numerator")
            if h["name"] == "gprod":
                num, dn = column(numf)
                out = be.gprod(num, dn, den, dd)
            else:
                if numf["op"] != "number":
                    raise ValueError("gsum takes a constant numerator")
                out = be.gsum(be.from_host(np.array([int(numf["value"]) % P], dtype=np.uint64)), 1, den, dd)
            store(ref, out, max(dd, dn if h["name"] == "gprod" else 1))
            res = field(h, "result", required=False)
            if res is not None:
                last = [int(v) for v in be.to_host(out).reshape(N, -1)[N - 1]]
                sv = ctx.setdefault("subproofValues", [])
                while len(sv) <= res["id"]:
                    sv.append(0)
                sv[res["id"]] = last if len(last) == 3 else last[0]
        elif h["name"] == "h1h2":
            h1f = field(h, "referenceH1")
            if info["cmPolsMap"][h1f["id"]]["stage"] != stage:
                continue
            f_, df = column(field(h, "f")); t_, dt = column(field(h, "t"))
            if df != dt:
                raise ValueError("h1h2: f and t differ in dimension")
            h1, h2 = be.h1h2(f_, t_, df)
            store(h1f, h1, df); store(field(h, "referenceH2"), h2, df)
        elif h["name"] in ("public", "subproofValue"):
            ef = field(h, "expression")
            if max(1, field_stage(ef)) != stage:
                continue
            col, dim = column(ef)
            row = field(h, "row_index", required=False)
            r = int(row["value"]) if row is not None else N - 1
            v = [int(x) for x in be.to_host(col).reshape(N, -1)[r]]
            v = v if dim == 3 else v[0]
            ref = field(h, "reference")
            tgt = ctx["publics"] if h["name"] == "public" else ctx.setdefault("subproofValues", [])
            while len(tgt) <= ref["id"]:
                tgt.append(0)
            tgt[ref["id"]] = v
        else:
            raise ValueError("Unknown hint type " + h["name"])


def resolve_hints(be, info, stage, bufs, widths, nb, ctx, exprs=None):
    if exprs is not None and exprs.get("hintsInfo"):
        resolve_hints_info(be, info, exprs, stage, bufs, widths, nb, ctx)
    N = 1 << nb
    for h in info.get("hints", []):
        if h["stage"] != stage:
            continue
        name = "cm%d_n" % stage
        w = widths[name]

        def col(pid):
            p = info["cmPolsMap"][pid]
            return be.get_column(bufs[name], w, p["stagePos"], p["dim"], N), p["dim"]
        den, dd = col(h["denominator"])
        ref = info["cmPolsMap"][h["reference"]]
        if h["name"] == "gprod":
            num, dn = col(h["numerator"])
            out = be.gprod(num, dn, den, dd)
        elif h["name"] == "gsum":
            num = be.from_host(np.array([int(v) % P for v in h["numerator"]], dtype=np.uint64))
# ... 316 lines not shown
```

Baseline: 1.810 billion trace-cells/s.

## Fuse FRI polynomial combine into MFMA dot, batch xDiv kernels, single-block Merkle tail

The FRI polynomial step now folds the vf1 powers into the coefficients on the host. The MFMA rows-dot kernel combines each finished tile with xDivXSubXi and writes f directly, using one wave as a combiner that works one tile behind. This removes the intermediate accumulator round-trip and the separate combine kernel. The xDivXSubXi tables for all openings are built in one 2D-grid launch, and the Merkle tree build drops its memset and runs the last levels in a single-block kernel to cut many tiny launches. The risks are extra LDS use, one wave taken from the MFMA work, and changed padding handling for odd-sized levels.

```diff
diff --git a/include/pil2gl.h b/include/pil2gl.h
--- a/include/pil2gl.h
+++ b/include/pil2gl.h
@@ -99,6 +99,7 @@
 int pil2gl_x_div_x_sub_xi_dev(uint32_t nBitsExt, const uint64_t xi[3], uint64_t nOpen, uint64_t iOpen, uint64_t *out, void *stream);
 int pil2gl_x_div_x_sub_xi_cosets_dev(uint32_t nBitsExt, uint32_t extBits, const uint64_t xi[3], uint64_t nOpen, uint64_t iOpen,
                                      uint32_t cosetBegin, uint32_t cosetCount, uint64_t *out, void *stream);
+int pil2gl_x_div_x_sub_xi_all_dev(uint32_t nBitsExt, const uint64_t *xis, uint32_t nOpen, uint64_t *out, void *stream);
 int pil2gl_build_lev_dev(uint32_t nBits, const uint64_t xi[3], uint64_t *lev, void *stream);
 typedef struct { const uint64_t *buf; uint64_t width; uint64_t offset; uint32_t dim; uint32_t levIndex; } pil2gl_eval_desc;
 int pil2gl_compute_evals_dev(const pil2gl_eval_desc *descs, uint32_t nEvals, uint32_t nBits, uint32_t extendBits,
@@ -112,6 +113,9 @@
                            uint32_t nOpen, uint64_t nRows, uint64_t *f, void *stream);
 int pil2gl_fri_combine_order_dev(const uint64_t *acc, const uint64_t *hostK, const uint64_t vf1[3], const uint64_t *xDivXSubXi,
                                  uint32_t nOpen, const uint32_t *order, uint64_t nRows, uint64_t *f, void *stream);
+int pil2gl_fri_polynomial_dev(const uint64_t *const *bufs, const uint64_t *widths, uint32_t nBufs, uint64_t nRows,
+                              const uint64_t *const *hostCoefs, uint32_t nOpen, const uint64_t *hostK, const uint64_t vf1[3],
+                              const uint32_t *order, const uint64_t *xDivXSubXi, uint64_t *f, void *stream);
 int pil2gl_cols_dot_ext_dev(const uint64_t *buf, uint64_t width, uint64_t nRows, uint64_t rowStep, const uint64_t *const *levs,
                             uint32_t nLev, uint64_t *hostOut, void *stream);
 int pil2gl_cols_dot_ext_multi_dev(const uint64_t *const *bufs, const uint64_t *widths, uint32_t nBufs, uint64_t nRows, uint64_t rowStep,
diff --git a/pil2-stark-js_amd/csrc/dot.hip b/pil2-stark-js_amd/csrc/dot.hip
--- a/pil2-stark-js_amd/csrc/dot.hip
+++ b/pil2-stark-js_amd/csrc/dot.hip
@@ -191,6 +191,7 @@
 constexpr int MF_PLANE_OFFSET = 1 << 24;
 
 constexpr u32 MF_MAXSEG = 4;
+constexpr u32 MF_EXCH_BYTES = MF_ROWS * 6 * 8;
 struct RowsDotMfmaParams {
     const u64 *segBuf[MF_MAXSEG]; u32 segW[MF_MAXSEG], segPitch[MF_MAXSEG], segU0[MF_MAXSEG], nSeg;
     u64 nRows; u32 width, nOut;
@@ -199,10 +200,13 @@
     u64 *acc; u32 accumulate, accStride;
     u64 nTiles;
     u32 kSteps;
+    const u64 *xdiv; u64 *f;
+    u64 K[6];
+    u32 nOpen, o0, addF;
 };
 
 typedef int v4i_a8 __attribute__((ext_vector_type(4), aligned(8)));
-template <int NT, bool ODD = false>
+template <int NT, bool ODD = false, bool FUSE = false>
 __global__ void __launch_bounds__(512, 1) rows_dot_mfma_kernel(RowsDotMfmaParams P) {
     extern __shared__ u64 sm[];
     constexpr u32 NTH = 64 * MF_WAVES, NG = MF_ROWS / 32;
@@ -211,6 +215,30 @@
     const u32 rowBytes = P.width * 8, LDB = rowBytes + 16;
     unsigned char *tile = (unsigned char *)sm;
     v4i *Alds = (v4i *)(tile + MF_ROWS * LDB);
+    u64 *exch = (u64 *)(Alds + P.kSteps * NT * 64);
+    const bool combiner = FUSE && wave == MF_WAVES - 1;
+    const u32 nOutF = NT == 2 ? 1 : 2;
+    u64 prevRow0 = 0; bool pend = false;
+    u64 ex[6], xd[6], fp[3];
+    auto combine_load = [&](u64 row) {
+        if (row >= P.nRows) return;
+        const u64 *x = P.xdiv + (row * P.nOpen + P.o0) * 3;
+#pragma unroll
+        for (u32 j = 0; j < 6; j++) if (j < 3 * nOutF) xd[j] = x[j];
+        if (P.addF) { fp[0] = P.f[3 * row]; fp[1] = P.f[3 * row + 1]; fp[2] = P.f[3 * row + 2]; }
+    };
+    auto combine = [&](u64 row) {
+        if (row >= P.nRows) return;
+        E3 res = { { 0, 0, 0 } };
+        if (P.addF) res = { { fp[0], fp[1], fp[2] } };
+#pragma unroll
+        for (u32 j = 0; j < 2; j++) if (j < nOutF) {
+            const E3 F = { { sub(ex[3 * j], P.K[3 * j]), sub(ex[3 * j + 1], P.K[3 * j + 1]), sub(ex[3 * j + 2], P.K[3 * j + 2]) } };
+            const E3 X = { { xd[3 * j], xd[3 * j + 1], xd[3 * j + 2] } };
+            res = e3_add(res, e3_mul(F, X));
+        }
+        P.f[3 * row] = res.v[0]; P.f[3 * row + 1] = res.v[1]; P.f[3 * row + 2] = res.v[2];
+    };
     const u32 upr = P.width / 2;
     for (u32 i = tid; i < P.kSteps * NT * 64; i += NTH) Alds[i] = P.atab[i];
     const u32 n = lane & 31, gk = lane >> 5;
@@ -247,6 +275,7 @@
     for (u64 tileIdx = blockIdx.x; tileIdx < P.nTiles; tileIdx += gridDim.x) {
         const u64 row0 = tileIdx * MF_ROWS;
         __syncthreads();
+        if (combiner && pend) combine_load(prevRow0 + lane);
         {
             u32 r = r00, c = c00;
 #pragma unroll
@@ -257,6 +286,10 @@
             }
         }
         if (tileIdx + gridDim.x < P.nTiles) fetch(tileIdx + gridDim.x);
+        if (combiner && pend) {
+#pragma unroll
+            for (u32 j = 0; j < 6; j++) if (j < 3 * nOutF) ex[j] = exch[j * MF_ROWS + lane];
+        }
         __syncthreads();
         if (wave < NG * NT) {
             v16i acc;
@@ -275,8 +308,19 @@
                 v = add(sub(v, w[3]), P.bias[o]);
                 u64 *out = P.acc + row * (u64)P.accStride + o;
                 if (P.accumulate) v = add(v, *out);
-                *out = v;
-            }
+                if constexpr (FUSE) exch[o * MF_ROWS + 32 * g + n] = v;
+                else *out = v;
+            }
+        } else if (combiner && pend) combine(prevRow0 + lane);
+        if constexpr (FUSE) { prevRow0 = row0; pend = true; }
+    }
+    if constexpr (FUSE) {
+        __syncthreads();
+        if (combiner && pend) {
+            combine_load(prevRow0 + lane);
+#pragma unroll
+            for (u32 j = 0; j < 6; j++) if (j < 3 * nOutF) ex[j] = exch[j * MF_ROWS + lane];
+            combine(prevRow0 + lane);
         }
     }
 }
@@ -391,10 +435,12 @@
         ldsMax = v;
     }
     const u32 kSteps = (u32)((total * 8 + 31) / 32), NT = nOut == 1 ? 2 : 3;
-    const size_t need = (size_t)MF_ROWS * (total * 8 + 16) + (size_t)kSteps * NT * 1024;
+    const size_t need = (size_t)MF_ROWS * (total * 8 + 16) + (size_t)kSteps * NT * 1024 + MF_EXCH_BYTES;
     return (size_t)ldsMax >= need;
 }
-static int launch_rows_dot_mfma(const MfSeg *segs, u32 nBufs, u64 nRows, u32 nOut, u64 *acc, u32 accStride, bool accumulate, hipStream_t st) {
+struct MfFuse { const u64 *xdiv; u64 *f; const u64 *K; u32 nOpen, o0; bool addF; };
+static int launch_rows_dot_mfma(const MfSeg *segs, u32 nBufs, u64 nRows, u32 nOut, u64 *acc, u32 accStride, bool accumulate, hipStream_t st,
+                                const MfFuse *fuse = nullptr) {
     const u64 Pm = 0xFFFFFFFF00000001ull;
     const int NT = nOut == 1 ? 2 : 3;
     const u32 nO = 3 * nOut;
@@ -457,15 +503,23 @@
     }
     P.nSeg = nBufs; P.nRows = nRows; P.width = (u32)winWidth; P.nOut = nOut; P.atab = (const v4i *)d; P.bias = d + atWords;
     P.acc = acc; P.accumulate = (u32)accumulate; P.accStride = accStride; P.nTiles = (nRows + MF_ROWS - 1) / MF_ROWS; P.kSteps = kSteps;
-    const size_t lds = (size_t)MF_ROWS * (winWidth * 8 + 16) + atab.size();
+    P.xdiv = nullptr; P.f = nullptr; P.nOpen = P.o0 = P.addF = 0;
+    for (int i = 0; i < 6; i++) P.K[i] = 0;
+    if (fuse) {
+        P.xdiv = fuse->xdiv; P.f = fuse->f; P.nOpen = fuse->nOpen; P.o0 = fuse->o0; P.addF = fuse->addF;
+        for (u32 i = 0; i < nO; i++) P.K[i] = fuse->K[i] % Pm;
+    }
+    const size_t lds = (size_t)MF_ROWS * (winWidth * 8 + 16) + atab.size() + (fuse ? MF_EXCH_BYTES : 0);
     int dev = 0, cus = 256;
     (void)hipGetDevice(&dev);
     (void)hipDeviceGetAttribute(&cus, hipDeviceAttributeMultiprocessorCount, dev);
     const unsigned grid = (unsigned)std::min<u64>(P.nTiles, (u64)cus);
-#define RD_LAUNCH(NT_, ODD_) { HIP_TRY(hipFuncSetAttribute((const void *)rows_dot_mfma_kernel<NT_, ODD_>, hipFuncAttributeMaxDynamicSharedMemorySize, (int)lds)); \
-                              hipLaunchKernelGGL((rows_dot_mfma_kernel<NT_, ODD_>), dim3(grid), dim3(64 * MF_WAVES), lds, st, P); }
-    if (NT == 2) { if (odd) RD_LAUNCH(2, true) else RD_LAUNCH(2, false) }
-    else { if (odd) RD_LAUNCH(3, true) else RD_LAUNCH(3, false) }
+#define RD_LAUNCH(NT_, ODD_, FUSE_) { HIP_TRY(hipFuncSetAttribute((const void *)rows_dot_mfma_kernel<NT_, ODD_, FUSE_>, hipFuncAttributeMaxDynamicSharedMemorySize, (int)lds)); \
+                                     hipLaunchKernelGGL((rows_dot_mfma_kernel<NT_, ODD_, FUSE_>), dim3(grid), dim3(64 * MF_WAVES), lds, st, P); }
+#define RD_LAUNCH_F(NT_, ODD_) { if (fuse) RD_LAUNCH(NT_, ODD_, true) else RD_LAUNCH(NT_, ODD_, false) }
+    if (NT == 2) { if (odd) RD_LAUNCH_F(2, true) else RD_LAUNCH_F(2, false) }
+    else { if (odd) RD_LAUNCH_F(3, true) else RD_LAUNCH_F(3, false) }
+#undef RD_LAUNCH_F
 #undef RD_LAUNCH
     KERNEL_CHECK();
     HIP_TRY(hipStreamSynchronize(st));
@@ -618,6 +672,68 @@
     return PIL2GL_OK;
 }
 
+int pil2gl_fri_polynomial_dev(const uint64_t *const *bufs, const uint64_t *widths, uint32_t nBufs, uint64_t nRows,
+                              const uint64_t *const *hostCoefs, uint32_t nOpen, const uint64_t *hostK, const uint64_t vf1[3],
+                              const uint32_t *order, const uint64_t *xDivXSubXi, uint64_t *f, void *stream) {
+    P2_TRY(ensure_init());
+    if (!bufs || !widths || !hostCoefs || !hostK || !vf1 || !order || !xDivXSubXi || !f || nBufs == 0) return fail(PIL2GL_EINVAL, "null buffer");
+    for (uint32_t k = 0; k < nBufs; k++) if (!bufs[k] || !hostCoefs[k]) return fail(PIL2GL_EINVAL, "null buffer");
+    if (nOpen < 1 || nOpen > 4) return fail(PIL2GL_EINVAL, "nOpen must be 1..4");
+    u32 seen = 0;
+    for (u32 k = 0; k < nOpen; k++) {
+        if (order[k] >= nOpen || (seen >> order[k] & 1)) return fail(PIL2GL_EINVAL, "order must be a permutation of the openings");
+        seen |= 1u << order[k];
+    }
+    if (nRows == 0) return PIL2GL_OK;
+    const u64 Pm = 0xFFFFFFFF00000001ull;
+    u64 V[4][3];
+    {
+        const u64 v[3] = { vf1[0] % Pm, vf1[1] % Pm, vf1[2] % Pm };
+        u64 cur[3] = { 1, 0, 0 };
+        for (u32 k = nOpen; k-- > 0;) { for (int c = 0; c < 3; c++) V[order[k]][c] = cur[c]; u64 t[3]; h_e3_mul(cur, v, t); for (int c = 0; c < 3; c++) cur[c] = t[c]; }
+    }
+    std::vector<std::vector<u64>> sc(nBufs);
+    std::vector<const u64 *> scp(nBufs);
+    for (u32 k = 0; k < nBufs; k++) {
+        sc[k].resize((u64)nOpen * widths[k] * 3 + 1);
+        for (u32 o = 0; o < nOpen; o++)
+            for (u64 c = 0; c < widths[k]; c++) {
+                const u64 *w = hostCoefs[k] + ((u64)o * widths[k] + c) * 3;
+                const u64 wc[3] = { w[0] % Pm, w[1] % Pm, w[2] % Pm };
+                h_e3_mul(V[o], wc, sc[k].data() + ((u64)o * widths[k] + c) * 3);
+            }
+        scp[k] = sc[k].data();
+    }
+    u64 K[12];
+    for (u32 o = 0; o < nOpen; o++) { const u64 kc[3] = { hostK[3 * o] % Pm, hostK[3 * o + 1] % Pm, hostK[3 * o + 2] % Pm }; h_e3_mul(V[o], kc, K + 3 * o); }
+    std::vector<std::vector<MfSeg>> launches;
+    std::vector<u32> leftovers;
+    if (!rows_dot_mfma_plan(bufs, widths, scp.data(), nBufs, nOpen, launches, leftovers)) {
+        u64 *acc;
+        P2_TRY(scratch(1, nRows * 3 * nOpen, &acc));
+        P2_TRY(pil2gl_rows_dot_ext_multi_dev(bufs, widths, nBufs, nRows, scp.data(), nOpen, acc, 0, stream));
+        const u64 one[3] = { 1, 0, 0 };
+        return pil2gl_fri_combine_order_dev(acc, K, one, xDivXSubXi, nOpen, order, nRows, f, stream);
+    }
+    u64 *acc = nullptr;
+    if (launches.size() > 1 || !leftovers.empty()) P2_TRY(scratch(1, nRows * 3 * nOpen, &acc));
+    bool first = true;
+    for (u32 k : leftovers) { P2_TRY(rows_dot_ext_plain(bufs[k], widths[k], nRows, scp[k], nOpen, acc, first ? 0 : 1, stream)); first = false; }
+    for (u32 o0 = 0; o0 < nOpen; o0 += 2) {
+        const u32 no = std::min<u32>(2, nOpen - o0);
+        bool accg = !leftovers.empty();
+        for (size_t li = 0; li < launches.size(); li++) {
+            std::vector<MfSeg> l = launches[li];
+            for (MfSeg &sg : l) sg.coef += (u64)o0 * sg.pitch * 3;
+            const MfFuse fu = { xDivXSubXi, f, K + 3 * o0, nOpen, o0, o0 != 0 };
+            P2_TRY(launch_rows_dot_mfma(l.data(), (u32)l.size(), nRows, no, acc ? acc + 3 * o0 : nullptr, 3 * nOpen, accg, as_stream(stream),
+                                        li + 1 == launches.size() ? &fu : nullptr));
+            accg = true;
+        }
+    }
+    return PIL2GL_OK;
+}
+
 int pil2gl_cols_dot_ext_multi_dev(const uint64_t *const *bufs, const uint64_t *widths, uint32_t nBufs, uint64_t nRows, uint64_t rowStep,
                                   const uint64_t *const *levs, uint32_t nLev, uint64_t *const *hostOuts, void *stream) {
     return pil2gl_cols_dot_ext_range_dev(bufs, widths, nullptr, widths, nBufs, nRows, rowStep, levs, nLev, hostOuts, stream);
diff --git a/pil2-stark-js_amd/csrc/fri.hip b/pil2-stark-js_amd/csrc/fri.hip
--- a/pil2-stark-js_amd/csrc/fri.hip
+++ b/pil2-stark-js_amd/csrc/fri.hip
@@ -107,8 +107,8 @@
 }
 constexpr int XD_BATCH = 16;
 struct XDivConst { u64 xi0, b, c, c2, bc2, m1, k0, cc, ccbb; };
-__global__ void __launch_bounds__(256) x_div_x_sub_xi_kernel(u32 nBitsExt, XDivConst K, u64 nOpen, u64 iOpen, const u64 *__restrict__ powW, u64 wStep, u64 *__restrict__ out,
-                                                             u64 E , u32 extBits, u32 cosetBegin, u32 ccLog) {
+__device__ __forceinline__ void x_div_x_sub_xi_rows(u32 nBitsExt, const XDivConst &K, u64 nOpen, u64 iOpen, const u64 *__restrict__ powW, u64 wStep, u64 *__restrict__ out,
+                                                    u64 E , u32 extBits, u32 cosetBegin, u32 ccLog) {
     const u64 T = (u64)gridDim.x * blockDim.x;
     const u64 k0 = (u64)blockIdx.x * blockDim.x + threadIdx.x;
     if (k0 >= E) return;
@@ -143,6 +143,15 @@
         }
     }
 }
+__global__ void __launch_bounds__(256) x_div_x_sub_xi_kernel(u32 nBitsExt, XDivConst K, u64 nOpen, u64 iOpen, const u64 *__restrict__ powW, u64 wStep, u64 *__restrict__ out,
+                                                             u64 E, u32 extBits, u32 cosetBegin, u32 ccLog) {
+    x_div_x_sub_xi_rows(nBitsExt, K, nOpen, iOpen, powW, wStep, out, E, extBits, cosetBegin, ccLog);
+}
+constexpr u32 XD_MAX_OPEN = 8;
+struct XDivConstAll { XDivConst K[XD_MAX_OPEN]; };
+__global__ void __launch_bounds__(256) x_div_x_sub_xi_all_kernel(u32 nBitsExt, XDivConstAll A, u64 nOpen, const u64 *__restrict__ powW, u64 wStep, u64 *__restrict__ out) {
+    x_div_x_sub_xi_rows(nBitsExt, A.K[blockIdx.y], nOpen, blockIdx.y, powW, wStep, out, 1ull << nBitsExt, 0, 0, 0);
+}
 __global__ void lev_pow_kernel(u32 nBits, const u64 *__restrict__ xiPow, u64 *__restrict__ lev) {
     const u64 k = (u64)blockIdx.x * blockDim.x + threadIdx.x;
     if (k >= (1ull << nBits)) return;
@@ -420,6 +429,17 @@
 static bool base_point_is_a_row(u64 xi0, u64 xi1, u64 xi2, u32 nBitsExt) {
     return xi1 == 0 && xi2 == 0 && h_pow(h_mul(xi0, h_inv(7)), 1ull << nBitsExt) == 1;
 }
+static int x_div_consts(u32 nBitsExt, const uint64_t xi[3], XDivConst &K) {
+    const u64 GP = 0xFFFFFFFF00000001ull;
+    const u64 xi0 = xi[0] % GP, b = h_sub(0, xi[1] % GP), c = h_sub(0, xi[2] % GP);
+    if (base_point_is_a_row(xi0, b, c, nBitsExt)) return fail(PIL2GL_EINVAL, "xi is a point of the 2^%u-row coset 7<w>: x / (x - xi) divides by zero at that row", nBitsExt);
+    const u64 bb = h_mul(b, b), cc = h_mul(c, c), bc = h_mul(b, c);
+    K.xi0 = xi0; K.b = b; K.c = c; K.c2 = h_add(c, c); K.bc2 = h_add(bc, bc);
+    K.m1 = h_sub(h_add(bc, bb), cc);
+    K.k0 = h_sub(h_sub(h_mul(b, cc), h_mul(bb, b)), h_mul(cc, c));
+    K.cc = cc; K.ccbb = h_sub(cc, bb);
+    return PIL2GL_OK;
+}
 int pil2gl_x_div_x_sub_xi_dev(uint32_t nBitsExt, const uint64_t xi[3], uint64_t nOpen, uint64_t iOpen, uint64_t *out, void *stream) {
     return pil2gl_x_div_x_sub_xi_cosets_dev(nBitsExt, 0, xi, nOpen, iOpen, 0, 1, out, stream);
 }
@@ -431,20 +451,26 @@
         return fail(PIL2GL_EINVAL, "coset range [%u,%u) outside 2^%u (the count must be a power of two)", cosetBegin, cosetBegin + cosetCount, extBits);
     if (cosetCount > 256) return fail(PIL2GL_EINVAL, "at most 256 cosets per call (%u asked)", cosetCount);
     u32 ccLog = 0; while ((1u << ccLog) < cosetCount) ccLog++;
-    const u64 GP = 0xFFFFFFFF00000001ull;
-    const u64 xi0 = xi[0] % GP, b = h_sub(0, xi[1] % GP), c = h_sub(0, xi[2] % GP);
-    if (base_point_is_a_row(xi0, b, c, nBitsExt)) return fail(PIL2GL_EINVAL, "xi is a point of the 2^%u-row coset 7<w>: x / (x - xi) divides by zero at that row", nBitsExt);
-    const u64 bb = h_mul(b, b), cc = h_mul(c, c), bc = h_mul(b, c);
     XDivConst K;
-    K.xi0 = xi0; K.b = b; K.c = c; K.c2 = h_add(c, c); K.bc2 = h_add(bc, bc);
-    K.m1 = h_sub(h_add(bc, bb), cc);
-    K.k0 = h_sub(h_sub(h_mul(b, cc), h_mul(bb, b)), h_mul(cc, c));
-    K.cc = cc; K.ccbb = h_sub(cc, bb);
+    P2_TRY(x_div_consts(nBitsExt, xi, K));
     const u64 E = (1ull << (nBitsExt - extBits)) << ccLog;
     const unsigned blocks = nblk((E + XD_BATCH - 1) / XD_BATCH);
     const u64 T = (u64)blocks * 256;
     const u64 wStep = h_pow(h_root(nBitsExt), (T >> ccLog) << extBits);
     x_div_x_sub_xi_kernel<<<blocks, 256, 0, as_stream(stream)>>>(nBitsExt, K, nOpen, iOpen, tables().powW, wStep, out, E, extBits, cosetBegin, ccLog);
+    KERNEL_CHECK();
+    return PIL2GL_OK;
+}
+int pil2gl_x_div_x_sub_xi_all_dev(uint32_t nBitsExt, const uint64_t *xis, uint32_t nOpen, uint64_t *out, void *stream) {
+    P2_TRY(ensure_init());
+    if (!xis || !out || nOpen < 1 || nOpen > XD_MAX_OPEN || nBitsExt > 31) return fail(PIL2GL_EINVAL, "bad xDivXSubXi arguments");
+    XDivConstAll A;
+    for (u32 o = 0; o < XD_MAX_OPEN; o++) A.K[o] = XDivConst{};
+    for (u32 o = 0; o < nOpen; o++) P2_TRY(x_div_consts(nBitsExt, xis + 3 * o, A.K[o]));
+    const u64 E = 1ull << nBitsExt;
+    const unsigned blocks = nblk((E + XD_BATCH - 1) / XD_BATCH);
+    const u64 wStep = h_pow(h_root(nBitsExt), (u64)blocks * 256);
+    x_div_x_sub_xi_all_kernel<<<dim3(blocks, nOpen), 256, 0, as_stream(stream)>>>(nBitsExt, A, nOpen, tables().powW, wStep, out);
     KERNEL_CHECK();
     return PIL2GL_OK;
 }
diff --git a/pil2-stark-js_amd/csrc/merkle.hip b/pil2-stark-js_amd/csrc/merkle.hip
--- a/pil2-stark-js_amd/csrc/merkle.hip
+++ b/pil2-stark-js_amd/csrc/merkle.hip
@@ -93,20 +93,55 @@
     o[0] = canon(st[8]); o[1] = canon(st[9]); o[2] = canon(st[10]); o[3] = canon(st[11]);
 }
 
-__global__ void __launch_bounds__(256, 4) merkle_level_kernel(const u64 *__restrict__ in, u64 nOps, u64 *__restrict__ out) {
+__global__ void __launch_bounds__(256, 4) merkle_level_kernel(const u64 *__restrict__ in, u64 nOps, u64 *__restrict__ out, u64 *__restrict__ padIn) {
     const u64 i0 = (u64)blockIdx.x * blockDim.x + threadIdx.x;
     const bool live = i0 < nOps;
     const u64 i = live ? i0 : nOps - 1;
-    MdsMfma m;
-    poseidon_init(m);
-    u64 st[12];
-#pragma unroll
-    for (int j = 0; j < 8; j++) st[j] = in[8 * i + j];
+    const bool half = padIn && i == nOps - 1;
+    MdsMfma m;
+    poseidon_init(m);
+    u64 st[12];
+#pragma unroll
+    for (int j = 0; j < 4; j++) st[j] = in[8 * i + j];
+#pragma unroll
+    for (int j = 4; j < 8; j++) st[j] = half ? 0 : in[8 * i + j];
     st[8] = st[9] = st[10] = st[11] = 0;
     poseidon_perm<4, 4>(st, m);
     if (!live) return;
     u64 *o = out + 4 * i;
     o[0] = st[0]; o[1] = st[1]; o[2] = st[2]; o[3] = st[3];
+    if (half) padIn[0] = padIn[1] = padIn[2] = padIn[3] = 0;
+}
+
+constexpr u32 MERKLE_TAIL_OPS = 1024, MERKLE_TAIL_THREADS = 512;
+__global__ void __launch_bounds__(MERKLE_TAIL_THREADS) merkle_tail_kernel(u64 *in, u32 nIn) {
+    const u32 tid = threadIdx.x;
+    MdsMfma m;
+    poseidon_init(m);
+    if (nIn == 1 && tid < 4) in[4 + tid] = 0;
+    while (nIn > 1) {
+        const u32 nOps = (nIn + 1) / 2;
+        u64 *out = in + 8ull * nOps;
+        for (u32 i0 = tid; (u32)__builtin_amdgcn_readfirstlane((int)i0) < nOps; i0 += MERKLE_TAIL_THREADS) {
+            const bool live = i0 < nOps;
+            const u32 i = live ? i0 : nOps - 1;
+            const bool half = (nIn & 1) && i == nOps - 1;
+            u64 st[12];
+#pragma unroll
+            for (int j = 0; j < 4; j++) st[j] = in[8 * i + j];
+#pragma unroll
+            for (int j = 4; j < 8; j++) st[j] = half ? 0 : in[8 * i + j];
+            st[8] = st[9] = st[10] = st[11] = 0;
+            poseidon_perm<4, 4>(st, m);
+            if (live) {
+                u64 *o = out + 4 * i;
+                o[0] = st[0]; o[1] = st[1]; o[2] = st[2]; o[3] = st[3];
+                if (half) { u64 *p = in + 4ull * nIn; p[0] = p[1] = p[2] = p[3] = 0; }
+            }
+        }
+        __syncthreads();
+        in = out; nIn = nOps;
+    }
 }
 
 __global__ void __launch_bounds__(256, 2) merkle_path_roots_kernel(const u64 *__restrict__ leaf, const u64 *__restrict__ sib, const u64 *__restrict__ idx,
@@ -295,7 +330,7 @@
     if (nOps == 0) return PIL2GL_OK;
     if (!in || !out) return fail(PIL2GL_EINVAL, "null buffer");
     if (nOps > (0x7fffffffull << 8)) return fail(PIL2GL_EINVAL, "grid too large");
-    merkle_level_kernel<<<(unsigned)((nOps + 255) / 256), 256, 0, as_stream(stream)>>>(in, nOps, out);
+    merkle_level_kernel<<<(unsigned)((nOps + 255) / 256), 256, 0, as_stream(stream)>>>(in, nOps, out, nullptr);
     KERNEL_CHECK();
     return PIL2GL_OK;
 }
@@ -315,19 +350,17 @@
     P2_TRY(ensure_init());
     if (height == 0) return fail(PIL2GL_EINVAL, "height must be > 0");
     if (!nodes) return fail(PIL2GL_EINVAL, "null buffer");
+    if (height > (0x7fffffffull << 8)) return fail(PIL2GL_EINVAL, "grid too large");
     hipStream_t st = as_stream(stream);
-    u64 total = pil2gl_merkle_num_nodes(height);
-    if (total > height * 4) HIP_TRY(hipMemsetAsync(nodes + height * 4, 0, (total - height * 4) * 8, st));
-    u64 pIn = 0, n64 = height * 4;
-    u64 nextN64 = ((n64 - 1) / 8 + 1) * 4;
-    u64 pOut = pIn + nextN64 * 2;
-    while (n64 > 4) {
-        P2_TRY(pil2gl_merkelize_level_dev(nodes + pIn, nextN64 / 4, nodes + pOut, stream));
-        n64 = nextN64;
-        nextN64 = ((n64 - 1) / 8 + 1) * 4;
-        pIn = pOut;
-        pOut = pIn + nextN64 * 2;
-    }
+    u64 pIn = 0, nIn = height;
+    while (nIn > 1 && (nIn + 1) / 2 > MERKLE_TAIL_OPS) {
+        const u64 nOps = (nIn + 1) / 2, pOut = pIn + 8 * nOps;
+        merkle_level_kernel<<<(unsigned)((nOps + 255) / 256), 256, 0, st>>>(nodes + pIn, nOps, nodes + pOut, (nIn & 1) ? nodes + pIn + 4 * nIn : nullptr);
+        KERNEL_CHECK();
+        pIn = pOut; nIn = nOps;
+    }
+    merkle_tail_kernel<<<1, MERKLE_TAIL_THREADS, 0, st>>>(nodes + pIn, (u32)nIn);
+    KERNEL_CHECK();
     return PIL2GL_OK;
 }
 
diff --git a/pil2-stark-js_amd/python/pil2gl/_lib.py b/pil2-stark-js_amd/python/pil2gl/_lib.py
--- a/pil2-stark-js_amd/python/pil2gl/_lib.py
+++ b/pil2-stark-js_amd/python/pil2gl/_lib.py
@@ -110,12 +110,14 @@
     "pil2gl_extend_coefs_brev_cosets_dev": (_I, [vp, _U64, _U32, vp, _U32, _U32, _U32, vp]),
     "pil2gl_x_div_x_sub_xi_dev": (_I, [_U32, vp, _U64, _U64, vp, vp]),
     "pil2gl_x_div_x_sub_xi_cosets_dev": (_I, [_U32, _U32, vp, _U64, _U64, _U32, _U32, vp, vp]),
+    "pil2gl_x_div_x_sub_xi_all_dev": (_I, [_U32, vp, _U32, vp, vp]),
     "pil2gl_build_lev_dev": (_I, [_U32, vp, vp, vp]),
     "pil2gl_compute_evals_dev": (_I, [C.POINTER(EvalDesc), _U32, _U32, _U32, C.POINTER(vp), _U32, vp, vp]),
     "pil2gl_rows_dot_ext_dev": (_I, [vp, _U64, _U64, vp, _U32, vp, _I, vp]),
     "pil2gl_rows_dot_ext_multi_dev": (_I, [vp, vp, _U32, _U64, vp, _U32, vp, _I, vp]),
     "pil2gl_fri_combine_dev": (_I, [vp, vp, vp, vp, _U32, _U64, vp, vp]),
     "pil2gl_fri_combine_order_dev": (_I, [vp, vp, vp, vp, _U32, vp, _U64, vp, vp]),
+    "pil2gl_fri_polynomial_dev": (_I, [vp, vp, _U32, _U64, vp, _U32, vp, vp, vp, vp, vp, vp]),
     "pil2gl_cols_dot_ext_dev": (_I, [vp, _U64, _U64, _U64, C.POINTER(vp), _U32, vp, vp]),
     "pil2gl_cols_dot_ext_multi_dev": (_I, [vp, vp, _U32, _U64, _U64, vp, _U32, vp, vp]),
     "pil2gl_cols_dot_ext_range_dev": (_I, [vp, vp, vp, vp, _U32, _U64, _U64, vp, _U32, vp, vp]),
diff --git a/pil2-stark-js_amd/python/pil2gl/stark.py b/pil2-stark-js_amd/python/pil2gl/stark.py
--- a/pil2-stark-js_amd/python/pil2gl/stark.py
+++ b/pil2-stark-js_amd/python/pil2gl/stark.py
@@ -726,9 +726,8 @@
 
     def x_div_x_sub_xi(self, nbe, xis):
         n_open = len(xis); o = self.empty((3 * n_open) << nbe)
-        for i, xi in enumerate(xis):
-            a = np.array([int(v) % P for v in xi], dtype=np.uint64)
-            call("pil2gl_x_div_x_sub_xi_dev", nbe, C.c_void_p(a.ctypes.data), n_open, i, self._p(o), self._st())
+        a = np.array([[int(v) % P for v in xi] for xi in xis], dtype=np.uint64)
+        call("pil2gl_x_div_x_sub_xi_all_dev", nbe, C.c_void_p(a.ctypes.data), n_open, self._p(o), self._st())
         return o
 
     def x_div_x_sub_xi_cosets(self, nbe, eb, xis, cb, cc):
@@ -765,16 +764,14 @@
         if plan is None:
             return False
         coefs, K, n_open, order = plan
-        acc = self.empty((3 * n_open) << nbe)
         names = list(coefs)
         ptrs = (C.c_void_p * len(names))(*[bufs[nm].data_ptr() for nm in names])
         ws = np.array([widths[nm] for nm in names], dtype=np.uint64)
         cps = (C.c_void_p * len(names))(*[coefs[nm].ctypes.data for nm in names])
-        call("pil2gl_rows_dot_ext_multi_dev", ptrs, C.c_void_p(ws.ctypes.data), len(names), 1 << nbe, cps, n_open, self._p(acc), 0, self._st())
         v1 = np.array([int(c) % P for c in vf1], dtype=np.uint64)
         od = np.array(order, dtype=np.uint32)
-        call("pil2gl_fri_combine_order_dev", self._p(acc), C.c_void_p(K.ctypes.data), C.c_void_p(v1.ctypes.data), self._p(bufs["xDivXSubXi_ext"]),
-             n_open, C.c_void_p(od.ctypes.data), 1 << nbe, self._p(f_ext), self._st())
+        call("pil2gl_fri_polynomial_dev", ptrs, C.c_void_p(ws.ctypes.data), len(names), 1 << nbe, cps, n_open, C.c_void_p(K.ctypes.data),
+             C.c_void_p(v1.ctypes.data), C.c_void_p(od.ctypes.data), self._p(bufs["xDivXSubXi_ext"]), self._p(f_ext), self._st())
         return True
 
     def eval_matrices(self, info):
```

Result: no change. 1.805 billion trace-cells/s (-0.3%).
